# HyoJong-Moon/Distributed-Inference-System-based-Storm

Hardware: AMD Instinct MI355X
Metric: images/sec (whole node) + p50 latency, CIFAR-10 ResNet-20 at 1/2/4/8 GPUs (higher is better)
Workload: dtype bf16

## Files before the change

### csrc/bindings/host_bindings.cpp

```cpp
#include <pybind11/functional.h>
#include <pybind11/numpy.h>
#include <pybind11/pybind11.h>
#include <pybind11/stl.h>

#include <time.h>

#include <atomic>
#include <chrono>
#include <mutex>
#include <thread>

#include "../codec/json_codec.h"
#include "gale/llc_pair.h"
#include "../codec/text_pack.h"
#include "../kafka/broker.h"
#include "../kafka/client.h"
#include "../kafka/compress.h"
#include "../kafka/fetch_framing.h"
#include "../runtime/batch_plan.h"
#include "../runtime/ingest_plan.h"
#include "../runtime/pack_tap.h"
#include "../runtime/resize_plan.h"
#include "../kafka/protocol.h"
#include "../kafka/wire.h"
// ... 380 lines not shown
    const std::string_view s = view(b);
    const codec::Scan sc =
        codec::scan_instances(reinterpret_cast<const uint8_t*>(s.data()), s.size(), H, W, C);
    const int n = sc.status == codec::OK ? sc.images : 0;
    py::array_t<float> out({(py::ssize_t)n, (py::ssize_t)H, (py::ssize_t)W, (py::ssize_t)C});
    int images = 0;
    int st = sc.status;
    if (st == codec::OK)
      st = codec::parse_instances_host(reinterpret_cast<const uint8_t*>(s.data()), s.size(), H, W,
                                       C, out.mutable_data(), max_images, &images);
    return py::make_tuple(st, out);
  }, py::arg("data"), py::arg("H"), py::arg("W"), py::arg("C"), py::arg("max_images") = -1);
  m.def("scan_instances_b64", [](py::bytes b, int H, int W, int C) {
    const std::string_view s = view(b);
    const codec::Scan sc =
        codec::scan_instances_b64(reinterpret_cast<const uint8_t*>(s.data()), s.size(), H, W, C);
    return py::make_tuple(sc.status, sc.arr_off, sc.arr_len, sc.images);
  });
  m.def("parse_instances_b64_host", [](py::bytes b, int H, int W, int C, int max_images) {
    const std::string_view s = view(b);
    const uint8_t* p = reinterpret_cast<const uint8_t*>(s.data());
    const codec::Scan sc = codec::scan_instances_b64(p, s.size(), H, W, C);
    const int n = sc.status == codec::OK ? sc.images : 0;
    py::array_t<float> out({(py::ssize_t)n, (py::ssize_t)H, (py::ssize_t)W, (py::ssize_t)C});
    int images = 0;
    int st = sc.status;
    if (st == codec::OK)
      st = codec::parse_instances_b64_host(p, s.size(), H, W, C, out.mutable_data(), max_images,
                                           &images);
    return py::make_tuple(st, out);
  }, py::arg("data"), py::arg("H"), py::arg("W"), py::arg("C"), py::arg("max_images") = -1);
  m.def("b64_image_offsets", [](py::bytes arr, int H, int W, int C) -> py::object {
    const std::string_view s = view(arr);
    std::vector<uint32_t> offs;
    if (!codec::b64_image_offsets(reinterpret_cast<const uint8_t*>(s.data()), s.size(), H, W, C,
                                  offs))
      return py::none();
    return py::cast(offs);
  });
  m.def("plan_b64_ingest",
        [](std::vector<std::pair<int64_t, int64_t>> batches,
           std::vector<std::tuple<int, int, int64_t, int64_t, int64_t>> recs,
           std::vector<uint32_t> offs, int H, int W, int C, size_t arena_bytes,
           size_t fetch_size, bool check_crcs) {
          std::vector<B64PlanRecord> rs(recs.size());
          for (size_t i = 0; i < recs.size(); ++i) {
            rs[i].status = std::get<0>(recs[i]);
            rs[i].images = std::get<1>(recs[i]);
            rs[i].value_off = std::get<2>(recs[i]);
            rs[i].value_len = std::get<3>(recs[i]);
            rs[i].arr_off = std::get<4>(recs[i]);
          }
          B64IngestPlan p;
          plan_b64_ingest(batches, kafka::kBatchAttrOffset, check_crcs, rs, offs, H, W, C,
                          arena_bytes, fetch_size, p);
          py::list windows, imgs;
          for (const CrcChunk& c : p.chunks) windows.append(py::make_tuple(c.end, c.len));
          for (const B64Image& d : p.imgs) imgs.append(py::make_tuple(d.off, d.slot, d.rec));
          py::dict out;
          out["windows"] = windows;
          out["batch_windows"] = py::cast(p.batch_chunks);
          out["images"] = imgs;
          out["slot0"] = py::cast(p.slot0);
          out["img0"] = py::cast(p.img0);
          out["chunks_per_image"] = p.chunks_per_image;
          out["lo"] = p.lo;
          out["hi"] = p.hi;
          out["o_chunks"] = p.o_chunks;
          out["o_imgs"] = p.o_imgs;
          out["plan_bytes"] = p.plan_bytes;
          out["o_crc"] = p.o_crc;
          out["o_bad"] = p.o_bad;
          out["result_bytes"] = p.result_bytes;
          return out;
        },
        py::arg("batches"), py::arg("recs"), py::arg("offs"), py::arg("H"), py::arg("W"),
        py::arg("C"), py::arg("arena_bytes"), py::arg("fetch_size"),
        py::arg("check_crcs") = true,
        "The host plan of a b64 fetch's device ingest (csrc/runtime/ingest_plan.h)");
  m.def("plan_json_ingest",
        [](std::vector<std::pair<int64_t, int64_t>> batches,
           std::vector<std::tuple<int, int64_t, int64_t, int64_t, int64_t>> recs, int H, int W,
           int C, size_t arena_bytes, size_t fetch_size, size_t dev_cap, int64_t tap_result,
           bool plan_separate, bool check_crcs) {
          std::vector<JsonPlanRecord> rs(recs.size());
          for (size_t i = 0; i < recs.size(); ++i) {
            rs[i].status = std::get<0>(recs[i]);
            rs[i].value_off = std::get<1>(recs[i]);
            rs[i].value_len = std::get<2>(recs[i]);
            rs[i].arr_off = std::get<3>(recs[i]);
            rs[i].arr_len = std::get<4>(recs[i]);
          }
          JsonIngestPlan p;
          plan_json_ingest(batches, kafka::kBatchAttrOffset, check_crcs, rs, H, W, C, arena_bytes,
                           fetch_size, dev_cap, tap_result, plan_separate, p);
          std::string plan(p.o_gsum, '\0');
          if (!p.empty()) fill_json_ingest(p, rs, reinterpret_cast<uint8_t*>(&plan[0]));
          py::list windows;
          for (const CrcChunk& c : p.chunks) windows.append(py::make_tuple(c.end, c.len));
          py::dict out;
          out["windows"] = windows;
          out["batch_windows"] = py::cast(p.batch_chunks);
          out["rec_of"] = py::cast(p.rec_of);
          out["pjs"] = py::cast(p.pjs);
          out["nc"] = p.nc();
          out["nr"] = p.nr();
          out["np"] = p.np();
          out["ntiles"] = p.ntiles;
          out["ngroups"] = p.ngroups;
          out["ptiles"] = p.ptiles;
          out["ng"] = p.ng;
          out["packed"] = p.packed;
          out["lo"] = p.lo;
          out["span"] = p.span;
          out["link"] = p.link;
          out["c_lo"] = p.c_lo;
          out["c_len"] = p.c_len;
          out["tab_off"] = p.tab_off;
          out["used"] = p.used;
          out["cnt_base"] = p.cnt_base;
          out["o_chunks"] = p.o_chunks;
          out["o_groups"] = p.o_groups;
          out["o_recs"] = p.o_recs;
          out["o_precs"] = p.o_precs;
          out["o_ptr"] = p.o_ptr;
          out["o_gsum"] = p.o_gsum;
          out["prefix"] = p.o_gsum;
          out["o_crc"] = p.o_crc;
          out["o_gbad"] = p.o_gbad;
          out["o_pbad"] = p.o_pbad;
          out["io_bytes"] = p.io_bytes;
          out["plan_off"] = p.plan_off;
          out["plan_in_chunk"] = p.plan_in_chunk;
          out["plan"] = py::bytes(plan);
          return out;
        },
        py::arg("batches"), py::arg("recs"), py::arg("H"), py::arg("W"), py::arg("C"),
        py::arg("arena_bytes"), py::arg("fetch_size"), py::arg("dev_cap"),
        py::arg("tap_result") = (int64_t)-1, py::arg("plan_separate") = false,
        py::arg("check_crcs") = true,
        "The host plan of a JSON fetch's device ingest, laid out and filled "
        "(csrc/runtime/ingest_plan.h)");
  m.def("plan_batch",
        [](std::vector<py::dict> recs, int max_batch, int tiles_cap, int64_t per,
           const std::string& form, bool ptr_input, bool b64, uint64_t d_bytes,
           uint64_t input_base) {
          std::vector<BatchPlanRecord> rs(recs.size());
          std::vector<uint32_t> offs;
          for (size_t i = 0; i < recs.size(); ++i) {
            const py::dict& d = recs[i];
            BatchPlanRecord& r = rs[i];
            auto get = [&d](const char* k, auto& v) {
              if (d.contains(k)) v = d[k].cast<std::decay_t<decltype(v)>>();
            };
            get("buf", r.buf);
            get("arr_off", r.arr_off);
            get("arr_len", r.arr_len);
            get("images", r.images);
            get("pinned", r.pinned);
            get("resident", r.resident);
            get("preparsed", r.preparsed);
            get("dev_text", r.dev_text);
            get("dev_counts", r.dev_counts);
            get("dev_image", r.dev_image);
            if (d.contains("b64_offs")) {
              const auto o = d["b64_offs"].cast<std::vector<uint32_t>>();
              r.b64_first = (int32_t)offs.size();
              r.b64_n = (int32_t)o.size();
              offs.insert(offs.end(), o.begin(), o.end());
            }
          }
          const StepForm f = form == "op-by-op"   ? StepForm::OpByOp
                             : form == "captured" ? StepForm::Captured
                             : form == "kernels"  ? StepForm::Kernels
                                                  : throw std::invalid_argument("plan_batch: form");
          BatchPlan p;
          plan_batch(rs, max_batch, per, f, ptr_input, b64, p);
          const MetaLayout L(max_batch, std::max(tiles_cap, p.ntiles));
          const MetaRange used = L.used(p);
          std::string meta(L.total, '\xee');
          fill_batch(p, rs, offs, L, d_bytes, input_base, reinterpret_cast<uint8_t*>(&meta[0]));
          py::list spans, staged;
          for (const BatchPlan::Span& x : p.spans)
            spans.append(py::make_tuple(x.buf, x.lo, x.len, x.dev));
          for (const BatchPlan::Staged& g : p.staged)
            staged.append(py::make_tuple(g.rec, g.host, g.len));
          py::dict out;
          out["spans"] = spans;
          out["staged"] = staged;
          out["parse_idx"] = py::cast(p.parse_idx);
          out["staged_bytes"] = p.staged_bytes;
          out["staged_dev"] = p.staged_dev;
          out["dev_total"] = p.dev_total;
          out["nrec"] = p.nrec;
          out["ntiles"] = p.ntiles;
          out["img"] = p.img;
          out["b64n"] = p.b64n;
          out["npre"] = p.npre;
          out["resident"] = p.resident;
          out["count_pass"] = p.count_pass;
          py::dict lay;
          lay["hdr"] = L.hdr;
          lay["recs"] = L.recs;
          lay["xs"] = L.xs;
          lay["tiles"] = L.tiles;
          lay["b64_table"] = L.b64_table;
          lay["b64_status"] = L.b64_status;
          lay["total"] = L.total;
          out["layout"] = lay;
          out["used"] = py::make_tuple(used.off, used.bytes);
          out["meta"] = py::bytes(meta);
          return out;
        },
        py::arg("recs"), py::arg("max_batch"), py::arg("tiles_cap"), py::arg("per"),
        py::arg("form"), py::arg("ptr_input") = false, py::arg("b64") = false,
        py::arg("d_bytes") = (uint64_t)0, py::arg("input_base") = (uint64_t)0,
        "The host plan of a GPU replica's batch, laid out and filled "
        "(csrc/runtime/batch_plan.h)");
  m.attr("BATCH_ATTR_OFFSET") = (int)kafka::kBatchAttrOffset;
  m.def("split_instances_b64", [](py::bytes arr, int H, int W, int C) -> py::object {
    const std::string_view s = view(arr);
    std::vector<std::pair<uint32_t, uint32_t>> spans;
    if (!codec::split_instances_b64(reinterpret_cast<const uint8_t*>(s.data()), s.size(), H, W,
// ... 891 lines not shown
```

### csrc/bindings/module.cpp

```cpp
#include <pybind11/numpy.h>
#include <pybind11/pybind11.h>
#include <pybind11/stl.h>

#include <optional>
#include <stdexcept>
#include <vector>

#include "../comm/rccl.h"
#include "gale/executor.h"
#include "gale/kernels.h"

namespace py = pybind11;

namespace gale {
void bind_host(py::module_& m);
}

namespace {

using gale::ConvDesc;

template <typename T>
T get_or(const py::dict& d, const char* k, T dflt) {
  return d.contains(k) ? d[k].cast<T>() : dflt;
// ... 279 lines not shown
        [](int images, uintptr_t imgs, uintptr_t bytes, int HS, int WS, int C, uintptr_t out,
           uintptr_t status, uintptr_t stream, uintptr_t d_images, const std::string& format,
           std::optional<std::vector<float>> a, std::optional<std::vector<float>> b, bool nchw) {
          const auto prep = prep_from("b64_packed_instances", a, b, nchw);
          return (int)gale::b64_packed_instances(
              images, static_cast<const gale::B64Image*>(P(imgs)),
              static_cast<const uint8_t*>(P(bytes)), HS, WS, C, static_cast<float*>(P(out)),
              static_cast<int*>(P(status)), S(stream), static_cast<const int*>(P(d_images)),
              prep ? &*prep : nullptr, gale::packed_format_of(format.c_str()));
        },
        py::arg("images"), py::arg("imgs"), py::arg("bytes"), py::arg("HS"), py::arg("WS"),
        py::arg("C"), py::arg("out"), py::arg("status"), py::arg("stream"),
        py::arg("d_images") = 0, py::arg("format") = "bgr24", py::arg("a") = py::none(),
        py::arg("b") = py::none(), py::arg("nchw") = false);
  m.def("b64_yuv_pairs", &gale::b64_yuv_pairs);
  m.def("b64_yuv_lds_bytes", &gale::b64_yuv_lds_bytes);
  m.attr("YUV_LDS_BUDGET") = (int)gale::kYuvLdsBudget;
  m.attr("HIP_ERROR_INVALID_VALUE") = (int)hipErrorInvalidValue;
  m.attr("B64_IMAGE_BYTES") = (int)sizeof(gale::B64Image);
  py::module_ comm = m.def_submodule("comm", "in-process RCCL communicator (ncclCommInitAll)");
  py::class_<gale::CommGroup, std::shared_ptr<gale::CommGroup>>(comm, "CommGroup")
      .def(py::init([](std::vector<int> devices) {
             py::gil_scoped_release nogil;
             return std::make_shared<gale::CommGroup>(devices);
           }),
           py::arg("devices"))
      .def_property_readonly("size", &gale::CommGroup::size)
      .def_property_readonly("devices", &gale::CommGroup::devices)
      .def("broadcast",
           [](gale::CommGroup& g, uintptr_t send_root, std::vector<uintptr_t> recv, size_t bytes,
              int root) {
             std::vector<void*> r;
             for (uintptr_t p : recv) r.push_back(reinterpret_cast<void*>(p));
             py::gil_scoped_release nogil;
             g.broadcast(reinterpret_cast<const void*>(send_root), r, bytes, root);
           },
           py::arg("send_root"), py::arg("recv"), py::arg("bytes"), py::arg("root") = 0)
      .def("all_reduce_sum_f64",
           [](gale::CommGroup& g, std::vector<uintptr_t> bufs, size_t count) {
             std::vector<double*> b;
             for (uintptr_t p : bufs) b.push_back(reinterpret_cast<double*>(p));
             py::gil_scoped_release nogil;
             g.all_reduce_sum_f64(b, count);
           },
           py::arg("bufs"), py::arg("count"));
  m.def("crc32c_chunks",
        [](uintptr_t bytes, uintptr_t chunks, int n, uintptr_t tables, uintptr_t out,
           uintptr_t stream) {
          gale::check_hip(gale::crc32c_chunks(reinterpret_cast<const uint8_t*>(bytes),
                                              reinterpret_cast<const gale::CrcChunk*>(chunks), n,
                                              reinterpret_cast<const uint32_t*>(tables),
                                              reinterpret_cast<uint32_t*>(out),
                                              reinterpret_cast<hipStream_t>(stream)),
                          "crc32c_chunks");
        });
  m.def("ingest_crc_count",
        [](uintptr_t bytes, uintptr_t chunks, int nchunks, uintptr_t tables, uintptr_t crc_out,
           int nrec, int ngroups, uintptr_t recs, uintptr_t groups, uintptr_t counts,
           uintptr_t gsum, uintptr_t stream, uintptr_t gbad, uintptr_t packed, uintptr_t tab,
           uintptr_t text_out) {
          gale::check_hip(
              gale::ingest_crc_count(reinterpret_cast<const uint8_t*>(bytes),
                                     reinterpret_cast<const gale::CrcChunk*>(chunks), nchunks,
                                     reinterpret_cast<const uint32_t*>(tables),
                                     reinterpret_cast<uint32_t*>(crc_out), nrec, ngroups,
                                     reinterpret_cast<gale::JsonRecord*>(recs),
                                     reinterpret_cast<const int2*>(groups),
                                     reinterpret_cast<int*>(counts),
                                     reinterpret_cast<int*>(gsum),
                                     reinterpret_cast<int*>(gbad),
                                     reinterpret_cast<hipStream_t>(stream),
                                     reinterpret_cast<const uint8_t*>(packed),
                                     reinterpret_cast<const uint32_t*>(tab),
                                     reinterpret_cast<uint8_t*>(text_out)),
              "ingest_crc_count");
        },
        py::arg("bytes"), py::arg("chunks"), py::arg("nchunks"), py::arg("tables"),
        py::arg("crc_out"), py::arg("nrec"), py::arg("ngroups"), py::arg("recs"),
        py::arg("groups"), py::arg("counts"), py::arg("gsum"), py::arg("stream"),
        py::arg("gbad") = 0, py::arg("packed") = 0, py::arg("tab") = 0, py::arg("text_out") = 0,
        "groups: int32 (record, first tile) pairs, GROUP_TILES tiles each; counts: per record "
        "tile0 + grp0 -> [tile counts][group sums]; gsum: one int per group");
  m.attr("GROUP_TILES") = gale::kGroupTiles;
  m.def("ingest_crc_b64",
        [](uintptr_t bytes, uintptr_t chunks, int nchunks, uintptr_t tables, uintptr_t crc_out,
           int images, uintptr_t imgs, int H, int W, int C, uintptr_t arena, uintptr_t wg_bad,
           uintptr_t stream, std::optional<std::vector<float>> a,
           std::optional<std::vector<float>> b, bool nchw) {
          const auto prep = prep_from("ingest_crc_b64", a, b, nchw);
          chk(gale::ingest_crc_b64(static_cast<const uint8_t*>(P(bytes)),
                                   static_cast<const gale::CrcChunk*>(P(chunks)), nchunks,
                                   static_cast<const uint32_t*>(P(tables)),
                                   static_cast<uint32_t*>(P(crc_out)), images,
                                   static_cast<const gale::B64Image*>(P(imgs)), H, W, C,
                                   static_cast<float*>(P(arena)), static_cast<int*>(P(wg_bad)),
                                   S(stream), prep ? &*prep : nullptr),
              "ingest_crc_b64");
        },
        py::arg("bytes"), py::arg("chunks"), py::arg("nchunks"), py::arg("tables"),
        py::arg("crc_out"), py::arg("images"), py::arg("imgs"), py::arg("H"), py::arg("W"),
        py::arg("C"), py::arg("arena"), py::arg("wg_bad"), py::arg("stream"),
        py::arg("a") = py::none(), py::arg("b") = py::none(), py::arg("nchw") = false);
  m.attr("B64_CHUNK_CHARS") = gale::kB64ChunkChars;
  m.def("text_unpack", [](uintptr_t packed, uintptr_t tab, int64_t n, uintptr_t out,
                          uintptr_t stream) {
    if (out % 16 || packed % 8) throw std::invalid_argument("text_unpack: misaligned buffers");
    gale::check_hip(gale::text_unpack(reinterpret_cast<const uint8_t*>(packed),
                                      reinterpret_cast<const uint32_t*>(tab), n,
                                      reinterpret_cast<uint8_t*>(out),
                                      reinterpret_cast<hipStream_t>(stream)),
                    "text_unpack");
  });
  m.def("format_floats_java", [](int n, uintptr_t x, uintptr_t out16, uintptr_t stream) {
    gale::check_hip(gale::format_floats_java(n, reinterpret_cast<const float*>(x),
                                             reinterpret_cast<void*>(out16),
                                             reinterpret_cast<hipStream_t>(stream)),
                    "format_floats_java");
  });
  m.def("format_floats_java_dev",
        [](int max_n, uintptr_t d_count, int per, uintptr_t x, uintptr_t out16,
           uintptr_t stream) {
          chk(gale::format_floats_java_dev(max_n, static_cast<const int*>(P(d_count)), per,
                                           static_cast<const float*>(P(x)), P(out16), S(stream)),
              "format_floats_java_dev");
        },
        py::arg("max_n"), py::arg("d_count"), py::arg("per"), py::arg("x"), py::arg("out16"),
        py::arg("stream"));
  m.def("format_floats_java_step",
        [](int max_n, uintptr_t d_count, int per, uintptr_t x, uintptr_t out16, uintptr_t d_nrec,
           uintptr_t status, uintptr_t status_out, uintptr_t stream) {
          chk(gale::format_floats_java_step(max_n, static_cast<const int*>(P(d_count)), per,
                                            static_cast<const float*>(P(x)), P(out16),
                                            static_cast<const int*>(P(d_nrec)),
                                            static_cast<int*>(P(status)),
                                            static_cast<int*>(P(status_out)), S(stream)),
              "format_floats_java_step");
        },
        py::arg("max_n"), py::arg("d_count"), py::arg("per"), py::arg("x"), py::arg("out16"),
        py::arg("d_nrec"), py::arg("status"), py::arg("status_out"), py::arg("stream"));
  m.def("topk_java",
        [](int rows, int classes, int k, uintptr_t x, uintptr_t text16, uintptr_t idx,
           uintptr_t stream) {
          chk(gale::topk_java(rows, classes, k, static_cast<const float*>(P(x)), P(text16),
                              static_cast<int32_t*>(P(idx)), S(stream)),
              "topk_java");
        },
        py::arg("rows"), py::arg("classes"), py::arg("k"), py::arg("x"), py::arg("text16"),
        py::arg("idx"), py::arg("stream"));
  m.def("topk_java_dev",
        [](int max_rows, uintptr_t d_rows, int classes, int k, uintptr_t x, uintptr_t text16,
           uintptr_t idx, uintptr_t stream) {
          chk(gale::topk_java_dev(max_rows, static_cast<const int*>(P(d_rows)), classes, k,
                                  static_cast<const float*>(P(x)), P(text16),
                                  static_cast<int32_t*>(P(idx)), S(stream)),
              "topk_java_dev");
        },
        py::arg("max_rows"), py::arg("d_rows"), py::arg("classes"), py::arg("k"), py::arg("x"),
        py::arg("text16"), py::arg("idx"), py::arg("stream"));
  m.def("topk_java_step",
        [](int max_rows, uintptr_t d_rows, int classes, int k, uintptr_t x, uintptr_t text16,
           uintptr_t idx, uintptr_t d_nrec, uintptr_t status, uintptr_t status_out,
           uintptr_t stream) {
          chk(gale::topk_java_step(max_rows, static_cast<const int*>(P(d_rows)), classes, k,
                                   static_cast<const float*>(P(x)), P(text16),
                                   static_cast<int32_t*>(P(idx)),
                                   static_cast<const int*>(P(d_nrec)),
// ... 203 lines not shown
```

### csrc/include/gale/kernels.h

```cpp
#pragma once
#include <hip/hip_runtime.h>
#include <stdint.h>

#include "../../codec/pixfmt.h"
#include "../../codec/yuv.h"

namespace gale {

struct ConvDesc {
  int H, W, Cin;
  int Ho, Wo, Cout;
  int KH, KW, stride, pad;
  int K;
  int Kpad;
  int Npad;
  int relu;
  int has_res, res_H, res_W, res_C, res_stride;
  int in_f32;
  int out_f32;
  int fp8;
  float in_scale;
  float out_scale;
  float res_scale;
  int stem;
// ... 152 lines not shown
  int nchw = 0;
  float a[4] = {1.f, 1.f, 1.f, 1.f};
  float b[4] = {0.f, 0.f, 0.f, 0.f};
  bool identity() const {
    for (int i = 0; i < 4; ++i)
      if (a[i] != 1.f || b[i] != 0.f) return false;
    return !nchw;
  }
};
hipError_t json_parse_instances(int nrec, int ntiles, JsonRecord* recs, const int* tile_rec,
                                const uint8_t* bytes, int H, int W, int C, int* tile_counts,
                                float* out, hipStream_t stream, bool count_pass = true,
                                const int* d_ntiles = nullptr, int* status = nullptr,
                                int* tile_bad = nullptr, const InputPrep* prep = nullptr);

constexpr int kB64ChunkChars = 4096;
struct B64Image {
  int64_t off;
  int32_t slot;
  int32_t rec;
};
static_assert(sizeof(B64Image) == 16, "B64Image layout (host <-> device tables)");
hipError_t b64_decode_instances(int images, const B64Image* imgs, const uint8_t* bytes, int H,
                                int W, int C, float* out, int* status, hipStream_t stream,
                                const int* d_images = nullptr, const InputPrep* prep = nullptr);

constexpr size_t kYuvLdsBudget = 64 * 1024;
int b64_yuv_pairs(int HS, int WS);
size_t b64_yuv_lds_bytes(int WS, int pairs);
hipError_t b64_yuv_instances(int images, const B64Image* imgs, const uint8_t* bytes, int HS,
                             int WS, int C, float* out, int* status, hipStream_t stream,
                             const int* d_images, const InputPrep* prep, int format,
                             const YuvCoeffs& coeffs, int pairs = 0);

hipError_t b64_packed_instances(int images, const B64Image* imgs, const uint8_t* bytes, int HS,
                                int WS, int C, float* out, int* status, hipStream_t stream,
                                const int* d_images, const InputPrep* prep, int format);

struct ResizePlan {
  int HS = 0, WS = 0, H = 0, W = 0, C = 0;
  const int32_t* y0 = nullptr;
  const int32_t* y1 = nullptr;
  const float* wy = nullptr;
  const int32_t* x0 = nullptr;
  const int32_t* x1 = nullptr;
  const float* wx = nullptr;
};
hipError_t resize_crop(int images, const ResizePlan& plan, const float* src, float* dst,
                       hipStream_t stream);
hipError_t resize_crop_dev(int max_images, const int* d_images, const ResizePlan& plan,
                           const float* src, float* dst, hipStream_t stream);

struct ResizeAaPlan {
  int HS = 0, WS = 0, HR = 0, WR = 0, H = 0, W = 0, C = 0;
  int ty = 0, tx = 0;
  int band = 0, band_rows = 0;
  const int32_t* ys = nullptr;
  const int32_t* yn = nullptr;
  const float* wy = nullptr;
  const int32_t* xs = nullptr;
  const int32_t* xn = nullptr;
  const float* wx = nullptr;
};
hipError_t resize_crop_aa(int images, const ResizeAaPlan& plan, const float* src, float* dst,
                          hipStream_t stream);
hipError_t resize_crop_aa_dev(int max_images, const int* d_images, const ResizeAaPlan& plan,
                              const float* src, float* dst, hipStream_t stream);

constexpr int kCrcChunkBytes = 4096;
struct CrcChunk {
  int64_t end;
  int32_t len;
  int32_t pad_;
};
hipError_t crc32c_chunks(const uint8_t* bytes, const CrcChunk* chunks, int n,
                         const uint32_t* tables, uint32_t* out, hipStream_t stream);

hipError_t ingest_crc_count(const uint8_t* bytes, const CrcChunk* chunks, int nchunks,
                            const uint32_t* tables, uint32_t* crc_out, int nrec, int ngroups,
                            JsonRecord* recs, const int2* groups, int* counts, int* gsum,
                            int* gbad, hipStream_t stream, const uint8_t* packed = nullptr,
                            const uint32_t* tab = nullptr, uint8_t* text_out = nullptr);

hipError_t ingest_crc_b64(const uint8_t* bytes, const CrcChunk* chunks, int nchunks,
                          const uint32_t* tables, uint32_t* crc_out, int images,
                          const B64Image* imgs, int H, int W, int C, float* arena, int* wg_bad,
                          hipStream_t stream, const InputPrep* prep = nullptr);

hipError_t text_unpack(const uint8_t* packed, const uint32_t* tab, int64_t n, uint8_t* out,
                       hipStream_t stream);

constexpr int kFloatTextSlot = 16;
hipError_t format_floats_java(int n, const float* x, void* out16, hipStream_t stream);
hipError_t format_floats_java_dev(int max_n, const int* d_count, int per, const float* x,
                                  void* out16, hipStream_t stream);
hipError_t format_floats_java_step(int max_n, const int* d_count, int per, const float* x,
                                   void* out16, const int* d_nrec, int* status, int* status_out,
                                   hipStream_t stream);

hipError_t topk_java(int rows, int classes, int k, const float* x, void* text16, int32_t* idx,
                     hipStream_t stream);
hipError_t topk_java_dev(int max_rows, const int* d_rows, int classes, int k, const float* x,
                         void* text16, int32_t* idx, hipStream_t stream);
hipError_t topk_java_step(int max_rows, const int* d_rows, int classes, int k, const float* x,
                          void* text16, int32_t* idx, const int* d_nrec, int* status,
                          int* status_out, hipStream_t stream);

}
```

### csrc/kernels/json_parse.hip

```cpp
#include "common.cuh"
#include "crc32c.cuh"
#include "gale/kernels.h"
#include "exact_decimal.cuh"
#include "text_expand.cuh"

namespace gale {
namespace {

constexpr int kTile = kJsonTileBytes;
constexpr int kLaneBytes = kTile / 64;
constexpr int kChunks = kLaneBytes / 16;
static_assert(kChunks >= 1 && kChunks * 16 * 64 == kTile, "tile = 64 lanes x 16-byte chunks");
constexpr int kHalo = 64;
constexpr int kWaves = 4;
constexpr int kText = kTile + 2 * kHalo + 16;
constexpr int kMaxTok = kTile / 2;

__device__ __forceinline__ bool is_ws(unsigned c) {
  return c == ' ' || c == '\n' || c == '\r' || c == '\t';
}
__device__ __forceinline__ bool is_delim(unsigned c) {
  return c == '[' || c == ']' || c == ',' || is_ws(c);
}

__device__ __forceinline__ double pow10_exact(int k) {
  const double a = (k & 1) ? 1e1 : 1.0, b = (k & 2) ? 1e2 : 1.0, c = (k & 4) ? 1e4 : 1.0,
               d = (k & 8) ? 1e8 : 1.0, e = (k & 16) ? 1e16 : 1.0;
  return ((a * b) * (c * d)) * e;
}

constexpr uint32_t kHi03 = 0x08060001u, kHi47 = 0x00102010u;
constexpr uint32_t kLo03 = 0x0808080Au, kLo47 = 0x08081808u, kLo8B = 0x24010908u,
                   kLoCF = 0x00042502u;
constexpr uint32_t kDelimG = 0x23232323u, kNumG = 0x1C1C1C1Cu, kDigitG = 0x08080808u;

__device__ __forceinline__ uint32_t classify4(uint32_t x) {
  const uint32_t hi = __builtin_amdgcn_perm(kHi47, kHi03, (x >> 4) & 0x07070707u);
  const uint32_t l = x & 0x0F0F0F0Fu;
  const uint32_t s = l & 0x07070707u;
  const uint32_t p0 = __builtin_amdgcn_perm(kLo47, kLo03, s);
  const uint32_t p1 = __builtin_amdgcn_perm(kLoCF, kLo8B, s);
  const uint32_t m = ((l >> 3) & 0x01010101u) * 0xFFu;
  const uint32_t lo = (m & p1) | (~m & p0);
  const uint32_t ascii = ~(((x >> 7) & 0x01010101u) * 0xFFu);
  return hi & lo & ascii;
}

__device__ __forceinline__ uint32_t nz4(uint32_t cls, uint32_t g) {
  const uint32_t t = ((cls & g) + 0x7F7F7F7Fu) & 0x80808080u;
  return ((t >> 7) * 0x01020408u) >> 24;
}

struct Masks16 {
  uint32_t delim, num, digit;
};

__device__ __forceinline__ Masks16 classify16(uint32_t w0, uint32_t w1, uint32_t w2,
                                              uint32_t w3) {
  const uint32_t c0 = classify4(w0), c1 = classify4(w1), c2 = classify4(w2), c3 = classify4(w3);
  Masks16 m;
  m.delim = nz4(c0, kDelimG) | nz4(c1, kDelimG) << 4 | nz4(c2, kDelimG) << 8 |
            nz4(c3, kDelimG) << 12;
  m.num = nz4(c0, kNumG) | nz4(c1, kNumG) << 4 | nz4(c2, kNumG) << 8 | nz4(c3, kNumG) << 12;
  m.digit = nz4(c0, kDigitG) | nz4(c1, kDigitG) << 4 | nz4(c2, kDigitG) << 8 |
            nz4(c3, kDigitG) << 12;
  return m;
}

__device__ __forceinline__ uint32_t bits_range(int a, int b) {
  return b > a ? ((1u << b) - 1u) & ~((1u << a) - 1u) : 0u;
}

__device__ __forceinline__ uint32_t valid16(int p, int beg, int end) {
  return bits_range(min(max(beg - p, 0), 16), min(max(end - p, 0), 16));
}

__device__ __forceinline__ uint32_t chunk_masks(const Masks16& m, int p, int beg, int end) {
  const uint32_t vm = valid16(p, beg, end);
  return ((m.delim | ~vm) & 0xFFFFu) | (m.digit & vm) << 16;
}

__device__ __forceinline__ void token_starts(const uint4 (&v)[kChunks], int o, int beg, int end,
                                             bool prev_delim, uint32_t (&st)[kChunks],
                                             uint32_t (&cm)[kChunks], bool* bad) {
  uint32_t carry = prev_delim ? 1u : 0u;
  bool b = false;
#pragma unroll
  for (int i = 0; i < kChunks; ++i) {
    const Masks16 m = classify16(v[i].x, v[i].y, v[i].z, v[i].w);
    cm[i] = chunk_masks(m, o + 16 * i, beg, end);
    const uint32_t dx = cm[i] & 0xFFFFu;
    const uint32_t tokb = ~dx & 0xFFFFu;
    b |= (tokb & ~m.num) != 0;
    st[i] = tokb & ((dx << 1) | carry) & 0xFFFFu;
    carry = dx >> 15;
  }
  *bad = b;
}

__device__ __forceinline__ int wave_sum_i(int v) {
#pragma unroll
  for (int o = 32; o > 0; o >>= 1) v += __shfl_xor(v, o, 64);
  return v;
}

__device__ __forceinline__ void wave_lds_sync() { asm volatile("s_waitcnt lgkmcnt(0)" ::: "memory"); }

struct Text {
  const uint8_t* g;
  const uint8_t* l;
  int lbase, lo, hi;
  __device__ __forceinline__ unsigned at(int q) const {
    return (q >= lo && q < hi) ? (unsigned)l[q - lbase] : (unsigned)g[q];
  }
};


__device__ __forceinline__ void limbs_mul(uint32_t* N, int* nl, uint32_t m) {
  uint64_t carry = 0;
  for (int i = 0; i < *nl; ++i) {
    const uint64_t v = (uint64_t)N[i] * m + carry;
    N[i] = (uint32_t)(v % 1000000000ull);
    carry = v / 1000000000ull;
  }
  while (carry) {
    N[(*nl)++] = (uint32_t)(carry % 1000000000ull);
    carry /= 1000000000ull;
  }
}

__device__ __noinline__ int cmp_token_dyadic(const Text& t, int i0, int end, uint64_t K, int E) {
  uint32_t N[16];
  int nl = 0, s = 0;
  for (uint64_t k = K; k || nl == 0; k /= 1000000000ull) N[nl++] = (uint32_t)(k % 1000000000ull);
  if (E >= 0) {
    for (int k = E; k > 0; k -= 29) limbs_mul(N, &nl, 1u << (k < 29 ? k : 29));
  } else {
    s = -E;
    for (int k = s; k > 0; k -= 13) {
      uint32_t p = 1;
      for (int j = 0; j < (k < 13 ? k : 13); ++j) p *= 5u;
      limbs_mul(N, &nl, p);
    }
  }
  int top = 1;
  for (uint32_t v = N[nl - 1]; v >= 10; v /= 10) ++top;
  const int nd = 9 * (nl - 1) + top;
  int k = i0;
  if (t.at(k) == '-') ++k;
  int int_sig = 0, lead_zeros = 0, first = -1;
  unsigned c = k < end ? t.at(k) : 0u;
  for (; c >= '0' && c <= '9'; c = ++k < end ? t.at(k) : 0u)
    if (first >= 0 || c != '0') {
      if (first < 0) first = k;
      ++int_sig;
    }
  if (c == '.')
    for (c = ++k < end ? t.at(k) : 0u; c >= '0' && c <= '9'; c = ++k < end ? t.at(k) : 0u)
      if (first < 0) {
        if (c == '0') ++lead_zeros;
        else first = k;
      }
  int ex = 0;
  if (c == 'e' || c == 'E') {
    c = ++k < end ? t.at(k) : 0u;
    const bool eneg = c == '-';
    if (c == '+' || c == '-') c = ++k < end ? t.at(k) : 0u;
    for (; c >= '0' && c <= '9'; c = ++k < end ? t.at(k) : 0u)
      if (ex < 100000) ex = ex * 10 + (int)(c - '0');
    if (eneg) ex = -ex;
  }
  if (first < 0) return -1;
  const int Lx = (int_sig > 0 ? int_sig : -lead_zeros) + ex, Lm = nd - s;
  if (Lx != Lm) return Lx > Lm ? 1 : -1;
  int j = nd - 1;
  for (k = first; k < end; ++k) {
    c = t.at(k);
    if (c == '.') continue;
    if (c < '0' || c > '9') break;
    int dm = 0;
    if (j >= 0) {
      uint32_t v = N[j / 9];
      for (int r = j % 9; r > 0; --r) v /= 10;
      dm = (int)(v % 10);
    }
    const int dx = (int)(c - '0');
// ... 301 lines not shown
  const uint64_t pat = k == 0 ? 0x2Cull : k == 1 ? 0x5B2C5Dull
                     : k == 2 ? 0x5B5B2C5D5Dull : 0x5B5B5B2C5D5D5Dull;
  if ((g >> (8 * (8 - plen))) != pat) return false;
  const uint32_t prev = (uint32_t)(g >> (8 * (7 - plen))) & 0xFFu;
  return prev - '0' < 10u;
}

__device__ __forceinline__ int tile_tokens(const JsonRecord& r, int tl, const uint8_t* bytes,
                                           bool* bad) {
  const int lane = threadIdx.x & 63;
  const int64_t abeg = r.off & ~(int64_t)15;
  const uint8_t* rb = bytes + abeg;
  const int beg = (int)(r.off - abeg), end = beg + r.len;
  const int o = tl * kTile + kLaneBytes * lane;
  uint4 v[kChunks];
#pragma unroll
  for (int i = 0; i < kChunks; ++i)
    v[i] = (o + 16 * i < end) ? *reinterpret_cast<const uint4*>(rb + o + 16 * i)
                              : make_uint4(0, 0, 0, 0);
  unsigned prevb = __shfl_up(v[kChunks - 1].w >> 24, 1, 64);
  if (lane == 0 && o - 1 >= beg) prevb = rb[o - 1];
  const bool pd = (o - 1 < beg) || is_delim(prevb);
  uint32_t st[kChunks], cm[kChunks];
  token_starts(v, o, beg, end, pd, st, cm, bad);
  int lc = 0;
#pragma unroll
  for (int i = 0; i < kChunks; ++i) lc += __builtin_popcount(st[i]);
  return wave_sum_i(lc);
}

__device__ __forceinline__ int tile_tokens_packed(const JsonRecord& r, int tl, uint8_t* bytes,
                                                  const PackedText& pt, bool* bad) {
  const int lane = threadIdx.x & 63;
  const int64_t abeg = r.off & ~(int64_t)15;
  uint8_t* rb = bytes + abeg;
  const int beg = (int)(r.off - abeg), end = beg + r.len;
  const int o = tl * kTile + kLaneBytes * lane;
  uint4 v[kChunks];
#pragma unroll
  for (int i = 0; i < kChunks; ++i) {
    if (o + 16 * i < end) {
      v[i] = expand16(pt, abeg + o + 16 * i);
      *reinterpret_cast<uint4*>(rb + o + 16 * i) = v[i];
    } else {
      v[i] = make_uint4(0, 0, 0, 0);
    }
  }
  unsigned prevb = __shfl_up(v[kChunks - 1].w >> 24, 1, 64);
  if (lane == 0 && o - 1 >= beg) prevb = expand16(pt, abeg + o - 16).w >> 24;
  const bool pd = (o - 1 < beg) || is_delim(prevb);
  uint32_t st[kChunks], cm[kChunks];
  token_starts(v, o, beg, end, pd, st, cm, bad);
  int lc = 0;
#pragma unroll
  for (int i = 0; i < kChunks; ++i) lc += __builtin_popcount(st[i]);
  return wave_sum_i(lc);
}

__device__ __forceinline__ int record_tiles(const JsonRecord& r) {
  const int64_t abeg = r.off & ~(int64_t)15;
  return (int)((r.off + r.len - abeg + kTile - 1) / kTile);
}

__device__ __forceinline__ void count_tile(JsonRecord* recs, const int* tile_rec, int t,
                                           const uint8_t* bytes, int* counts, int* status) {
  const int ri = tile_rec[t];
  const JsonRecord r = recs[ri];
  if (r.has_cnt) return;
  bool bad;
  const int cnt = tile_tokens(r, t - r.tile0, bytes, &bad);
  if ((threadIdx.x & 63) == 0) counts[t] = cnt;
  if (bad) atomicMax(status ? &status[ri] : &recs[ri].status, 2);
}

template <bool PACKED>
__device__ __forceinline__ void count_group(JsonRecord* recs, const int2* groups, int g,
                                            uint8_t* bytes, const PackedText& pt, int* counts,
                                            int* gsum, int* gbad, int* lds8) {
  const int wave = threadIdx.x >> 6;
  const int2 gr = groups[g];
  const JsonRecord r = recs[gr.x];
  const int nt = record_tiles(r);
  const int tl = gr.y + wave;
  int cnt = 0;
  bool bad = false;
  if (tl < nt) {
    cnt = PACKED ? tile_tokens_packed(r, tl, bytes, pt, &bad)
                 : tile_tokens(r, tl, bytes, &bad);
    if ((threadIdx.x & 63) == 0) counts[r.tile0 + (int)r.grp0 + tl] = cnt;
    if (bad && !gbad) atomicMax(&recs[gr.x].status, 2);
    bad = __ballot(bad) != 0;
  }
  if ((threadIdx.x & 63) == 0) {
    lds8[wave] = cnt;
    lds8[kGroupTiles + wave] = bad ? 1 : 0;
  }
  __syncthreads();
  if (threadIdx.x == 0) {
    int acc = 0, nbad = 0;
#pragma unroll
    for (int w = 0; w < kGroupTiles; ++w) {
      acc += lds8[w];
      nbad += lds8[kGroupTiles + w];
    }
    counts[r.tile0 + (int)r.grp0 + nt + gr.y / kGroupTiles] = acc;
    gsum[g] = acc;
    if (gbad) gbad[g] = nbad ? 2 : 0;
  }
}

__global__ __launch_bounds__(256) void json_count_kernel(JsonRecord* recs, const int* tile_rec,
                                                         int ntiles, const uint8_t* bytes,
                                                         int* counts, const int* d_ntiles,
                                                         int* status) {
  const int t = blockIdx.x * kWaves + (threadIdx.x >> 6);
  if (d_ntiles) ntiles = min(ntiles, *d_ntiles);
  if (t >= ntiles) return;
  count_tile(recs, tile_rec, t, bytes, counts, status);
}

__device__ __forceinline__ void crc_windows_packed(const PackedText& pt, const CrcChunk* chunks,
                                                   int n, const uint32_t* T, uint32_t* out,
                                                   int block, int nblocks) {
  const int lane = threadIdx.x & 63, wave = threadIdx.x >> 6;
  for (int c = block * crc::kCrcWaves + wave; c < n; c += nblocks * crc::kCrcWaves) {
    const CrcChunk ch = chunks[c];
    const int64_t cs = ch.end - ch.len;
    const int64_t wa = ch.end - (int64_t)64 * (64 - lane);
    const int64_t hi = wa + 64;
    uint32_t crc = 0;
    if (hi > cs) {
      const int64_t b16 = wa & ~(int64_t)15;
      uint32_t w[20];
#pragma unroll
      for (int j = 0; j < 5; ++j) {
        const int64_t p = b16 + 16 * j;
        const uint4 v = (p < hi && p + 16 > cs) ? expand16(pt, p) : make_uint4(0, 0, 0, 0);
        w[4 * j] = v.x;
        w[4 * j + 1] = v.y;
        w[4 * j + 2] = v.z;
        w[4 * j + 3] = v.w;
      }
      const uint32_t sh = (uint32_t)(wa & 3);
      uint32_t x[16];
      switch ((int)((wa & 15) >> 2)) {
#define GALE_ALIGN_WORDS(D)                                                       \
  _Pragma("unroll") for (int t = 0; t < 16; ++t) x[t] =                           \
      __builtin_amdgcn_alignbyte(w[t + (D) + 1], w[t + (D)], sh);
        case 0: GALE_ALIGN_WORDS(0) break;
        case 1: GALE_ALIGN_WORDS(1) break;
        case 2: GALE_ALIGN_WORDS(2) break;
        default: GALE_ALIGN_WORDS(3) break;
#undef GALE_ALIGN_WORDS
      }
#pragma unroll
      for (int t = 0; t < 16; ++t) {
        const int64_t at = wa + 4 * t;
        uint32_t v = x[t];
        if (at + 4 <= cs) v = 0;
        else if (at < cs) v &= 0xffffffffu << (8 * (uint32_t)(cs - at));
        crc = crc::crc_word(T, crc, v);
      }
    }
    crc = crc::gf2_mulmod(crc, T[1024 + lane]);
#pragma unroll
    for (int o = 32; o > 0; o >>= 1) crc ^= __shfl_xor(crc, o, 64);
    if (lane == 0) out[c] = crc;
  }
}

static_assert(kGroupTiles == kWaves, "one tile group per counting workgroup");
template <bool PACKED>
__global__ __launch_bounds__(256) void ingest_crc_count_kernel(
    uint8_t* bytes, PackedText pt, const CrcChunk* chunks, int nchunks, const uint32_t* tables,
    uint32_t* crc_out, int crc_blocks, JsonRecord* recs, const int2* groups, int ngroups,
    int* counts, int* gsum, int* gbad) {
  __shared__ uint32_t T[crc::kTableWords];
  if ((int)blockIdx.x < crc_blocks) {
    crc::crc_stage_tables(tables, T);
    if (PACKED)
      crc_windows_packed(pt, chunks, nchunks, T, crc_out, blockIdx.x, crc_blocks);
    else
      crc::crc_windows(bytes, chunks, nchunks, T, crc_out, blockIdx.x, crc_blocks);
    return;
  }
  const int g = (int)blockIdx.x - crc_blocks;
  if (g >= ngroups) return;
  count_group<PACKED>(recs, groups, g, bytes, pt, counts, gsum, gbad, reinterpret_cast<int*>(T));
}

template <bool PREP>
__device__ __forceinline__ void json_parse_tile(JsonRecord* recs, const int* tile_rec, int ntiles,
                                                const uint8_t* bytes, int H, int W, int C,
                                                const int* counts, float* out,
                                                const int* d_ntiles, int* status, int* tile_bad,
                                                const InputPrep& prep) {
  __shared__ __attribute__((aligned(16))) uint8_t lds_text[kWaves][kText];
  __shared__ uint16_t lds_tok[kWaves][kMaxTok];
  __shared__ uint32_t lds_cm[kWaves][kTile / 16 + 1];
  const int lane = threadIdx.x & 63, wave = threadIdx.x >> 6;
  const int t = blockIdx.x * kWaves + wave;
  if (d_ntiles) ntiles = min(ntiles, *d_ntiles);
  if (t >= ntiles) return;
  uint8_t* text = lds_text[wave];
  uint16_t* tok = lds_tok[wave];
  uint32_t* cmk = lds_cm[wave];
  const int ri = tile_rec[t];
  const JsonRecord r = recs[ri];
  const int64_t abeg = r.off & ~(int64_t)15;
  const uint8_t* rb = bytes + abeg;
  const int beg = (int)(r.off - abeg), end = beg + r.len;
  const int aend = (end + 15) & ~15;
  const int per_image = H * W * C;
  int expected = r.images * per_image;
  if (r.images < 0) {
    const int* rc = reinterpret_cast<const int*>(bytes + r.cnt_off);
    const int nt = record_tiles(r);
    const int ng = (nt + kGroupTiles - 1) / kGroupTiles;
    int s = 0;
    for (int k = lane; k < ng; k += 64) s += rc[nt + k];
    const int tot = wave_sum_i(s);
    expected = (tot % per_image == 0 && tot / per_image <= r.len / (2 * per_image)) ? tot : 0;
  }
  const int tl = t - r.tile0;
  const int t0 = tl * kTile;
  const bool last_tile = t0 + kTile >= end;

  Text tx;
  tx.g = rb;
  tx.l = text;
  tx.lbase = t0 - kHalo;
  tx.lo = max(t0 - kHalo, 0);
  tx.hi = min(t0 + kTile + kHalo, aend);
  for (int q = tx.lo + 16 * lane; q < tx.hi; q += 16 * 64)
    *reinterpret_cast<uint4*>(text + (q - tx.lbase)) = *reinterpret_cast<const uint4*>(rb + q);

  int part = 0;
  if (r.has_cnt) {
    const int* rc = reinterpret_cast<const int*>(bytes + r.cnt_off);
    const int* gs = rc + record_tiles(r);
    const int gi = tl / kGroupTiles;
    for (int k = lane; k < gi; k += 64) part += gs[k];
    if (lane < tl - gi * kGroupTiles) part += rc[gi * kGroupTiles + lane];
  } else {
    for (int k = r.tile0 + lane; k < t; k += 64) part += counts[k];
  }
  const int base = wave_sum_i(part);
  wave_lds_sync();

  const int o = t0 + kLaneBytes * lane;
  uint4 v[kChunks];
#pragma unroll
  for (int i = 0; i < kChunks; ++i)
    v[i] = (o + 16 * i < end) ? *reinterpret_cast<const uint4*>(text + (o + 16 * i - tx.lbase))
                              : make_uint4(0, 0, 0, 0);
  const bool pd = (o - 1 < beg) || is_delim(text[o - 1 - tx.lbase]);
  uint32_t st[kChunks], cm[kChunks];
  bool bad_ignored;
  token_starts(v, o, beg, end, pd, st, cm, &bad_ignored);
#pragma unroll
  for (int i = 0; i < kChunks; ++i) cmk[kChunks * lane + i] = cm[i];
  if (lane == 63) {
    const int p = t0 + kTile;
    const uint4 h = p < end ? *reinterpret_cast<const uint4*>(text + (p - tx.lbase))
                            : make_uint4(0, 0, 0, 0);
    cmk[kTile / 16] = chunk_masks(classify16(h.x, h.y, h.z, h.w), p, beg, end);
  }
  int cnt = 0;
#pragma unroll
  for (int i = 0; i < kChunks; ++i) cnt += __builtin_popcount(st[i]);
  int inc = cnt;
#pragma unroll
  for (int d = 1; d < 64; d <<= 1) {
    const int u = __shfl_up(inc, d, 64);
    if (lane >= d) inc += u;
  }
  const int ntok = __shfl(inc, 63, 64);
  int li = inc - cnt;
#pragma unroll
  for (int i = 0; i < kChunks; ++i) {
    uint32_t s = st[i];
    while (s) {
      const int j = __builtin_ctz(s);
      s &= s - 1;
      tok[li++] = (uint16_t)(o + 16 * i + j - tx.lbase);
    }
  }
  wave_lds_sync();

  const bool nchw = PREP && prep.nchw;
  const int d0 = nchw ? W : C, d1 = nchw ? H : W, d2 = nchw ? C : H;
  Dims dims;
  dims.C = (uint32_t)d0; dims.W = (uint32_t)d1; dims.H = (uint32_t)d2;
  dims.rC = 1.0 / d0; dims.rW = 1.0 / d1; dims.rH = 1.0 / d2;
  float* dst = out + (int64_t)r.slot * per_image;
  int bad = 0;
  for (int j = lane; j < ntok; j += 64) {
    const int x = tok[j];
    const int pos = x + tx.lbase;
    const int idx = base + j;
    float val;
    int len = 0;
    bool ok;
    const int ci = (pos - t0) >> 4;
    if (parse_window(text, x, cmk[ci], cmk[ci + 1], pos & 15, &val)) {
      ok = true;
      len = -1;
    } else {
      ok = false;
      val = parse_number(tx, pos, end, &ok, &len);
    }
    int kn = 0;
    if (PREP) {
      const uint32_t px = udiv_rcp((uint32_t)idx, dims.C, dims.rC);
      const uint32_t i0 = (uint32_t)idx - px * dims.C;
      uint32_t sidx = (uint32_t)idx, ch = i0;
      if (prep.nchw) {
        const uint32_t row = udiv_rcp(px, dims.W, dims.rW);
        const uint32_t i1 = px - row * dims.W;
        const uint32_t img = udiv_rcp(row, dims.H, dims.rH);
        ch = row - img * dims.H;
        kn = i0 ? 0 : i1 ? 1 : ch ? 2 : 3;
        sidx = img * (uint32_t)per_image + (i1 * (uint32_t)W + i0) * (uint32_t)C + ch;
      }
      if (idx < expected) {
        const float a = ch == 0 ? prep.a[0] : ch == 1 ? prep.a[1] : ch == 2 ? prep.a[2] : prep.a[3];
        const float b = ch == 0 ? prep.b[0] : ch == 1 ? prep.b[1] : ch == 2 ? prep.b[2] : prep.b[3];
        dst[sidx] = __builtin_fmaf(val, a, b);
      }
    }
    if (!ok) {
      bad = max(bad, 2);
    } else {
      const int k = idx <= 0 ? 0 : (PREP && prep.nchw) ? kn : wraps((uint32_t)idx, dims);
      const bool fast_gap = idx > 0 && pos - 8 >= tx.lo && pos - (2 * k + 2) >= beg &&
                            gap_window(text, x, k);
      if (!fast_gap && !gap_ok(tx, beg, pos, (uint32_t)idx, k)) {
        bad = 3;
      } else if (idx == expected - 1) {
        if (len < 0) parse_number(tx, pos, end, &ok, &len);
        if (!tail_ok(tx, pos + len, end)) bad = 3;
      }
    }
    if (!PREP && idx < expected) dst[idx] = val;
  }
  if (last_tile && lane == 0 && base + ntok != expected) bad = max(bad, 1);
  if (tile_bad) {
#pragma unroll
    for (int d = 32; d > 0; d >>= 1) bad = max(bad, __shfl_xor(bad, d, 64));
    if (lane == 0) tile_bad[t] = bad;
  } else if (bad) {
    atomicMax(status ? &status[ri] : &recs[ri].status, bad);
  }
}

__global__ __launch_bounds__(256) void json_parse_kernel(JsonRecord* recs, const int* tile_rec,
                                                         int ntiles, const uint8_t* bytes, int H,
                                                         int W, int C, const int* counts,
                                                         float* out, const int* d_ntiles,
                                                         int* status, int* tile_bad) {
  json_parse_tile<false>(recs, tile_rec, ntiles, bytes, H, W, C, counts, out, d_ntiles, status,
                         tile_bad, InputPrep());
}

__global__ __launch_bounds__(256) __attribute__((amdgpu_waves_per_eu(4, 4)))
void json_parse_prep_kernel(JsonRecord* recs, const int* tile_rec, int ntiles,
                            const uint8_t* bytes, int H, int W, int C, const int* counts,
                            float* out, const int* d_ntiles, int* status, int* tile_bad,
                            InputPrep prep) {
  json_parse_tile<true>(recs, tile_rec, ntiles, bytes, H, W, C, counts, out, d_ntiles, status,
                        tile_bad, prep);
}

}



hipError_t ingest_crc_count(const uint8_t* bytes, const CrcChunk* chunks, int nchunks,
                            const uint32_t* tables, uint32_t* crc_out, int nrec, int ngroups,
                            JsonRecord* recs, const int2* groups, int* counts, int* gsum,
                            int* gbad, hipStream_t stream, const uint8_t* packed,
                            const uint32_t* tab, uint8_t* text_out) {
  if (nrec <= 0) ngroups = 0;
  int crc_blocks = (nchunks + crc::kCrcWaves - 1) / crc::kCrcWaves;
  if (crc_blocks > 1024) crc_blocks = 1024;
  if (crc_blocks + ngroups == 0) return hipSuccess;
  if (packed) {
    if (!tab || !text_out || (reinterpret_cast<uintptr_t>(packed) & 7) ||
        (reinterpret_cast<uintptr_t>(text_out) & 15))
      return hipErrorInvalidValue;
    hipLaunchKernelGGL(ingest_crc_count_kernel<true>, dim3(crc_blocks + ngroups), dim3(256), 0,
                       stream, text_out, PackedText{packed, tab}, chunks, nchunks, tables,
                       crc_out, crc_blocks, recs, groups, ngroups, counts, gsum, gbad);
  } else {
    hipLaunchKernelGGL(ingest_crc_count_kernel<false>, dim3(crc_blocks + ngroups), dim3(256), 0,
                       stream, const_cast<uint8_t*>(bytes), PackedText{nullptr, nullptr}, chunks,
                       nchunks, tables, crc_out, crc_blocks, recs, groups, ngroups, counts, gsum,
                       gbad);
  }
  return hipGetLastError();
}

hipError_t json_parse_instances(int nrec, int ntiles, JsonRecord* recs, const int* tile_rec,
                                const uint8_t* bytes, int H, int W, int C, int* tile_counts,
                                float* out, hipStream_t stream, bool count_pass,
                                const int* d_ntiles, int* status, int* tile_bad,
                                const InputPrep* prep) {
  if (nrec <= 0 || ntiles <= 0) return hipSuccess;
  if (H <= 0 || W <= 0 || C <= 0) return hipErrorInvalidValue;
  const bool with_prep = prep && !prep->identity();
  if (with_prep) {
    if ((int64_t)H * W * C >= (1 << 20)) return hipErrorInvalidValue;
    if (C > 4)
      for (int i = 1; i < 4; ++i)
        if (prep->a[i] != prep->a[0] || prep->b[i] != prep->b[0]) return hipErrorInvalidValue;
  }
  if (tile_bad && count_pass) return hipErrorInvalidValue;
  const int blocks = (ntiles + kWaves - 1) / kWaves;
  if (count_pass)
    hipLaunchKernelGGL(json_count_kernel, dim3(blocks), dim3(64 * kWaves), 0, stream, recs,
                       tile_rec, ntiles, bytes, tile_counts, d_ntiles, status);
  if (with_prep)
    hipLaunchKernelGGL(json_parse_prep_kernel, dim3(blocks), dim3(64 * kWaves), 0, stream, recs,
                       tile_rec, ntiles, bytes, H, W, C, tile_counts, out, d_ntiles, status,
                       tile_bad, *prep);
  else
    hipLaunchKernelGGL(json_parse_kernel, dim3(blocks), dim3(64 * kWaves), 0, stream, recs,
                       tile_rec, ntiles, bytes, H, W, C, tile_counts, out, d_ntiles, status,
                       tile_bad);
  return hipGetLastError();
}

}
```

### csrc/runtime/engine.cpp

```cpp
#include "engine.h"
#include "gale/llc_pair.h"
#include "gale/thread_name.h"

#include <hip/hip_runtime.h>
#include <stdio.h>
#include <stdlib.h>
#include <string.h>
#include <sched.h>
#include <sys/prctl.h>

#include <algorithm>
#include <sstream>

#include "../codec/json_codec.h"
#include "../kafka/compress.h"
#include "pack_tap.h"
#include "../kafka/fetch_framing.h"
#include "trace.h"

namespace gale {


class Engine::Batcher {
 public:
// ... 212 lines not shown
bool Engine::fault_hit(double p) {
  if (p <= 0) return false;
  std::lock_guard<std::mutex> lk(rng_mu_);
  return std::uniform_real_distribution<double>(0, 1)(rng_) < p;
}

void Engine::start() {
  if (running_) return;
  if (replicas_.empty()) throw std::logic_error("engine: no replicas");
  for (int i = 0; i < cfg_.sink_parallelism; ++i) {
    kafka::ProducerConfig pc;
    pc.bootstrap = cfg_.bootstrap;
    pc.client_id = cfg_.client_id + "-sink-" + std::to_string(i);
    pc.acks = cfg_.acks;
    pc.linger_ms = cfg_.linger_ms;
    pc.batch_size = cfg_.batch_size;
    pc.buffer_memory = cfg_.producer_buffer_bytes;
    pc.max_request_size = (int)cfg_.producer_request_bytes;
    pc.compression = kafka::codec_from_name(cfg_.compression);
    pc.retries = cfg_.producer_retries;
    pc.retry_backoff_ms = cfg_.retry_backoff_ms;
    pc.delivery_timeout_ms = cfg_.delivery_timeout_ms;
    pc.fail_p = producer_fail_p_;
    pc.fail_seed = cfg_.seed + (uint64_t)i + 1;
    auto prod = std::make_unique<kafka::Producer>(pc);
    std::lock_guard<std::mutex> lk(prod_mu_);
    producers_.push_back(std::move(prod));
  }
  std::vector<int> parts = cfg_.partitions;
  int ns = cfg_.source_parallelism;
  if (!cfg_.group_membership) {
    if (parts.empty()) {
      kafka::Cluster cl(kafka::ClientConfig{cfg_.bootstrap, cfg_.client_id, 30000, 10000});
      const int n = cl.partitions(cfg_.input_topic);
      if (n <= 0) throw kafka::KafkaError(kafka::UNKNOWN_TOPIC_OR_PARTITION,
                                          "input topic " + cfg_.input_topic + " not found");
      for (int p = 0; p < n; ++p) parts.push_back(p);
    }
    ns = std::min<int>(cfg_.source_parallelism, (int)parts.size());
  } else if (cfg_.group_id.empty()) {
    throw std::invalid_argument("engine: group_membership needs a group_id");
  }
  src_ctl_.clear();
  for (int i = 0; i < ns; ++i) src_ctl_.push_back(std::make_unique<SourceCtl>());
  if (!cfg_.group_membership) {
    for (size_t i = 0; i < parts.size(); ++i) src_ctl_[i % (size_t)ns]->parts.push_back(parts[i]);
    for (auto& c : src_ctl_) c->epoch = 1;
  }
  slot_key_.clear();
  slot_dev_.clear();
  for (auto& rs : replicas_) {
    const int key = rs->rep->locality();
    auto it = std::find(slot_key_.begin(), slot_key_.end(), key);
    rs->slot = (int)(it - slot_key_.begin());
    if (it == slot_key_.end()) {
      slot_key_.push_back(key);
      slot_dev_.push_back(rs->rep->device() >= 0 ? rs->rep->device() : key);
    }
  }
  const size_t nslots = slot_key_.size();
  batchers_.clear();
  for (size_t i = 0; i < nslots; ++i)
    batchers_.push_back(std::make_unique<Batcher>(
        (size_t)std::max(1, cfg_.queue_depth / (int)nslots)));
  pools_.assign(nslots, nullptr);
  for (size_t i = 0; i < nslots; ++i) {
    bool gpu = false;
    for (auto& rs : replicas_) gpu |= rs->slot == (int)i && rs->rep->device() >= 0;
    if (!gpu || cfg_.pinned_fetch_bytes <= 0) continue;
    const size_t body = (size_t)cfg_.fetch_max_bytes + (1 << 20);
    const bool pack = cfg_.text_pack && ingest_for((int)i);
    const size_t budget = (size_t)cfg_.pinned_fetch_bytes * (pack ? 2 : 1) / nslots;
    pools_[i] = std::make_shared<PinnedPool>(pack ? codec::pack_layout_bytes(body) + 4096 : body,
                                             budget);
    if (ingest_for((int)i)) {
      const size_t per = (size_t)cfg_.rec_h() * cfg_.rec_w() * cfg_.C;
      const size_t b64_L = 4 * ((per + 2) / 3);
      const size_t slots = !per ? 0 : cfg_.input_b64 ? body / b64_L + 2 : body / (2 * per) + 2;
      const size_t arena = cfg_.ingest_parse ? slots * per * 4 : 0;
      pools_[i]->set_mirror_device(slot_dev_[i], arena);
    }
    pools_[i]->set_wait_ms(200);
  }
  running_ = true;
  stopping_ = false;
  workers_done_ = false;
  sources_done_ = false;
  sources_active_ = ns;
  dec_closed_ = false;
  for (int i = 0; i < cfg_.decode_threads; ++i)
    decoders_.emplace_back([this, i] {
      name_thread("gl-dec", i);
      prctl(PR_SET_TIMERSLACK, 1000UL, 0, 0, 0);
      decode_loop(i);
    });
  for (auto& rs : replicas_)
    workers_.emplace_back([this, rs] {
      name_thread("gl-rep", rs->index);
      pin_thread(rs->rep->device());
      prctl(PR_SET_TIMERSLACK, 1000UL, 0, 0, 0);
      worker_loop(rs.get());
    });
  for (int i = 0; i < ns; ++i)
    sources_.emplace_back([this, i] {
      name_thread("gl-src", i);
      pin_thread(slot_dev_[(size_t)i % slot_dev_.size()]);
      llc::pin_self_next_domain();
      source_loop(i);
    });
  group_stop_ = false;
  if (cfg_.group_membership)
    group_thread_ = std::thread([this] {
      name_thread("gl-group");
      group_loop();
    });
  watchdog_ = std::thread([this] {
    name_thread("gl-watchdog");
    watchdog_loop();
  });
}

void Engine::stop() {
  if (!running_) return;
  stopping_ = true;
  {
    std::lock_guard<std::mutex> lk(dec_mu_);
  }
  dec_space_cv_.notify_all();
  {
    std::unique_lock<std::mutex> lk(done_mu_);
    done_cv_.wait_for(lk, std::chrono::seconds(30), [&] { return sources_active_ == 0; });
  }
  {
    std::lock_guard<std::mutex> lk(dec_mu_);
    dec_closed_ = true;
  }
  dec_cv_.notify_all();
  dec_space_cv_.notify_all();
  for (auto& t : decoders_) t.join();
  decoders_.clear();
  for (auto& b : batchers_) b->close();
  for (size_t i = 0; i < workers_.size(); ++i) {
    if (replicas_[i]->alive || replicas_[i]->restarting) {
      workers_[i].join();
    } else {
      workers_[i].detach();
    }
  }
  workers_done_ = true;
  workers_.clear();
  for (auto& p : producers_) p->flush();
  sources_done_ = true;
  done_cv_.notify_all();
  for (auto& t : sources_) t.join();
  sources_.clear();
  group_stop_ = true;
  if (group_thread_.joinable()) group_thread_.join();
  running_ = false;
  done_cv_.notify_all();
  if (watchdog_.joinable()) watchdog_.join();
  for (auto& p : producers_) p->close();
  {
    std::lock_guard<std::mutex> lk(prod_mu_);
    for (const auto& p : producers_) {
      const kafka::ProducerStats ps = p->stats();
      prod_retried_ += ps.records_retried;
// ... 420 lines not shown
  for (;;) {
    FetchItem it;
    {
      std::unique_lock<std::mutex> lk(dec_mu_);
      dec_cv_.wait(lk, [&] { return !dec_q_.empty() || dec_closed_; });
      if (dec_q_.empty()) return;
      it = std::move(dec_q_.front());
      dec_q_.pop_front();
      dec_space_cv_.notify_one();
    }
    good.clear();
    const int64_t t0 = mono_ns();
    {
      trace::Range tr("gale:decode");
      decode_fetch(it, good, idx);
    }
    ns_decode_ += mono_ns() - t0;
    if (!good.empty()) batchers_[(size_t)it.slot]->push_many(good, stopping_);
  }
}

bool Engine::ingest_fetch(FetchItem& it, std::vector<InRecord>& good, int lane) {
  Ingest* ingest = ingest_for(it.slot);
  if (!ingest || !it.pinned || ingest_failed_) return false;
  kafka::Fetched& f = it.f;
  uint8_t* dev = pools_[(size_t)it.slot]->mirror(f.buf.get());
  if (!dev) return false;
  const int64_t t0 = mono_ns();
  ns_lane_wait_ += t0 - it.t_fetch_ns;
  const size_t n = f.records.size();
  IngestIO io;
  io.status.assign(n, codec::OK);
  io.arr_off.assign(n, 0);
  io.arr_len.assign(n, 0);
  const bool b64 = cfg_.input_b64;
  if (b64 && f.sparse) throw std::logic_error("engine: sparse fetch buffer in b64 mode");
  if (b64) io.images.assign(n, 0);
  std::vector<uint32_t> offs;
  int64_t b64_accepted = 0;
  for (size_t i = 0; i < n; ++i) {
    const kafka::RecordRef& rr = f.records[i];
    if (rr.poison) {
      io.status[i] = codec::CORRUPT;
      continue;
    }
    if (rr.value_len < 0) {
      io.status[i] = codec::BAD_ENVELOPE;
      continue;
    }
    if (b64) {
      const uint8_t* v = f.buf.get() + rr.value_off;
      codec::Scan s = codec::scan_instances_b64_bytes(v, (size_t)rr.value_len, cfg_.rec_bytes());
      if (s.status == codec::OK &&
          (!codec::b64_image_offsets_bytes(v + s.arr_off, (size_t)s.arr_len, cfg_.rec_bytes(),
                                           offs) ||
           (int64_t)offs.size() != s.images))
        s.status = codec::BAD_SHAPE;
      io.status[i] = s.status;
      io.arr_off[i] = s.arr_off;
      io.arr_len[i] = s.arr_len;
      if (s.status != codec::OK) continue;
      io.images[i] = (int32_t)s.images;
      io.b64_offs.insert(io.b64_offs.end(), offs.begin(), offs.end());
      ++b64_accepted;
      continue;
    }
    const codec::Scan s =
        f.sparse ? codec::scan_envelope(f.buf.get() + rr.value_off, (size_t)rr.value_len,
                                        kafka::FramingWalker::kHead, kafka::FramingWalker::kTail)
                 : codec::scan_envelope(f.buf.get() + rr.value_off, (size_t)rr.value_len);
    io.status[i] = s.status;
    io.arr_off[i] = s.arr_off;
    io.arr_len[i] = s.arr_len;
  }
  PinnedPool& pool = *pools_[(size_t)it.slot];
  const size_t arena_bytes = pool.mirror_extra();
  float* arena =
      arena_bytes ? reinterpret_cast<float*>(dev + pool.mirror_extra_offset()) : nullptr;
  try {
    if (b64) {
      const PixelSource::Dims sd = cfg_.pixels.ingest_dims(cfg_.rec_h(), cfg_.rec_w(), cfg_.C);
      ingest->run_b64(lane, f, dev, pool.chunk_bytes(), cfg_.check_crcs && !f.crc_checked, sd.H,
                      sd.W, sd.C, io, arena, arena_bytes);
    } else
      ingest->run(lane, f, dev, pool.chunk_bytes(), cfg_.check_crcs && !f.crc_checked,
                  cfg_.rec_h(), cfg_.rec_w(), cfg_.C, io, arena, arena_bytes);
  } catch (const std::exception& e) {
    if (!ingest_failed_.exchange(true))
      fprintf(stderr, "[gale decode] GPU ingest failed (%s): host decode from now on\n", e.what());
    return false;
  }
  b64_records_ += b64_accepted;
  if (cfg_.pixels.kind() == PixelSource::YUV) yuv_records_ += b64_accepted;
  if (cfg_.pixels.kind() == PixelSource::PACKED) packed_records_ += b64_accepted;
  std::vector<char> corrupt(n, 0);
  for (size_t b = 0; b < f.batches.size(); ++b)
    if (!io.batch_ok[b])
      for (size_t i = 0; i < f.batches[b].nrec; ++i) corrupt[f.batches[b].first_rec + i] = 1;
  kafka::Producer* prod = producer_for(it.source);
  for (size_t i = 0; i < n; ++i) {
    const kafka::RecordRef& rr = f.records[i];
    InRecord r;
    r.buf = f.buf;
    r.pinned = true;
    r.value = rr.value_len >= 0 ? f.buf.get() + rr.value_off : nullptr;
    r.len = rr.value_len;
    r.key = rr.key_len >= 0 ? f.buf.get() + rr.key_off : nullptr;
    r.key_len = rr.key_len;
    r.partition = rr.partition;
    r.offset = rr.offset;
    r.timestamp_ms = rr.timestamp;
    r.t_fetch_ns = it.t_fetch_ns;
    r.source = it.source;
    r.dev_value = dev + rr.value_off;
    r.dev_locality = slot_key_[(size_t)it.slot];
    if (io.cnt_off[i] >= 0) r.dev_counts = dev + io.cnt_off[i];
    r.dev_image = io.img[i];
    r.dev_arena = r.dev_image ? arena : nullptr;
    if (r.dev_image) ++ingest_parsed_;
    ++records_in_;
    if (r.len >= 0) bytes_in_ += r.len;
    r.status = corrupt[i] ? (int)codec::CORRUPT : io.status[i];
    r.arr_off = io.arr_off[i];
    r.arr_len = io.arr_len[i];
    r.images = io.images[i];
    if (r.status == codec::OK && fault_hit(parse_error_p_)) r.status = codec::BAD_ENVELOPE;
    if (r.status == codec::OK && r.images > cfg_.max_batch) {
      images_in_ += r.images;
      if (f.sparse) {
        f.restore();
        ++restored_fetches_;
      }
      if (!split_record(r, good)) emit_error(r, codec::BAD_SHAPE, prod);
    } else if (r.status == codec::OK) {
      images_in_ += r.images;
      good.push_back(std::move(r));
    } else {
      emit_error(r, r.status, prod);
    }
  }
  ingested_records_ += (int64_t)n;
  ingest_ns_ += mono_ns() - t0;
  return true;
}

void Engine::decode_fetch(FetchItem& it, std::vector<InRecord>& good, int lane) {
  if (ingest_fetch(it, good, lane)) return;
  kafka::Fetched& f = it.f;
  if (f.sparse) {
    f.restore();
    ++restored_fetches_;
  }
  std::vector<char> corrupt;
  std::vector<codec::Scan> pre;
  std::vector<char> have_pre;
  const bool nchw = cfg_.prep.nchw != 0;
  const int rec_h = cfg_.rec_h(), rec_w = cfg_.rec_w();
  const int scan_h = nchw ? cfg_.C : rec_h, scan_w = nchw ? rec_h : rec_w,
            scan_c = nchw ? rec_w : cfg_.C;
  const bool b64 = cfg_.input_b64;
  auto scan = [&](const uint8_t* p, size_t n) {
    return b64 ? codec::scan_instances_b64_bytes(p, n, cfg_.rec_bytes())
               : codec::scan_instances(p, n, scan_h, scan_w, scan_c);
  };
  if (cfg_.check_crcs && !f.crc_checked) {
    corrupt.assign(f.records.size(), 0);
    pre.resize(f.records.size());
    have_pre.assign(f.records.size(), 0);
    const uint8_t* base = f.buf.get();
    for (const kafka::BatchSpan& b : f.batches) {
      const uint8_t* p = base + b.off;
      kafka::Reader r(p + kafka::kBatchCrcOffset, 4);
      const uint32_t want = r.u32();
      const uint8_t* pos = p + kafka::kBatchAttrOffset;
      const uint8_t* end = p + b.len;
      uint32_t crc = 0;
      for (size_t i = b.first_rec; i < b.first_rec + b.nrec; ++i) {
        const kafka::RecordRef& rr = f.records[i];
        if (rr.value_len < 0) continue;
        const uint8_t* vend = base + rr.value_off + rr.value_len;
        if (vend > pos && vend <= end) {
          crc = kafka::crc32c(pos, (size_t)(vend - pos), crc);
          pos = vend;
        }
        pre[i] = scan(base + rr.value_off, (size_t)rr.value_len);
        have_pre[i] = 1;
      }
      if (end > pos) crc = kafka::crc32c(pos, (size_t)(end - pos), crc);
      if (crc != want)
        for (size_t i = 0; i < b.nrec; ++i) corrupt[b.first_rec + i] = 1;
    }
  }
  kafka::Producer* prod = producer_for(it.source);
  for (size_t i = 0; i < f.records.size(); ++i) {
    const kafka::RecordRef& rr = f.records[i];
    InRecord r;
    r.buf = f.buf;
    r.pinned = it.pinned;
    r.value = rr.value_len >= 0 ? f.buf.get() + rr.value_off : nullptr;
    r.len = rr.value_len;
// ... 699 lines not shown
      lag_max = std::max(lag_max, o.lag);
    }
    s["lag_records"] = (double)lag;
    s["lag_records_max"] = (double)lag_max;
    s["fetch_lag_records"] = (double)fetch_lag;
  }
  s["batches"] = (double)batches_total_;
  size_t queued = 0;
  for (auto& q : batchers_) queued += q->size();
  s["queue_records"] = (double)queued;
  s["locality_slots"] = (double)batchers_.size();
  s["steals"] = (double)steals_;
  for (int i = 1; i < codec::kStatusCount; ++i)
    s[std::string("err_") + codec::status_name(i)] = (double)err_by_status_[i];
  const double el = (double)(t_last_ns_ - t_first_ns_) * 1e-9;
  s["elapsed_s"] = el > 0 ? el : 0;
  s["images_per_s"] = el > 0 ? (double)images_out_ / el : 0;
  auto q = [&](const char* n, const Histogram& h) {
    s[std::string(n) + "_p50"] = h.quantile(0.5);
    s[std::string(n) + "_p90"] = h.quantile(0.9);
    s[std::string(n) + "_p99"] = h.quantile(0.99);
    s[std::string(n) + "_max"] = (double)h.max();
    s[std::string(n) + "_mean"] = h.mean();
  };
  q("queue_us", h_queue_us_);
  q("device_us", h_device_us_);
  q("e2e_us", h_engine_e2e_us_);
  q("record_e2e_ms", h_record_e2e_ms_);
  q("batch_images", h_batch_images_);
  int alive = 0;
  for (auto& r : replicas_) alive += r->alive ? 1 : 0;
  s["replicas_alive"] = alive;
  s["rebalances"] = (double)rebalances_;
  s["lag_rebalances"] = (double)lag_rebalances_;
  s["lag_rebalances_skipped"] = (double)lag_rebalances_skipped_;
  s["capacity_rps"] = capacity_rps_.load();
  s["generation"] = (double)generation_;
  s["assigned_partitions"] = cfg_.group_membership ? (double)assigned_partitions_
                                                   : (double)partition_offsets().size();
  s["ingested_records"] = (double)ingested_records_;
  s["ingest_parsed_records"] = (double)ingest_parsed_;
  {
    int64_t step = 0, fwd = 0, pre = 0, tab = 0, rsz = 0;
    for (auto& r : replicas_) {
      rsz += r->rep->resized_images();
      step += r->rep->graph_step_batches();
      fwd += r->rep->graph_forward_batches();
      pre += r->rep->preparsed_records();
      tab += r->rep->table_batches();
    }
    s["resized_images"] = (double)rsz;
    s["table_batches"] = (double)tab;
    s["graph_step_batches"] = (double)step;
    s["graph_forward_batches"] = (double)fwd;
    s["preparsed_records"] = (double)pre;
  }
  {
    int64_t text = 0, link = 0;
    for (auto& kv : ingests_) {
      int64_t t = 0, l = 0;
      kv.second->link_bytes(t, l);
      text += t;
      link += l;
    }
    s["ingest_text_bytes"] = (double)text;
    s["ingest_link_bytes"] = (double)link;
  }
  s["thread_s_ingest"] = ingest_ns_ * 1e-9;
  {
    Ingest::Timing t;
    for (auto& kv : ingests_) {
      const Ingest::Timing q = kv.second->timing();
      t.runs += q.runs;
      t.prep_ns += q.prep_ns;
      t.plan_ns += q.plan_ns;
      t.wait_ns += q.wait_ns;
      t.post_ns += q.post_ns;
      t.dev_runs += q.dev_runs;
      t.dev_copy_ns += q.dev_copy_ns;
      t.dev_count_ns += q.dev_count_ns;
      t.dev_parse_ns += q.dev_parse_ns;
      t.dev_wait_ns += q.dev_wait_ns;
      t.plan_in_chunk += q.plan_in_chunk;
    }
    const double n = (double)std::max<int64_t>(1, t.runs);
    s["ingest_fetches"] = (double)t.runs;
    s["ingest_lane_wait_us"] = (double)ns_lane_wait_ / n / 1e3;
    s["ingest_prep_us"] = (double)t.prep_ns / n / 1e3;
    s["ingest_device_wait_us"] = (double)t.wait_ns / n / 1e3;
    s["ingest_post_us"] = (double)t.post_ns / n / 1e3;
    s["ingest_lane_us"] = (double)ingest_ns_ / n / 1e3;
    s["ingest_lane_wait_s"] = (double)ns_lane_wait_ * 1e-9;
    s["ingest_prep_s"] = (double)t.prep_ns * 1e-9;
    s["ingest_plan_s"] = (double)t.plan_ns * 1e-9;
    s["ingest_device_wait_s"] = (double)t.wait_ns * 1e-9;
    s["ingest_post_s"] = (double)t.post_ns * 1e-9;
    s["ingest_plan_in_chunk"] = (double)t.plan_in_chunk;
    s["ingest_dev_runs"] = (double)t.dev_runs;
    s["ingest_dev_copy_s"] = (double)t.dev_copy_ns * 1e-9;
    s["ingest_dev_count_s"] = (double)t.dev_count_ns * 1e-9;
    s["ingest_dev_parse_s"] = (double)t.dev_parse_ns * 1e-9;
    s["ingest_dev_wait_s"] = (double)t.dev_wait_ns * 1e-9;
  }
  s["eff_max_batch"] = (double)eff_batch_;
  s["eff_max_wait_us"] = (double)eff_wait_ns_ / 1000.0;
  s["slo_adjustments"] = (double)slo_adjustments_;
  s["thread_s_poll"] = ns_poll_ * 1e-9;
  s["thread_s_handoff"] = ns_handoff_ * 1e-9;
  s["thread_s_decode"] = ns_decode_ * 1e-9;
  s["thread_s_take"] = ns_take_ * 1e-9;
  s["thread_s_submit"] = ns_submit_ * 1e-9;
  s["thread_s_wait"] = ns_wait_ * 1e-9;
  s["thread_s_finish"] = ns_finish_ * 1e-9;
  return s;
}

std::vector<ReplicaStats> Engine::replica_stats() const {
  std::vector<ReplicaStats> v;
  for (auto& r : replicas_) {
    ReplicaStats s;
    s.name = r->rep->name();
    s.device = r->rep->device();
    s.alive = r->alive;
    s.batches = r->batches;
    s.images = r->images;
    s.records = r->records;
    s.restarts = r->restarts;
    s.slot = r->slot;
    s.resident_records = r->rep->resident_records();
    s.host_records = r->rep->host_records();
    v.push_back(s);
  }
  return v;
}

std::vector<PartitionOffsets> Engine::partition_offsets() const {
  std::vector<PartitionOffsets> v;
  std::lock_guard<std::mutex> lk(const_cast<std::mutex&>(pend_mu_));
  for (const auto& kv : next_fetch_) {
    PartitionOffsets o;
    o.partition = kv.first;
    o.fetched = kv.second;
    auto pit = pending_.find(kv.first);
    o.committed = (pit != pending_.end() && !pit->second.empty()) ? pit->second.first()
                                                                  : kv.second;
    auto hit = high_watermark_.find(kv.first);
    o.high_watermark = hit != high_watermark_.end() ? hit->second : -1;
    if (o.high_watermark >= 0) {
      o.lag = std::max<int64_t>(0, o.high_watermark - o.committed);
      o.fetch_lag = std::max<int64_t>(0, o.high_watermark - o.fetched);
    }
    v.push_back(o);
  }
  return v;
}

void Engine::reset_stats() {
  h_queue_us_.reset();
  h_device_us_.reset();
  h_engine_e2e_us_.reset();
  h_record_e2e_ms_.reset();
  h_batch_images_.reset();
  images_out_ = 0;
  records_out_ = 0;
  bytes_in_ = 0;
  ns_poll_ = ns_decode_ = ns_take_ = ns_submit_ = ns_wait_ = ns_finish_ = ns_handoff_ = 0;
  t_first_ns_ = mono_ns();
  t_last_ns_ = t_first_ns_.load();
}

}
```

### csrc/runtime/engine.h

```cpp
#pragma once
#include <stdint.h>

#include <atomic>
#include <condition_variable>
#include <deque>
#include <map>
#include <memory>
#include <mutex>
#include <random>
#include <set>
#include <string>
#include <utility>
#include <thread>
#include <vector>

#include "../kafka/client.h"
#include "ingest.h"
#include "metrics.h"
#include "pinned_pool.h"
#include "replica.h"

namespace gale {

struct EngineConfig {
// ... 159 lines not shown
  }
  bool empty() const { return npending == 0 && sparse.empty(); }
  int64_t first() const {
    if (npending == 0) return *sparse.begin();
    return sparse.empty() ? base : std::min(base, *sparse.begin());
  }
};

class Engine {
 public:
  explicit Engine(EngineConfig cfg);
  ~Engine();
  Engine(const Engine&) = delete;
  Engine& operator=(const Engine&) = delete;

  void add_replica(std::shared_ptr<Replica> r);
  void set_ingest(std::shared_ptr<Ingest> ing);
  void start();
  void stop();
  bool wait(int64_t timeout_ms);
  bool wait_completed(int64_t n, int64_t timeout_ms);
  std::pair<int64_t, int64_t> last_wait() const {
    std::lock_guard<std::mutex> lk(done_mu_);
    return {last_wait_ns_, last_wait_c_};
  }
  bool running() const { return running_; }
  int64_t completed() const { return completed_.load(); }

  std::map<std::string, double> stats() const;
  std::vector<ReplicaStats> replica_stats() const;
  std::vector<PartitionOffsets> partition_offsets() const;
  void reset_stats();
  void set_ack_log(bool on, size_t capacity = 8u << 20);
  std::vector<AckSample> take_ack_log();
  const EngineConfig& config() const { return cfg_; }

 private:
  struct ReplicaSlot;
  class Batcher;
  struct FetchItem {
    kafka::Fetched f;
    int source = 0;
    int slot = 0;
    int64_t t_fetch_ns = 0;
    bool pinned = false;
  };

  struct SourceCtl {
    std::mutex mu;
    std::condition_variable cv;
    std::vector<int> parts;
    uint64_t epoch = 0, acked = 0;
    int32_t generation = -1;
    std::string member;
  };
  void source_loop(int idx);
  void group_loop();
  bool distribute(const std::vector<int>& parts, int32_t generation, const std::string& member,
                  int timeout_ms);
  bool drain_pending(const std::vector<int>& parts, int timeout_ms);
  void decode_loop(int idx);
  void decode_fetch(FetchItem& it, std::vector<InRecord>& good, int lane);
  bool ingest_fetch(FetchItem& it, std::vector<InRecord>& good, int lane);
  void worker_loop(ReplicaSlot* rs);
  void serve(ReplicaSlot* rs);
  void watchdog_loop();
  void slo_step();
  void finish_batch(ReplicaSlot* rs, Batch& b);
  void emit(InRecord& r, std::string value, bool null_value, kafka::Producer* prod);
  bool split_record(InRecord& r, std::vector<InRecord>& good);
  void fragment_done(const InRecord& frag, std::string rows, int status, kafka::Producer* prod);
  void emit_error(InRecord& r, int status, kafka::Producer* prod);
  void complete_record(const InRecord& r, bool ok);
  void complete_records(const std::vector<InRecord>& rs, bool ok);
  void undelivered(const std::vector<InRecord>& rs);
  void commit(kafka::Consumer& c, const std::vector<int>& parts);
  kafka::Producer* producer_for(int i);
  bool fault_hit(double p);

  EngineConfig cfg_;
  std::vector<std::shared_ptr<ReplicaSlot>> replicas_;
  std::vector<std::unique_ptr<Batcher>> batchers_;
  std::vector<int> slot_key_;
  std::vector<int> slot_dev_;
  std::vector<std::unique_ptr<kafka::Producer>> producers_;
  std::vector<std::thread> sources_, workers_, decoders_;
  std::vector<std::unique_ptr<SourceCtl>> src_ctl_;
  std::thread group_thread_;
  std::atomic<bool> group_stop_{false};
  std::atomic<int64_t> rebalances_{0};
  std::atomic<int> assigned_partitions_{0}, generation_{-1};
  std::vector<std::shared_ptr<PinnedPool>> pools_;
  std::map<int, std::shared_ptr<Ingest>> ingests_;
  Ingest* ingest_for(int slot);
  void pin_thread(int device);
  std::atomic<int64_t> steals_{0};
  std::atomic<bool> ingest_failed_{false};
  std::atomic<int64_t> ingested_records_{0}, ingest_ns_{0};
  std::atomic<int64_t> ingest_parsed_{0};
  std::mutex dec_mu_;
  std::condition_variable dec_cv_, dec_space_cv_;
  std::deque<FetchItem> dec_q_;
  bool dec_closed_ = false;
  std::thread watchdog_;
  std::atomic<bool> running_{false}, stopping_{false}, sources_done_{false},
      workers_done_{false};
  std::atomic<int> sources_active_{0};

  std::mutex pend_mu_;
  std::map<int, OffsetWindow> pending_;
  std::map<int, int64_t> next_fetch_;
  std::map<int, int64_t> high_watermark_;

  mutable std::mutex done_mu_;
  int64_t hit_target_ = 0, hit_ns_ = 0, hit_c_ = 0, last_wait_ns_ = 0, last_wait_c_ = 0;
  void note_completed(int64_t c, int64_t now);
  std::condition_variable done_cv_;
  std::atomic<int64_t> completed_{0};
  std::atomic<int64_t> wait_target_{0};

  int64_t crash_at_batch_ = -1;
  double parse_error_p_ = 0, producer_fail_p_ = 0;
  std::atomic<int64_t> undelivered_{0};
  mutable std::mutex prod_mu_;
  int64_t prod_retried_ = 0, prod_req_failed_ = 0;
  std::atomic<bool> delivery_failed_{false};
  std::atomic<int64_t> batches_total_{0};
  std::mutex rng_mu_;
  std::mt19937_64 rng_;

  std::atomic<int64_t> records_in_{0}, images_in_{0}, records_out_{0}, images_out_{0};
  std::atomic<int64_t> bytes_in_{0}, errors_{0}, produce_failures_{0}, dropped_{0};
  std::atomic<int64_t> requeued_{0}, replica_failures_{0}, replica_restarts_{0}, commits_{0};
  std::atomic<int64_t> err_by_status_[16] = {};
  std::atomic<int64_t> converted_batches_{0}, poison_batches_{0}, poison_records_{0};
  std::atomic<int64_t> poison_unknown_span_{0};
  std::atomic<int64_t> split_records_{0}, split_fragments_{0};
  std::atomic<int64_t> b64_records_{0};
  std::atomic<int64_t> yuv_records_{0};
  std::atomic<int64_t> packed_records_{0};
  std::atomic<int64_t> sparse_fetches_{0}, restored_fetches_{0};
  Histogram h_queue_us_, h_device_us_, h_engine_e2e_us_, h_record_e2e_ms_, h_batch_images_;
  Histogram h_slo_win_us_;
  Histogram h_slo_batch_;
  std::atomic<int> eff_batch_{0};
  std::atomic<int64_t> eff_wait_ns_{0};
  std::atomic<int64_t> slo_adjustments_{0};
  std::atomic<int64_t> ns_poll_{0}, ns_decode_{0}, ns_take_{0}, ns_submit_{0}, ns_wait_{0},
      ns_finish_{0};
  std::atomic<int64_t> ns_handoff_{0};
  std::atomic<int64_t> ns_lane_wait_{0};
  int64_t replica_busy_ns() const;
  std::atomic<double> capacity_rps_{0.0};
  std::atomic<int64_t> lag_rebalances_{0};
  std::atomic<int64_t> lag_rebalances_skipped_{0};
  std::atomic<int64_t> t_first_ns_{0}, t_last_ns_{0};
  std::atomic<bool> ack_log_on_{false};
  std::mutex ack_mu_;
  static constexpr size_t kAckBlock = 1 << 16;
  std::vector<std::unique_ptr<AckSample[]>> ack_blocks_;
  size_t ack_n_ = 0;
  size_t ack_cap_ = 0;
  void ack_push(const AckSample& a);
};

}
// ... 1 lines not shown
```

### csrc/runtime/gpu_ingest.cpp

```cpp
#include "gpu_ingest.h"
#include "metrics.h"

#include <stdlib.h>
#include <string.h>

#include <chrono>
#include <stdexcept>
#include <thread>

#include "../codec/json_codec.h"
#include "gale/executor.h"
#include "replica.h"

namespace gale {

GpuIngest::GpuIngest(int device, int lanes, int poll_us)
    : device_(device), poll_us_(poll_us), shift_chunk_(kCrcChunkBytes) {
  check_hip(hipSetDevice(device_), "ingest: hipSetDevice");
  std::vector<uint32_t> t(kafka::kCrcDeviceTableWords);
  kafka::crc32c_device_tables(t.data());
  check_hip(hipMalloc(reinterpret_cast<void**>(&d_tables_), t.size() * 4), "ingest: tables");
  check_hip(hipMemcpy(d_tables_, t.data(), t.size() * 4, hipMemcpyHostToDevice),
            "ingest: tables H2D");
  for (int i = 0; i < std::max(1, lanes); ++i) {
    auto L = std::make_unique<Lane>();
    check_hip(hipStreamCreateWithFlags(&L->stream, hipStreamNonBlocking), "ingest: stream");
    check_hip(hipEventCreateWithFlags(&L->done, hipEventDisableTiming), "ingest: event");
    lanes_.push_back(std::move(L));
  }
  if (const char* e = getenv("GALE_INGEST_DEV_TIMING")) dev_every_ = std::max(0, atoi(e));
  if (const char* e = getenv("GALE_INGEST_PLAN_SEPARATE")) plan_separate_ = atoi(e) != 0;
  if (dev_every_ > 0)
    for (auto& L : lanes_)
      for (hipEvent_t& ev : L->tev) check_hip(hipEventCreate(&ev), "ingest: timing event");
}

GpuIngest::~GpuIngest() {
  hipSetDevice(device_);
  for (auto& L : lanes_) {
    if (L->stream) hipStreamSynchronize(L->stream);
    if (L->h_io) hipHostFree(L->h_io);
    if (L->d_io) hipFree(L->d_io);
    if (L->d_counts) hipFree(L->d_counts);
    if (L->done) hipEventDestroy(L->done);
    for (hipEvent_t ev : L->tev)
      if (ev) hipEventDestroy(ev);
    if (L->stream) hipStreamDestroy(L->stream);
  }
  if (d_tables_) hipFree(d_tables_);
}

void GpuIngest::grow(Lane& L, size_t io_bytes, size_t tiles) {
  check_hip(hipSetDevice(device_), "ingest: hipSetDevice");
  auto up = [](size_t want, size_t have) {
    return (std::max(want, have * 2) + 4095) & ~(size_t)4095;
  };
  if (io_bytes > L.io_cap) {
    if (L.h_io) hipHostFree(L.h_io);
    if (L.d_io) hipFree(L.d_io);
    L.io_cap = up(io_bytes, L.io_cap);
    check_hip(hipMalloc(reinterpret_cast<void**>(&L.d_io), L.io_cap), "ingest: d_io");
    check_hip(hipHostMalloc(reinterpret_cast<void**>(&L.h_io), L.io_cap, hipHostMallocMapped),
              "ingest: h_io");
    void* dp = nullptr;
    check_hip(hipHostGetDevicePointer(&dp, L.h_io, 0), "ingest: h_io device pointer");
    if (dp != L.h_io) throw std::runtime_error("ingest: mapped plan buffer has another address");
  }
  if (tiles * sizeof(int) > L.counts_cap) {
    if (L.d_counts) hipFree(L.d_counts);
    L.counts_cap = up(tiles * sizeof(int), L.counts_cap);
    check_hip(hipMalloc(reinterpret_cast<void**>(&L.d_counts), L.counts_cap), "ingest: counts");
  }
}

void GpuIngest::wait(Lane& L) {
  if (poll_us_ <= 0) {
    check_hip(hipEventSynchronize(L.done), "ingest: hipEventSynchronize");
    return;
  }
  for (;;) {
    const hipError_t e = hipEventQuery(L.done);
    if (e == hipSuccess) return;
    if (e != hipErrorNotReady) check_hip(e, "ingest: hipEventQuery");
    std::this_thread::sleep_for(std::chrono::microseconds(poll_us_));
  }
}

void GpuIngest::mark(Lane& L, const Stamps& ts, int k) {
  if (ts.timed) check_hip(hipEventRecord(L.tev[k], L.stream), "ingest: timing event");
}

void GpuIngest::begin(Lane& L, Stamps& ts, const kafka::Fetched& f, uint8_t* dev,
                      const Transfer& t) {
  hipStream_t st = L.stream;
  ts.plan = mono_ns();
  ts.timed = dev_every_ > 0 && L.nrun++ % dev_every_ == 0;
  mark(L, ts, 0);
  if (t.tab_bytes) memcpy(t.hpl, t.tab, t.tab_bytes);
  const bool has_plan = t.plan_bytes > 0;
  if (t.in_chunk && has_plan) {
    check_hip(hipMemcpyAsync(dev + t.lo, f.buf.get() + t.lo, t.plan_off + t.plan_bytes - t.lo,
                             hipMemcpyHostToDevice, st),
              "ingest: H2D text + plan");
  } else {
    check_hip(hipMemcpyAsync(dev + t.lo, f.buf.get() + t.lo, t.len, hipMemcpyHostToDevice, st),
              "ingest: H2D text");
    if (has_plan)
      check_hip(hipMemcpyAsync(L.d_io, L.h_io, t.plan_bytes, hipMemcpyHostToDevice, st),
                "ingest: H2D plan");
  }
  plan_in_chunk_ += t.in_chunk && has_plan;
  mark(L, ts, 1);
  text_bytes_ += (int64_t)t.text_bytes;
  link_bytes_ += (int64_t)t.link_bytes;
}

int64_t GpuIngest::end(Lane& L, const Stamps& ts, bool parsed) {
  mark(L, ts, 3);
  check_hip(hipEventRecord(L.done, L.stream), "ingest: event");
  const int64_t t_wait = mono_ns();
  wait(L);
  const int64_t t_post = mono_ns();
  ++runs_;
  prep_ns_ += t_wait - ts.start;
  plan_ns_ += ts.plan - ts.start;
  wait_ns_ += t_post - t_wait;
  if (ts.timed) {
    float ms[3] = {0.f, 0.f, 0.f};
    for (int k = 0; k < (parsed ? 3 : 2); ++k)
      check_hip(hipEventElapsedTime(&ms[k], L.tev[k], L.tev[k + 1]), "ingest: event time");
    ++dev_runs_;
    dev_copy_ns_ += (int64_t)(ms[0] * 1e6);
    dev_count_ns_ += (int64_t)(ms[1] * 1e6);
    dev_parse_ns_ += (int64_t)(ms[2] * 1e6);
    dev_wait_ns_ += t_post - t_wait;
  }
  return t_post;
}

void GpuIngest::join_batch_crcs(const kafka::Fetched& f,
                                const std::vector<std::pair<size_t, size_t>>& batch_chunks,
                                const uint32_t* crc, IngestIO& io) {
  for (size_t b = 0; b < batch_chunks.size(); ++b) {
    const kafka::BatchSpan& bs = f.batches[b];
    uint32_t raw = 0;
    for (size_t k = 0; k < batch_chunks[b].second; ++k) {
      const uint32_t c = crc[batch_chunks[b].first + k];
      raw = k == 0 ? c : shift_chunk_(raw) ^ c;
    }
    const uint64_t len = bs.len - (size_t)kafka::kBatchAttrOffset;
    const uint32_t got = raw ^ kafka::crc32c_shift(0xffffffffu, len) ^ 0xffffffffu;
    kafka::Reader cr(f.buf.get() + bs.off + kafka::kBatchCrcOffset, 4);
    io.batch_ok[b] = got == cr.u32();
  }
}

void GpuIngest::run_b64(int lane, const kafka::Fetched& f, uint8_t* dev, size_t dev_cap,
                        bool check_crcs, int H, int W, int C, IngestIO& io, float* arena,
                        size_t arena_bytes) {
  Lane& L = *lanes_[(size_t)lane % lanes_.size()];
  std::lock_guard<std::mutex> lk(L.mu);
  Stamps ts;
  ts.start = mono_ns();
  const size_t nrec_all = f.records.size();
  io.cnt_off.assign(nrec_all, -1);
  io.batch_ok.assign(f.batches.size(), 1);
  io.img.assign(nrec_all, nullptr);
  std::vector<std::pair<int64_t, int64_t>> batches;
  for (const kafka::BatchSpan& b : f.batches) batches.emplace_back((int64_t)b.off, (int64_t)b.len);
  std::vector<B64PlanRecord> recs(nrec_all);
  for (size_t i = 0; i < nrec_all; ++i) {
    const kafka::RecordRef& rr = f.records[i];
    B64PlanRecord& r = recs[i];
    r.status = io.status[i];
    r.images = io.images[i];
    r.value_off = rr.value_off;
    r.value_len = rr.value_len;
    r.arr_off = io.arr_off[i];
  }
  B64IngestPlan plan;
  plan_b64_ingest(batches, kafka::kBatchAttrOffset, check_crcs, recs, io.b64_offs, H, W, C,
                  arena ? arena_bytes : 0, f.size, plan);
  const size_t nc = plan.chunks.size(), ni = plan.imgs.size();
  if (nc == 0 && plan.ok_records == 0) return;
  grow(L, plan.plan_bytes + plan.result_bytes + 16, 1);
  Transfer t;
  t.lo = plan.c_lo;
  t.len = t.text_bytes = t.link_bytes = plan.c_len;
  t.plan_off = plan.plan_off;
  t.plan_bytes = plan.plan_bytes;
  t.in_chunk = !plan_separate_ && t.plan_off + plan.plan_bytes <= dev_cap;
  t.hpl = t.in_chunk ? f.buf.get() + t.plan_off : L.h_io;
  const uint8_t* dpl = t.in_chunk ? dev + t.plan_off : L.d_io;
  if (nc) memcpy(t.hpl + plan.o_chunks, plan.chunks.data(), nc * sizeof(CrcChunk));
  if (ni) memcpy(t.hpl + plan.o_imgs, plan.imgs.data(), ni * sizeof(B64Image));
  uint8_t* res = L.h_io + plan.plan_bytes;
  int* wg_bad = reinterpret_cast<int*>(res + plan.o_bad);
  begin(L, ts, f, dev, t);
  check_hip(ingest_crc_b64(dev, reinterpret_cast<const CrcChunk*>(dpl + plan.o_chunks), (int)nc,
                           d_tables_, reinterpret_cast<uint32_t*>(res + plan.o_crc), (int)ni,
                           reinterpret_cast<const B64Image*>(dpl + plan.o_imgs), H, W, C, arena,
                           wg_bad, L.stream, &input_prep_),
            "ingest: crc32c + b64 decode");
  mark(L, ts, 2);
  const int64_t t_post = end(L, ts, false);
  join_batch_crcs(f, plan.batch_chunks, reinterpret_cast<const uint32_t*>(res + plan.o_crc), io);
  const int64_t per = (int64_t)H * W * C;
  const int cpi = plan.chunks_per_image;
  for (size_t i = 0; i < nrec_all; ++i) {
    if (plan.img0[i] < 0) continue;
    const int* w = wg_bad + (size_t)plan.img0[i] * cpi;
    int v = 0;
    for (int64_t g = 0; g < (int64_t)io.images[i] * cpi; ++g) v = std::max(v, w[g]);
    if (v == 2) io.status[i] = codec::BAD_NUMBER;
    else io.img[i] = arena + (int64_t)plan.slot0[i] * per;
  }
  post_ns_ += mono_ns() - t_post;
}

void GpuIngest::run(int lane, const kafka::Fetched& f, uint8_t* dev, size_t dev_cap,
                    bool check_crcs, int H, int W, int C, IngestIO& io, float* arena,
                    size_t arena_bytes) {
  Lane& L = *lanes_[(size_t)lane % lanes_.size()];
  std::lock_guard<std::mutex> lk(L.mu);
  Stamps ts;
  ts.start = mono_ns();
  const size_t nrec_all = f.records.size();
  io.images.assign(nrec_all, 0);
  io.cnt_off.assign(nrec_all, -1);
  io.batch_ok.assign(f.batches.size(), 1);
  io.img.assign(nrec_all, nullptr);
  L.batches.clear();
  for (const kafka::BatchSpan& b : f.batches)
    L.batches.emplace_back((int64_t)b.off, (int64_t)b.len);
  L.recs.resize(nrec_all);
  for (size_t i = 0; i < nrec_all; ++i) {
    const kafka::RecordRef& rr = f.records[i];
    JsonPlanRecord& r = L.recs[i];
    r.status = io.status[i];
    r.value_off = rr.value_off;
    r.value_len = rr.value_len;
    r.arr_off = io.arr_off[i];
    r.arr_len = io.arr_len[i];
  }
  const JsonIngestPlan& p = L.plan;
  plan_json_ingest(L.batches, kafka::kBatchAttrOffset, check_crcs, L.recs, H, W, C,
                   arena ? arena_bytes : 0, f.size, dev_cap, f.tap_result, plan_separate_, L.plan);
  if (p.empty()) return;
  const size_t nc = p.nc(), nr = p.nr(), np = p.np();
  grow(L, p.io_bytes + 16, (size_t)p.ntiles + (size_t)p.ngroups + 1);
  uint8_t* hpl = p.plan_in_chunk ? f.buf.get() + p.plan_off : L.h_io;
  uint8_t* dpl = p.plan_in_chunk ? dev + p.plan_off : L.d_io;
  fill_json_ingest(p, L.recs, hpl);
  const JsonRecord* hr = reinterpret_cast<const JsonRecord*>(hpl + p.o_recs);
  const JsonRecord* hp = reinterpret_cast<const JsonRecord*>(hpl + p.o_precs);
  Transfer t;
  t.lo = p.c_lo;
  t.len = p.c_len;
  t.plan_off = p.plan_off;
  t.plan_bytes = p.o_gsum;
  t.in_chunk = p.plan_in_chunk;
  t.hpl = hpl;
  if (p.packed) {
    t.tab = f.buf.get() + p.tab_off;
    t.tab_bytes = p.ng * 2 * sizeof(uint32_t);
  }
  t.text_bytes = p.span;
  t.link_bytes = p.link;
  begin(L, ts, f, dev, t);
  uint32_t* d_crc = reinterpret_cast<uint32_t*>(L.h_io + p.o_crc);
  int* d_gsum = reinterpret_cast<int*>(L.h_io + p.o_gsum);
  int* d_gbad = reinterpret_cast<int*>(L.h_io + p.o_gbad);
  int* d_pbad = reinterpret_cast<int*>(L.h_io + p.o_pbad);
  int* d_cnt = p.cnt_base >= 0 ? reinterpret_cast<int*>(dev + p.cnt_base) : L.d_counts;
  check_hip(ingest_crc_count(dev, reinterpret_cast<const CrcChunk*>(dpl + p.o_chunks), (int)nc,
                             d_tables_, d_crc, (int)nr, p.ngroups,
                             reinterpret_cast<JsonRecord*>(dpl + p.o_recs),
                             reinterpret_cast<const int2*>(dpl + p.o_groups), d_cnt, d_gsum,
                             d_gbad, L.stream, p.packed ? dev + p.c_lo : nullptr,
                             p.packed ? reinterpret_cast<const uint32_t*>(dpl) : nullptr,
                             p.packed ? dev : nullptr),
            "ingest: crc32c + count");
  mark(L, ts, 2);
  if (np > 0)
    check_hip(json_parse_instances((int)np, p.ptiles,
                                   reinterpret_cast<JsonRecord*>(dpl + p.o_precs),
                                   reinterpret_cast<const int*>(dpl + p.o_ptr), dev, H, W, C,
                                   L.d_counts, arena, L.stream, false, nullptr,
                                   nullptr, d_pbad, &input_prep_),
              "ingest: parse");
  const int64_t t_post = end(L, ts, true);
  join_batch_crcs(f, p.batch_chunks, d_crc, io);
  size_t k = 0;
  for (size_t j = 0; j < nr; ++j) {
    const size_t i = (size_t)p.rec_of[j];
    const bool parsed = k < np && (size_t)p.pjs[k] == j;
    const JsonRecord* pr = parsed ? &hp[k++] : nullptr;
    const int64_t g1 = j + 1 < nr ? hr[j + 1].grp0 : p.ngroups;
    int64_t tok = 0;
    int bad = 0;
    for (int64_t g = hr[j].grp0; g < g1; ++g) {
      tok += d_gsum[g];
      bad |= d_gbad[g];
    }
    if (bad != 0) {
      io.status[i] = codec::BAD_NUMBER;
    } else if (tok == 0) {
      io.status[i] = codec::EMPTY;
    } else if (tok % p.per != 0) {
      io.status[i] = codec::BAD_SHAPE;
    } else {
      io.images[i] = (int32_t)(tok / p.per);
      if (p.cnt_base >= 0) io.cnt_off[i] = p.cnt_off(hr[j]);
      if (pr) {
        const int nt = json_tile_count(pr->off, pr->len);
        int v = 0;
        for (int t0 = 0; t0 < nt; ++t0) v = std::max(v, d_pbad[pr->tile0 + t0]);
        const int32_t verdict = device_verdict_status(v);
        if (verdict != codec::OK) io.status[i] = verdict;
        else io.img[i] = arena + (int64_t)pr->slot * p.per;
      }
    }
  }
  post_ns_ += mono_ns() - t_post;
}

}
```

### csrc/runtime/gpu_ingest.h

```cpp
#pragma once
#include <hip/hip_runtime.h>

#include <atomic>
#include <memory>
#include <mutex>
#include <utility>
#include <vector>

#include "gale/kernels.h"
#include "ingest.h"
#include "ingest_plan.h"

namespace gale {

class GpuIngest : public Ingest {
 public:
  GpuIngest(int device, int lanes, int poll_us);
  ~GpuIngest() override;
  int device() const override { return device_; }
  void run(int lane, const kafka::Fetched& f, uint8_t* dev, size_t dev_cap, bool check_crcs,
           int H, int W, int C, IngestIO& io, float* arena = nullptr,
           size_t arena_bytes = 0) override;
  void run_b64(int lane, const kafka::Fetched& f, uint8_t* dev, size_t dev_cap, bool check_crcs,
               int H, int W, int C, IngestIO& io, float* arena = nullptr,
               size_t arena_bytes = 0) override;
  void link_bytes(int64_t& text, int64_t& link) const override {
    text = text_bytes_.load();
    link = link_bytes_.load();
  }
  void set_input_prep(const InputPrep& p) { input_prep_ = p; }
  Timing timing() const override {
    Timing t;
    t.runs = runs_.load();
    t.prep_ns = prep_ns_.load();
    t.plan_ns = plan_ns_.load();
    t.wait_ns = wait_ns_.load();
    t.post_ns = post_ns_.load();
    t.dev_runs = dev_runs_.load();
    t.dev_copy_ns = dev_copy_ns_.load();
    t.dev_count_ns = dev_count_ns_.load();
    t.dev_parse_ns = dev_parse_ns_.load();
    t.dev_wait_ns = dev_wait_ns_.load();
    t.plan_in_chunk = plan_in_chunk_.load();
    return t;
  }

 private:
  struct Lane {
    std::mutex mu;
    hipStream_t stream = nullptr;
    hipEvent_t done = nullptr;
    uint8_t* h_io = nullptr;
    uint8_t* d_io = nullptr;
    size_t io_cap = 0;
    int* d_counts = nullptr;
    size_t counts_cap = 0;
    hipEvent_t tev[4] = {nullptr, nullptr, nullptr, nullptr};
    int64_t nrun = 0;
    std::vector<std::pair<int64_t, int64_t>> batches;
    std::vector<JsonPlanRecord> recs;
    JsonIngestPlan plan;
  };
  struct Transfer {
    size_t lo = 0, len = 0;
    size_t plan_off = 0, plan_bytes = 0;
    bool in_chunk = false;
    uint8_t* hpl = nullptr;
    const uint8_t* tab = nullptr;
    size_t tab_bytes = 0;
    size_t text_bytes = 0, link_bytes = 0;
  };
  struct Stamps {
    int64_t start = 0, plan = 0;
    bool timed = false;
  };
  void grow(Lane& L, size_t io_bytes, size_t tiles);
  void wait(Lane& L);
  void begin(Lane& L, Stamps& ts, const kafka::Fetched& f, uint8_t* dev, const Transfer& t);
  void mark(Lane& L, const Stamps& ts, int k);
  int64_t end(Lane& L, const Stamps& ts, bool parsed);
  void join_batch_crcs(const kafka::Fetched& f,
                       const std::vector<std::pair<size_t, size_t>>& batch_chunks,
                       const uint32_t* crc, IngestIO& io);
  int device_, poll_us_;
  InputPrep input_prep_;
  std::atomic<int64_t> text_bytes_{0}, link_bytes_{0};
  std::atomic<int64_t> runs_{0}, prep_ns_{0}, plan_ns_{0}, wait_ns_{0}, post_ns_{0};
  std::atomic<int64_t> dev_runs_{0}, dev_copy_ns_{0}, dev_count_ns_{0}, dev_parse_ns_{0},
      dev_wait_ns_{0};
  int dev_every_ = 0;
  bool plan_separate_ = false;
  std::atomic<int64_t> plan_in_chunk_{0};
  uint32_t* d_tables_ = nullptr;
  std::vector<std::unique_ptr<Lane>> lanes_;
  kafka::CrcShift shift_chunk_;
};

}
```

### csrc/runtime/gpu_replica.cpp

```cpp
#include <stdio.h>
#include <stdlib.h>
#include <string.h>

#include <algorithm>
#include <chrono>
#include <thread>
#include <vector>
#include <stdexcept>

#include "../codec/json_codec.h"
#include "b64_source.h"
#include "metrics.h"
#include "replica.h"

namespace gale {

namespace {

template <typename T>
T* meta_at(uint8_t* base, size_t off) {
  return reinterpret_cast<T*>(base + off);
}

}
// ... 124 lines not shown
    return d_images ? StepError{resize_crop_aa_dev(images, d_images, r.aa, src, dst, st),
                                "resize_crop_aa_dev"}
                    : StepError{resize_crop_aa(images, r.aa, src, dst, st), "resize_crop_aa"};
  return d_images ? StepError{resize_crop_dev(images, d_images, r.plain, src, dst, st),
                              "resize_crop_dev"}
                  : StepError{resize_crop(images, r.plain, src, dst, st), "resize_crop"};
}

std::string GpuReplica::name() const { return "gpu" + std::to_string(exec_->device()); }

void* GpuReplica::mapped_alloc(size_t bytes, const char* what) {
  void* h = nullptr;
  check_hip(hipHostMalloc(&h, bytes, hipHostMallocMapped), what);
  void* d = nullptr;
  check_hip(hipHostGetDevicePointer(&d, h, 0), what);
  if (d != h) {
    hipHostFree(h);
    throw std::runtime_error(std::string("GpuReplica: mapped ") + what +
                             " buffer has another device address");
  }
  return h;
}

void GpuReplica::ensure_host(Slot& s, size_t bytes) {
  if (bytes <= s.h_cap) return;
  const size_t cap = (std::max(bytes, s.h_cap * 2) + 4095) & ~(size_t)4095;
  if (s.h_bytes) {
    check_hip(hipEventSynchronize(s.done), "hipEventSynchronize");
    hipHostFree(s.h_bytes);
  }
  check_hip(hipHostMalloc(reinterpret_cast<void**>(&s.h_bytes), cap), "hipHostMalloc(bytes)");
  s.h_cap = cap;
}

void GpuReplica::drop_steps(Slot& s) {
  for (hipGraphExec_t& g : s.step) {
    if (g) hipGraphExecDestroy(g);
    g = nullptr;
  }
}

void GpuReplica::ensure_tiles(Slot& s, int ntiles) {
  if (ntiles <= s.meta.tiles_cap) return;
  const MetaLayout m(exec_->max_batch(), std::max(ntiles, s.meta.tiles_cap * 2));
  if (s.h_meta) {
    check_hip(hipEventSynchronize(s.done), "hipEventSynchronize");
    drop_steps(s);
    hipHostFree(s.h_meta);
    hipFree(s.d_meta);
    hipFree(s.d_tiles);
    s.h_meta = s.d_meta = nullptr;
    s.d_tiles = nullptr;
    s.meta = MetaLayout();
  }
  s.h_meta = static_cast<uint8_t*>(mapped_alloc(m.total, "meta"));
  memset(s.h_meta, 0, MetaLayout::kHeaderBytes);
  check_hip(hipMalloc(reinterpret_cast<void**>(&s.d_meta), m.total), "hipMalloc(meta)");
  check_hip(hipMalloc(reinterpret_cast<void**>(&s.d_tiles), sizeof(int) * (size_t)m.tiles_cap),
            "hipMalloc(tiles)");
  s.meta = m;
}

void GpuReplica::ensure_device(Slot& s, size_t bytes) {
  if (bytes <= s.d_cap) return;
  const size_t cap = (std::max(bytes, s.d_cap * 2) + 4095) & ~(size_t)4095;
  if (s.d_bytes) {
    check_hip(hipEventSynchronize(s.done), "hipEventSynchronize");
    drop_steps(s);
    hipFree(s.d_bytes);
  }
  check_hip(hipMalloc(reinterpret_cast<void**>(&s.d_bytes), cap), "hipMalloc(bytes)");
  s.d_cap = cap;
}

void GpuReplica::describe(const Batch& b, Slot& s) {
  s.recs.assign(b.recs.size(), BatchPlanRecord());
  s.b64_offs.clear();
  for (size_t i = 0; i < b.recs.size(); ++i) {
    const InRecord& r = b.recs[i];
    BatchPlanRecord& p = s.recs[i];
    p.arr_len = r.arr_len;
    p.images = r.images;
    p.pinned = r.pinned;
    p.resident = resident(r);
    p.preparsed = preparsed(r);
    if (p.resident) {
      p.dev_text = reinterpret_cast<uint64_t>(r.dev_value + r.arr_off);
      p.dev_counts = reinterpret_cast<uint64_t>(r.dev_counts);
      p.dev_image = reinterpret_cast<uint64_t>(r.dev_image);
    } else {
      p.buf = reinterpret_cast<uint64_t>(r.buf.get());
      p.arr_off = (r.value + r.arr_off) - r.buf.get();
    }
    if (b64_ && !p.preparsed) {
      p.b64_first = (int32_t)s.b64_offs.size();
      p.b64_n = codec::b64_image_offsets_bytes(r.value + r.arr_off, (size_t)r.arr_len,
                                               pixels_.bytes(recH_, recW_, C_), s.b64_scan)
                    ? (int32_t)s.b64_scan.size()
                    : -1;
      s.b64_offs.insert(s.b64_offs.end(), s.b64_scan.begin(), s.b64_scan.end());
    }
  }
}

void GpuReplica::submit(Batch& b) {
  const int slot = next_slot_;
  next_slot_ = (next_slot_ + 1) % (int)slots_.size();
  b.slot = slot;
  Slot& s = slots_[(size_t)slot];
  if (!(ptr_input_ && table_step(b, s, slot))) {
    BatchPlan& p = s.plan;
    describe(b, s);
    plan_batch(s.recs, exec_->max_batch(), (int64_t)H_ * W_ * C_, form_, ptr_input_, b64_, p);
    resident_ += p.resident;
    host_ += (int64_t)b.recs.size() - p.resident;
    preparsed_ += p.npre;
    b.images = p.img;
    ensure_device(s, p.dev_total + 16);
    if (p.staged_bytes) ensure_host(s, p.staged_bytes + 16);
    ensure_tiles(s, p.ntiles);
    stage_text(b, s);
    fill_batch(p, s.recs, s.b64_offs, s.meta, reinterpret_cast<uint64_t>(s.d_bytes),
               reinterpret_cast<uint64_t>(exec_->input(slot)), s.h_meta);
    launch_step(b, s, slot);
    if (d_resize_) resized_ += p.img;
  }
  check_hip(hipEventRecord(s.done, stream_), "hipEventRecord");
  s.t_submit_ns = mono_ns();
}

void GpuReplica::stage_text(const Batch& b, Slot& s) {
  const BatchPlan& p = s.plan;
  for (const BatchPlan::Span& x : p.spans)
    check_hip(hipMemcpyAsync(s.d_bytes + x.dev, reinterpret_cast<const uint8_t*>(x.buf) + x.lo,
                             x.len, hipMemcpyHostToDevice, stream_),
              "H2D span");
  if (!p.staged_bytes) return;
  for (const BatchPlan::Staged& g : p.staged) {
    const InRecord& r = b.recs[(size_t)g.rec];
    memcpy(s.h_bytes + g.host, r.value + r.arr_off, g.len);
  }
  check_hip(hipMemcpyAsync(s.d_bytes + p.staged_dev, s.h_bytes, p.staged_bytes,
                           hipMemcpyHostToDevice, stream_),
            "H2D staged");
}

void GpuReplica::launch_step(Batch& b, Slot& s, int slot) {
  const BatchPlan& p = s.plan;
  const bool captured =
      form_ == StepForm::Captured || (form_ == StepForm::Kernels && !step_direct_);
  hipGraphExec_t g = captured ? step_for(s, slot, p.count_pass) : nullptr;
  if (form_ == StepForm::Kernels) {
    const MetaRange m = s.meta.used(p);
    check_hip(hipMemcpyAsync(s.d_meta + m.off, s.h_meta + m.off, m.bytes, hipMemcpyHostToDevice,
                             stream_),
              "H2D step metadata");
  }
  if (g) {
    check_hip(hipGraphLaunch(g, stream_), "hipGraphLaunch(step)");
  } else {
    const StepError e = emit_step(s, slot, stream_, step_desc(), p.count_pass,
                                  form_ == StepForm::OpByOp || p.nrec > 0);
    check_hip(e.code, e.what);
  }
  if (form_ == StepForm::OpByOp) {
    if (use_graph_ && exec_->graph_pays()) ++fwd_graph_batches_;
  } else {
    b.step_graph = true;
// ... 201 lines not shown
```

### csrc/runtime/ingest.h

```cpp
#pragma once
#include <stdint.h>

#include <vector>

#include "../kafka/client.h"

namespace gale {

struct IngestIO {
  std::vector<int32_t> status;
  std::vector<int64_t> arr_off, arr_len;
  std::vector<int32_t> images;
  std::vector<int64_t> cnt_off;
  std::vector<char> batch_ok;
  std::vector<const float*> img;
  std::vector<uint32_t> b64_offs;
};

class Ingest {
 public:
  virtual ~Ingest() = default;
  virtual int device() const = 0;
  virtual void run(int lane, const kafka::Fetched& f, uint8_t* dev, size_t dev_cap,
                   bool check_crcs, int H, int W, int C, IngestIO& io, float* arena = nullptr,
                   size_t arena_bytes = 0) = 0;
  virtual void run_b64(int lane, const kafka::Fetched& f, uint8_t* dev, size_t dev_cap,
                       bool check_crcs, int H, int W, int C, IngestIO& io,
                       float* arena = nullptr, size_t arena_bytes = 0) {
    (void)lane, (void)f, (void)dev, (void)dev_cap, (void)check_crcs, (void)H, (void)W, (void)C;
    (void)arena, (void)arena_bytes;
    io.cnt_off.assign(f.records.size(), -1);
    io.batch_ok.assign(f.batches.size(), 1);
    io.img.assign(f.records.size(), nullptr);
  }
  virtual void link_bytes(int64_t& text, int64_t& link) const { text = link = 0; }
  struct Timing {
    int64_t runs = 0, prep_ns = 0, wait_ns = 0, post_ns = 0;
    int64_t plan_ns = 0;
    int64_t dev_runs = 0, dev_copy_ns = 0, dev_count_ns = 0, dev_parse_ns = 0, dev_wait_ns = 0;
    int64_t plan_in_chunk = 0;
  };
  virtual Timing timing() const { return Timing(); }
};

}
```

### csrc/runtime/ingest_plan.cpp

```cpp
#include "ingest_plan.h"

#include <string.h>

#include <algorithm>
#include <stdexcept>

#include "../codec/text_pack.h"

namespace gale {

namespace {

size_t align16(size_t n) { return (n + 15) & ~(size_t)15; }
size_t align256(size_t n) { return (n + 255) & ~(size_t)255; }

void plan_batches(const std::vector<std::pair<int64_t, int64_t>>& batches, int64_t attr_off,
                  bool check_crcs, size_t fetch_size, std::vector<CrcChunk>& chunks,
                  std::vector<std::pair<size_t, size_t>>& batch_chunks, size_t& lo, size_t& hi) {
  for (const auto& b : batches) {
    if (b.first < 0 || b.second < 0 || (uint64_t)b.first + (uint64_t)b.second > fetch_size)
      throw std::invalid_argument("ingest plan: batch outside the fetch");
    lo = std::min(lo, (size_t)b.first);
    hi = std::max(hi, (size_t)(b.first + b.second));
    if (!check_crcs) continue;
    const size_t first = chunks.size();
    const size_t n = append_crc_windows(b.first + attr_off, b.first + b.second, chunks);
    batch_chunks.emplace_back(first, n);
  }
}

int64_t image_elements(int H, int W, int C) {
  if (H <= 0 || W <= 0 || C <= 0) throw std::invalid_argument("ingest plan: bad image shape");
  const int64_t per = (int64_t)H * W * C;
  if (per > (1 << 30)) throw std::invalid_argument("ingest plan: image too large");
  return per;
}

}

size_t append_crc_windows(int64_t rs, int64_t re, std::vector<CrcChunk>& chunks) {
  const int64_t len = re - rs;
  if (len <= 0) return 0;
  const int64_t n = (len + kCrcChunkBytes - 1) / kCrcChunkBytes;
  for (int64_t k = 0; k < n; ++k) {
    CrcChunk c;
    c.end = re - (int64_t)kCrcChunkBytes * (n - 1 - k);
    c.len = k == 0 ? (int32_t)(len - (int64_t)kCrcChunkBytes * (n - 1)) : kCrcChunkBytes;
    c.pad_ = 0;
    chunks.push_back(c);
  }
  return (size_t)n;
}

void plan_json_ingest(const std::vector<std::pair<int64_t, int64_t>>& batches, int64_t attr_off,
                      bool check_crcs, const std::vector<JsonPlanRecord>& recs, int H, int W,
                      int C, size_t arena_bytes, size_t fetch_size, size_t dev_cap,
                      int64_t tap_result, bool plan_separate, JsonIngestPlan& out) {
  {
    JsonIngestPlan fresh;
    fresh.chunks.swap(out.chunks);
    fresh.batch_chunks.swap(out.batch_chunks);
    fresh.rec_of.swap(out.rec_of);
    fresh.pjs.swap(out.pjs);
    fresh.chunks.clear();
    fresh.batch_chunks.clear();
    fresh.rec_of.clear();
    fresh.pjs.clear();
    out = std::move(fresh);
  }
  const int64_t per = out.per = image_elements(H, W, C);
  size_t lo = fetch_size, hi = 0;
  plan_batches(batches, attr_off, check_crcs, fetch_size, out.chunks, out.batch_chunks, lo, hi);
  for (size_t i = 0; i < recs.size(); ++i) {
    const JsonPlanRecord& r = recs[i];
    if (r.status != 0) continue;
    if (r.value_off < 0 || r.value_len < 0 || r.arr_off < 0 || r.arr_len < 0 ||
        r.arr_len > 0x7fffffffll ||
        (uint64_t)r.value_off + (uint64_t)r.value_len > fetch_size)
      throw std::invalid_argument("ingest plan: record outside the fetch");
    if ((uint64_t)r.arr_off + (uint64_t)r.arr_len > (uint64_t)r.value_len)
      throw std::invalid_argument("ingest plan: array outside its record");
    out.rec_of.push_back((int)i);
    const int nt = json_tile_count(r.value_off + r.arr_off, (int32_t)r.arr_len);
    out.ntiles += nt;
    out.ngroups += (nt + kGroupTiles - 1) / kGroupTiles;
    lo = std::min(lo, (size_t)r.value_off);
    hi = std::max(hi, (size_t)(r.value_off + r.value_len));
  }
  if (out.empty()) return;
  const size_t nc = out.nc(), nr = out.nr();
  out.packed = tap_result >= 0;
  if (out.packed) {
    lo = 0;
    hi = fetch_size;
  }
  lo &= ~(size_t)15;
  const size_t span = hi - lo;
  out.lo = lo;
  out.span = span;
  out.ng = out.packed ? codec::pack_groups(span) : 0;
  out.link = out.packed ? (size_t)tap_result : span;
  out.c_lo = out.packed ? codec::pack_offset(span) : lo;
  out.c_len = out.link;
  out.tab_off = out.packed ? codec::tab_offset(span) : 0;
  out.used = out.c_lo + out.c_len;
  if (out.used > dev_cap) throw std::invalid_argument("ingest plan: the copy ends past the mirror");
  const size_t ncnt = (size_t)out.ntiles + (size_t)out.ngroups;
  if (out.ntiles > 0) {
    const size_t cb = align256(ncnt * sizeof(int));
    if (dev_cap > cb + 256 && ((dev_cap - cb) & ~(size_t)255) >= align256(out.used + 64))
      out.cnt_base = (int64_t)((dev_cap - cb) & ~(size_t)255);
  }
  if (arena_bytes > 0 && out.cnt_base >= 0) {
    const int64_t S = 2 * per;
    for (size_t j = 0; j < nr; ++j) {
      const JsonPlanRecord& r = recs[(size_t)out.rec_of[j]];
      const int64_t off = r.value_off + r.arr_off;
      const int64_t slot = (off + S - 1) / S, cap = r.arr_len / S;
      if (cap <= 0 || (slot + cap) * per * (int64_t)sizeof(float) > (int64_t)arena_bytes) continue;
      out.pjs.push_back((int)j);
      out.ptiles += json_tile_count(off, (int32_t)r.arr_len);
    }
  }
  const size_t np = out.np(), ngroups = (size_t)out.ngroups, ptiles = (size_t)out.ptiles;
  out.o_chunks = align16(out.ng * 2 * sizeof(uint32_t));
  out.o_groups = out.o_chunks + align16(nc * sizeof(CrcChunk));
  out.o_recs = out.o_groups + align16(ngroups * sizeof(int2));
  out.o_precs = out.o_recs + nr * sizeof(JsonRecord);
  out.o_ptr = out.o_precs + np * sizeof(JsonRecord);
  out.o_gsum = out.o_ptr + align16(ptiles * sizeof(int));
  out.o_crc = out.o_gsum + align16(ngroups * 4);
  out.o_gbad = out.o_crc + align16(nc * 4);
  out.o_pbad = out.o_gbad + align16(ngroups * 4);
  out.io_bytes = out.o_pbad + align16(ptiles * 4);
  out.plan_off = align256(std::max(fetch_size, out.used));
  const size_t plan_lim = out.cnt_base >= 0 ? (size_t)out.cnt_base : dev_cap;
  const bool on_tab = out.packed && out.plan_off < out.tab_off + out.ng * 2 * sizeof(uint32_t) &&
                      out.tab_off < out.plan_off + out.o_gsum;
  out.plan_in_chunk = !plan_separate && !on_tab && out.plan_off + out.o_gsum <= plan_lim;
}

void fill_json_ingest(const JsonIngestPlan& p, const std::vector<JsonPlanRecord>& recs,
                      uint8_t* dst) {
  const size_t nc = p.nc(), nr = p.nr(), np = p.np();
  if (nc) memcpy(dst + p.o_chunks, p.chunks.data(), nc * sizeof(CrcChunk));
  int2* hg = reinterpret_cast<int2*>(dst + p.o_groups);
  JsonRecord* hr = reinterpret_cast<JsonRecord*>(dst + p.o_recs);
  int tile = 0, grp = 0;
  for (size_t j = 0; j < nr; ++j) {
    const JsonPlanRecord& r = recs[(size_t)p.rec_of[j]];
    JsonRecord& jr = hr[j];
    jr.off = r.value_off + r.arr_off;
    jr.len = (int32_t)r.arr_len;
    jr.slot = 0;
    jr.images = 0;
    jr.status = 0;
    jr.tile0 = tile;
    jr.has_cnt = 0;
    jr.cnt_off = 0;
    jr.grp0 = grp;
    const int nt = json_tile_count(jr.off, jr.len);
    for (int t0 = 0; t0 < nt; t0 += kGroupTiles) {
      hg[grp].x = (int)j;
      hg[grp].y = t0;
      ++grp;
    }
    tile += nt;
  }
  JsonRecord* hp = reinterpret_cast<JsonRecord*>(dst + p.o_precs);
  int* hpt = reinterpret_cast<int*>(dst + p.o_ptr);
  const int64_t S = 2 * p.per;
  int pt = 0;
  for (size_t k = 0; k < np; ++k) {
    const JsonRecord& jr = hr[p.pjs[k]];
    JsonRecord& pr = hp[k];
    pr = jr;
    pr.slot = (int32_t)((jr.off + S - 1) / S);
    pr.images = -1;
    pr.status = 0;
    pr.tile0 = pt;
    pr.has_cnt = 1;
    pr.cnt_off = p.cnt_off(jr);
    pr.grp0 = 0;
    const int nt = json_tile_count(pr.off, pr.len);
    for (int t = 0; t < nt; ++t) hpt[pt + t] = (int)k;
    pt += nt;
  }
}

void plan_b64_ingest(const std::vector<std::pair<int64_t, int64_t>>& batches, int64_t attr_off,
                     bool check_crcs, const std::vector<B64PlanRecord>& recs,
                     const std::vector<uint32_t>& offs, int H, int W, int C, size_t arena_bytes,
                     size_t fetch_size, B64IngestPlan& out) {
  out = B64IngestPlan();
  const int64_t per = image_elements(H, W, C);
  const int64_t L = 4 * ((per + 2) / 3);
  out.chunks_per_image = (int)((L + kB64ChunkChars - 1) / kB64ChunkChars);
  size_t lo = fetch_size, hi = 0;
  plan_batches(batches, attr_off, check_crcs, fetch_size, out.chunks, out.batch_chunks, lo, hi);
  out.slot0.assign(recs.size(), -1);
  out.img0.assign(recs.size(), -1);
  size_t next_off = 0;
  int64_t next_slot = 0;
  bool cut = false;
  for (size_t i = 0; i < recs.size(); ++i) {
    const B64PlanRecord& r = recs[i];
    if (r.status != 0) continue;
    if (r.images <= 0 || r.value_off < 0 || r.value_len < 0 || r.arr_off < 0 ||
        r.arr_off > r.value_len || (uint64_t)r.value_off + (uint64_t)r.value_len > fetch_size)
      throw std::invalid_argument("b64 ingest plan: record outside the fetch");
    if (offs.size() - next_off < (size_t)r.images)
      throw std::invalid_argument("b64 ingest plan: fewer string offsets than images");
    ++out.ok_records;
    lo = std::min(lo, (size_t)r.value_off);
    hi = std::max(hi, (size_t)(r.value_off + r.value_len));
    const uint32_t* ro = offs.data() + next_off;
    next_off += (size_t)r.images;
    for (int32_t k = 0; k < r.images; ++k)
      if (r.arr_off + (int64_t)ro[k] + L > r.value_len)
        throw std::invalid_argument("b64 ingest plan: string outside its record");
    if (!cut && ((uint64_t)(next_slot + r.images) * (uint64_t)per * sizeof(float) > arena_bytes ||
                 next_slot + r.images > 0x7fffffffll))
      cut = true;
    if (cut) continue;
    out.slot0[i] = (int32_t)next_slot;
    out.img0[i] = (int32_t)out.imgs.size();
    for (int32_t k = 0; k < r.images; ++k) {
      B64Image d;
      d.off = r.value_off + r.arr_off + (int64_t)ro[k];
      d.slot = (int32_t)(next_slot + k);
      d.rec = (int32_t)i;
      out.imgs.push_back(d);
    }
    next_slot += r.images;
  }
  if (hi < lo) lo = hi = 0;
  out.lo = lo;
  out.hi = hi;
  out.c_lo = lo & ~(size_t)15;
  out.c_len = hi - out.c_lo;
  out.plan_off = align256(fetch_size);
  const size_t nc = out.chunks.size(), ni = out.imgs.size();
  out.o_chunks = 0;
  out.o_imgs = out.o_chunks + align16(nc * sizeof(CrcChunk));
  out.plan_bytes = out.o_imgs + align16(ni * sizeof(B64Image));
  out.o_crc = 0;
  out.o_bad = out.o_crc + align16(nc * sizeof(uint32_t));
  out.result_bytes = out.o_bad + align16(ni * (size_t)out.chunks_per_image * sizeof(int32_t));
}

}
```

### csrc/runtime/ingest_plan.h

```cpp
#pragma once
#include <stddef.h>
#include <stdint.h>

#include <utility>
#include <vector>

#include "gale/kernels.h"

namespace gale {

size_t append_crc_windows(int64_t rs, int64_t re, std::vector<CrcChunk>& chunks);


struct JsonPlanRecord {
  int32_t status = 0;
  int64_t value_off = 0;
  int64_t value_len = 0;
  int64_t arr_off = 0;
  int64_t arr_len = 0;
};

struct JsonIngestPlan {
  std::vector<CrcChunk> chunks;
  std::vector<std::pair<size_t, size_t>> batch_chunks;
  std::vector<int> rec_of;
  std::vector<int> pjs;
  int ntiles = 0, ngroups = 0;
  int ptiles = 0;
  bool packed = false;
  size_t lo = 0, span = 0, link = 0, ng = 0;
  size_t c_lo = 0, c_len = 0;
  size_t tab_off = 0;
  size_t used = 0;
  int64_t cnt_base = -1;
  size_t o_chunks = 0, o_groups = 0, o_recs = 0, o_precs = 0, o_ptr = 0;
  size_t o_gsum = 0;
  size_t o_crc = 0, o_gbad = 0, o_pbad = 0, io_bytes = 0;
  size_t plan_off = 0;
  bool plan_in_chunk = false;
  int64_t per = 0;

  size_t nc() const { return chunks.size(); }
  size_t nr() const { return rec_of.size(); }
  size_t np() const { return pjs.size(); }
  bool empty() const { return chunks.empty() && rec_of.empty(); }
  int64_t cnt_off(const JsonRecord& r) const {
    return cnt_base + ((int64_t)r.tile0 + r.grp0) * (int64_t)sizeof(int);
  }
};

void plan_json_ingest(const std::vector<std::pair<int64_t, int64_t>>& batches, int64_t attr_off,
                      bool check_crcs, const std::vector<JsonPlanRecord>& recs, int H, int W,
                      int C, size_t arena_bytes, size_t fetch_size, size_t dev_cap,
                      int64_t tap_result, bool plan_separate, JsonIngestPlan& out);

void fill_json_ingest(const JsonIngestPlan& plan, const std::vector<JsonPlanRecord>& recs,
                      uint8_t* dst);


struct B64PlanRecord {
  int32_t status = 0;
  int32_t images = 0;
  int64_t value_off = 0;
  int64_t value_len = 0;
  int64_t arr_off = 0;
};

struct B64IngestPlan {
  std::vector<CrcChunk> chunks;
  std::vector<std::pair<size_t, size_t>> batch_chunks;
  std::vector<B64Image> imgs;
  std::vector<int32_t> slot0;
  std::vector<int32_t> img0;
  int chunks_per_image = 1;
  size_t lo = 0, hi = 0;
  size_t c_lo = 0, c_len = 0;
  size_t plan_off = 0;
  size_t ok_records = 0;
  size_t o_chunks = 0, o_imgs = 0, plan_bytes = 0;
  size_t o_crc = 0, o_bad = 0, result_bytes = 0;
};

void plan_b64_ingest(const std::vector<std::pair<int64_t, int64_t>>& batches, int64_t attr_off,
                     bool check_crcs, const std::vector<B64PlanRecord>& recs,
                     const std::vector<uint32_t>& offs, int H, int W, int C, size_t arena_bytes,
                     size_t fetch_size, B64IngestPlan& out);

}
```

### csrc/runtime/replica.h

```cpp
#pragma once
#include <stdint.h>

#include <atomic>
#include <memory>
#include <optional>
#include <string>
#include <vector>

#include "../codec/json_codec.h"
#include "../codec/pixel_source.h"
#include "batch_plan.h"
#include "gale/executor.h"
#include "gale/kernels.h"
#include "resize_plan.h"

namespace gale {

inline int32_t device_verdict_status(int v) {
  return v == 1 || v == 3 ? codec::BAD_SHAPE : v == 2 ? codec::BAD_NUMBER : codec::OK;
}

struct InRecord;
struct SplitRecord;

struct InRecord {
  std::shared_ptr<uint8_t> buf;
  const uint8_t* value = nullptr;
  int32_t len = -1;
  const uint8_t* key = nullptr;
  int32_t key_len = -1;
  int32_t partition = -1;
  int64_t offset = -1;
  int64_t timestamp_ms = -1;
  int64_t t_fetch_ns = 0;
  int64_t t_take_ns = 0, t_done_ns = 0;
  int64_t t_ready_ns = 0;
  int64_t arr_off = 0, arr_len = 0;
  int32_t images = 0;
  int32_t status = 0;
  int32_t source = 0;
  bool pinned = false;
  const uint8_t* dev_value = nullptr;
  int32_t dev_locality = -1;
  const uint8_t* dev_counts = nullptr;
  const float* dev_image = nullptr;
  const float* dev_arena = nullptr;
  std::shared_ptr<SplitRecord> split;
  int32_t split_index = -1;
};

struct Batch {
  std::vector<InRecord> recs;
  int images = 0;
  int slot = 0;
  const float* probs = nullptr;
  const uint8_t* pred_text = nullptr;
  const int32_t* pred_idx = nullptr;
  std::vector<int32_t> dev_status;
  int64_t t_take_ns = 0, t_submit_ns = 0, t_done_ns = 0;
  bool step_graph = false;
};

class Replica {
 public:
  virtual ~Replica() = default;
  virtual std::string name() const = 0;
  virtual int max_images() const = 0;
  virtual int depth() const = 0;
  virtual void submit(Batch& b) = 0;
  virtual void wait(Batch& b) = 0;
  virtual int device() const { return -1; }
  virtual int locality() const { return device(); }
  virtual void recover() {}
  virtual int64_t resident_records() const { return 0; }
  virtual int64_t host_records() const { return 0; }
  virtual int64_t graph_step_batches() const { return 0; }
  virtual int64_t graph_forward_batches() const { return 0; }
  virtual int64_t preparsed_records() const { return 0; }
  virtual int64_t table_batches() const { return 0; }
  virtual int64_t resized_images() const { return 0; }
};

class StubReplica : public Replica {
 public:
  StubReplica(int H, int W, int C, int classes, int max_images, int delay_us, bool compute = true,
              int locality = -1);
  std::string name() const override { return "stub"; }
  int locality() const override { return locality_; }
  int max_images() const override { return max_images_; }
  int depth() const override { return 1; }
  void submit(Batch& b) override;
  void wait(Batch& b) override;
  void set_input_prep(const InputPrep& p) { prep_ = p; }
  void set_input_b64(bool on, const PixelSource& src = PixelSource()) {
    b64_ = on, pixels_ = src;
  }
  void set_input_resize(const InputResize& r);
  int64_t resized_images() const override { return resized_; }

 private:
  InputPrep prep_;
  bool b64_ = false;
  PixelSource pixels_;
  std::optional<InputResize> resize_;
  std::vector<float> src_;
  std::atomic<int64_t> resized_{0};
  int H_, W_, C_, classes_, max_images_, delay_us_;
  bool compute_;
  int locality_ = -1;
  std::vector<float> x_, probs_;
};

class GpuReplica : public Replica {
 public:
  GpuReplica(std::shared_ptr<Executor> exec, int H, int W, int C, int classes, bool use_graph,
             int wait_poll_us = 0, bool gpu_encode = false, int locality = -1,
             bool step_graph = true, bool high_priority = false, bool step_direct = false,
             int top_k = 0);
  ~GpuReplica() override;
  std::string name() const override;
  int max_images() const override { return exec_->max_batch(); }
  int depth() const override { return exec_->slots(); }
  int device() const override { return exec_->device(); }
  int locality() const override { return locality_ >= 0 ? locality_ : exec_->device(); }
  void submit(Batch& b) override;
  void wait(Batch& b) override;
  void recover() override;
  int64_t resident_records() const override { return resident_; }
  int64_t host_records() const override { return host_; }
  int64_t graph_step_batches() const override { return step_batches_; }
  int64_t graph_forward_batches() const override { return fwd_graph_batches_; }
  int64_t preparsed_records() const override { return preparsed_; }
  int64_t table_batches() const override { return table_batches_; }
  bool step_graph() const { return step_graph_; }
  void set_input_prep(const InputPrep& p) { prep_ = p; }
  void set_input_b64(bool on, const PixelSource& src = PixelSource()) {
    b64_ = on, pixels_ = src;
  }
  void set_input_resize(const InputResize& r);
  int64_t resized_images() const override { return resized_; }

 private:
  struct Slot {
    float* d_src = nullptr;
    uint8_t* h_bytes = nullptr;
    uint8_t* d_bytes = nullptr;
    size_t h_cap = 0, d_cap = 0;
    uint8_t* h_meta = nullptr;
    uint8_t* d_meta = nullptr;
    MetaLayout meta;
    hipGraphExec_t step[2] = {nullptr, nullptr};
    int* d_tiles = nullptr;
    float* h_out = nullptr;
    uint8_t* h_text = nullptr;
    int32_t* h_idx = nullptr;
    int* d_status = nullptr;
    int* h_status = nullptr;
    std::vector<BatchPlanRecord> recs;
    std::vector<uint32_t> b64_offs, b64_scan;
    BatchPlan plan;
    hipEvent_t done = nullptr;
    int64_t t_submit_ns = 0;
  };
  struct StepDesc;
  struct StepError;
  void ensure_host(Slot& s, size_t bytes);
  void ensure_device(Slot& s, size_t bytes);
  void ensure_tiles(Slot& s, int ntiles);
  void drop_steps(Slot& s);
  bool resident(const InRecord& r) const {
    return r.dev_value != nullptr && r.dev_locality == my_loc_;
  }
  bool preparsed(const InRecord& r) const { return ptr_input_ && resident(r) && r.dev_image; }
  void describe(const Batch& b, Slot& s);
  bool table_step(Batch& b, Slot& s, int slot);
  void stage_text(const Batch& b, Slot& s);
  void launch_step(Batch& b, Slot& s, int slot);
  hipGraphExec_t step_for(Slot& s, int slot, bool count_pass);
  StepDesc step_desc() const;
  StepError emit_step(Slot& s, int slot, hipStream_t st, const StepDesc& d, bool count_pass,
                      bool parse);
  static StepError launch_resize(const BoundResize& r, int images, const int* d_images,
                                 const float* src, float* dst, hipStream_t st);
  static void* mapped_alloc(size_t bytes, const char* what);
  std::shared_ptr<Executor> exec_;
  InputPrep prep_;
  bool b64_ = false;
  PixelSource pixels_;
  uint8_t* d_resize_ = nullptr;
  BoundResize resize_;
  std::atomic<int64_t> resized_{0};
  int H_, W_, C_, classes_;
  int recH_, recW_;
  bool use_graph_;
  int wait_poll_us_ = 0;
  bool gpu_encode_ = false;
  int top_k_ = 0;
  hipStream_t stream_ = nullptr;
  std::vector<Slot> slots_;
  int next_slot_ = 0;
  int locality_ = -1;
  int my_loc_ = -1;
  std::atomic<int64_t> resident_{0}, host_{0};
  std::atomic<int64_t> step_batches_{0}, fwd_graph_batches_{0};
  bool step_graph_ = false;
  bool step_direct_ = false;
  StepForm form_ = StepForm::OpByOp;
  bool ptr_input_ = false;
  std::atomic<int64_t> preparsed_{0};
  std::atomic<int64_t> table_batches_{0};
  int64_t expect_ns_ = 0;
// ... 4 lines not shown
```

Measured before the change: 2.072 million.

## Fuse CRC, token count and parse for small JSON records into one kernel

Adds a fused ingest path that handles small JSON records (aligned extent within a cap) in a single kernel doing CRC, token counting and number parsing straight into the arena. The host plan now sorts such records into a separate fused list with its own table and result region. The count/parse tile code is factored into shared helpers. This is meant to remove the separate count pass and the second launch for small records, at the cost of more planner complexity and a new dev_text_gone state that affects residency.

```diff
diff --git a/csrc/bindings/host_bindings.cpp b/csrc/bindings/host_bindings.cpp
--- a/csrc/bindings/host_bindings.cpp
+++ b/csrc/bindings/host_bindings.cpp
@@ -486,7 +486,7 @@
         [](std::vector<std::pair<int64_t, int64_t>> batches,
            std::vector<std::tuple<int, int64_t, int64_t, int64_t, int64_t>> recs, int H, int W,
            int C, size_t arena_bytes, size_t fetch_size, size_t dev_cap, int64_t tap_result,
-           bool plan_separate, bool check_crcs) {
+           bool plan_separate, bool check_crcs, int64_t fused_cap) {
           std::vector<JsonPlanRecord> rs(recs.size());
           for (size_t i = 0; i < recs.size(); ++i) {
             rs[i].status = std::get<0>(recs[i]);
@@ -497,7 +497,7 @@
           }
           JsonIngestPlan p;
           plan_json_ingest(batches, kafka::kBatchAttrOffset, check_crcs, rs, H, W, C, arena_bytes,
-                           fetch_size, dev_cap, tap_result, plan_separate, p);
+                           fetch_size, dev_cap, tap_result, plan_separate, p, fused_cap);
           std::string plan(p.o_gsum, '\0');
           if (!p.empty()) fill_json_ingest(p, rs, reinterpret_cast<uint8_t*>(&plan[0]));
           py::list windows;
@@ -507,6 +507,11 @@
           out["batch_windows"] = py::cast(p.batch_chunks);
           out["rec_of"] = py::cast(p.rec_of);
           out["pjs"] = py::cast(p.pjs);
+          out["frec_of"] = py::cast(p.frec_of);
+          out["nf"] = p.nf();
+          out["fused_tiles_max"] = p.fused_tiles_max;
+          out["o_frecs"] = p.o_frecs;
+          out["o_fres"] = p.o_fres;
           out["nc"] = p.nc();
           out["nr"] = p.nr();
           out["np"] = p.np();
@@ -542,7 +547,7 @@
         py::arg("batches"), py::arg("recs"), py::arg("H"), py::arg("W"), py::arg("C"),
         py::arg("arena_bytes"), py::arg("fetch_size"), py::arg("dev_cap"),
         py::arg("tap_result") = (int64_t)-1, py::arg("plan_separate") = false,
-        py::arg("check_crcs") = true,
+        py::arg("check_crcs") = true, py::arg("fused_cap") = (int64_t)0,
         "The host plan of a JSON fetch's device ingest, laid out and filled "
         "(csrc/runtime/ingest_plan.h)");
   m.def("plan_batch",
diff --git a/csrc/bindings/module.cpp b/csrc/bindings/module.cpp
--- a/csrc/bindings/module.cpp
+++ b/csrc/bindings/module.cpp
@@ -385,6 +385,44 @@
         "groups: int32 (record, first tile) pairs, GROUP_TILES tiles each; counts: per record "
         "tile0 + grp0 -> [tile counts][group sums]; gsum: one int per group");
   m.attr("GROUP_TILES") = gale::kGroupTiles;
+  m.def("ingest_crc_fused",
+        [](uintptr_t bytes, uintptr_t chunks, int nchunks, uintptr_t tables, uintptr_t crc_out,
+           int nfused, uintptr_t frecs, int H, int W, int C, uintptr_t arena, uintptr_t fres,
+           int nw, uintptr_t stream, int ngroups, uintptr_t recs, uintptr_t groups,
+           uintptr_t counts, uintptr_t gsum, uintptr_t gbad, uintptr_t packed, uintptr_t tab,
+           uintptr_t text_out, std::optional<std::vector<float>> a,
+           std::optional<std::vector<float>> b, bool nchw) {
+          const auto prep = prep_from("ingest_crc_fused", a, b, nchw);
+          gale::check_hip(
+              gale::ingest_crc_fused(reinterpret_cast<const uint8_t*>(bytes),
+                                     reinterpret_cast<const gale::CrcChunk*>(chunks), nchunks,
+                                     reinterpret_cast<const uint32_t*>(tables),
+                                     reinterpret_cast<uint32_t*>(crc_out), nfused,
+                                     reinterpret_cast<const gale::FusedRecord*>(frecs), H, W, C,
+                                     reinterpret_cast<float*>(arena),
+                                     reinterpret_cast<int*>(fres), nw, ngroups,
+                                     reinterpret_cast<gale::JsonRecord*>(recs),
+                                     reinterpret_cast<const int2*>(groups),
+                                     reinterpret_cast<int*>(counts),
+                                     reinterpret_cast<int*>(gsum), reinterpret_cast<int*>(gbad),
+                                     reinterpret_cast<hipStream_t>(stream),
+                                     reinterpret_cast<const uint8_t*>(packed),
+                                     reinterpret_cast<const uint32_t*>(tab),
+                                     reinterpret_cast<uint8_t*>(text_out),
+                                     prep ? &*prep : nullptr),
+              "ingest_crc_fused");
+        },
+        py::arg("bytes"), py::arg("chunks"), py::arg("nchunks"), py::arg("tables"),
+        py::arg("crc_out"), py::arg("nfused"), py::arg("frecs"), py::arg("H"), py::arg("W"),
+        py::arg("C"), py::arg("arena"), py::arg("fres"), py::arg("nw"), py::arg("stream"),
+        py::arg("ngroups") = 0, py::arg("recs") = 0, py::arg("groups") = 0,
+        py::arg("counts") = 0, py::arg("gsum") = 0, py::arg("gbad") = 0, py::arg("packed") = 0,
+        py::arg("tab") = 0, py::arg("text_out") = 0, py::arg("a") = py::none(),
+        py::arg("b") = py::none(), py::arg("nchw") = false);
+  m.def("json_fused_waves", &gale::json_fused_waves);
+  m.def("json_aligned_extent", &gale::json_aligned_extent);
+  m.attr("FUSED_RECORD_BYTES") = gale::kFusedRecordBytes;
+  m.attr("FUSED_RECORD_BYTES_EACH") = (int)sizeof(gale::FusedRecord);
   m.def("ingest_crc_b64",
         [](uintptr_t bytes, uintptr_t chunks, int nchunks, uintptr_t tables, uintptr_t crc_out,
            int images, uintptr_t imgs, int H, int W, int C, uintptr_t arena, uintptr_t wg_bad,
diff --git a/csrc/include/gale/kernels.h b/csrc/include/gale/kernels.h
--- a/csrc/include/gale/kernels.h
+++ b/csrc/include/gale/kernels.h
@@ -258,6 +258,27 @@
                             int* gbad, hipStream_t stream, const uint8_t* packed = nullptr,
                             const uint32_t* tab = nullptr, uint8_t* text_out = nullptr);
 
+constexpr int kFusedRecordBytes = 40 * 1024;
+constexpr int kFusedTiles = kFusedRecordBytes / kJsonTileBytes;
+struct FusedRecord {
+  int64_t off;
+  int32_t len;
+  int32_t slot;
+};
+static_assert(sizeof(FusedRecord) == 16, "FusedRecord layout (host <-> device tables)");
+constexpr int kFusedResultWords = 3;
+inline int64_t json_aligned_extent(int64_t off, int64_t len) {
+  return ((off & 15) + len + 15) & ~(int64_t)15;
+}
+inline int json_fused_waves(int tiles) { return tiles <= 4 ? 4 : tiles <= 8 ? 8 : 16; }
+hipError_t ingest_crc_fused(const uint8_t* bytes, const CrcChunk* chunks, int nchunks,
+                            const uint32_t* tables, uint32_t* crc_out, int nfused,
+                            const FusedRecord* frecs, int H, int W, int C, float* arena,
+                            int* fres, int nw, int ngroups, JsonRecord* recs, const int2* groups,
+                            int* counts, int* gsum, int* gbad, hipStream_t stream,
+                            const uint8_t* packed = nullptr, const uint32_t* tab = nullptr,
+                            uint8_t* text_out = nullptr, const InputPrep* prep = nullptr);
+
 hipError_t ingest_crc_b64(const uint8_t* bytes, const CrcChunk* chunks, int nchunks,
                           const uint32_t* tables, uint32_t* crc_out, int images,
                           const B64Image* imgs, int H, int W, int C, float* arena, int* wg_bad,
diff --git a/csrc/kernels/json_parse.hip b/csrc/kernels/json_parse.hip
--- a/csrc/kernels/json_parse.hip
+++ b/csrc/kernels/json_parse.hip
@@ -102,6 +102,32 @@
 #pragma unroll
   for (int o = 32; o > 0; o >>= 1) v += __shfl_xor(v, o, 64);
   return v;
+}
+
+__device__ __forceinline__ int compact_token_starts(const uint32_t (&st)[kChunks], int x0,
+                                                    uint16_t* list) {
+  const int lane = threadIdx.x & 63;
+  int cnt = 0;
+#pragma unroll
+  for (int i = 0; i < kChunks; ++i) cnt += __builtin_popcount(st[i]);
+  int inc = cnt;
+#pragma unroll
+  for (int d = 1; d < 64; d <<= 1) {
+    const int u = __shfl_up(inc, d, 64);
+    if (lane >= d) inc += u;
+  }
+  const int ntok = __shfl(inc, 63, 64);
+  int li = inc - cnt;
+#pragma unroll
+  for (int i = 0; i < kChunks; ++i) {
+    uint32_t s = st[i];
+    while (s) {
+      const int j = __builtin_ctz(s);
+      s &= s - 1;
+      list[li++] = (uint16_t)(x0 + 16 * i + j);
+    }
+  }
+  return ntok;
 }
 
 __device__ __forceinline__ void wave_lds_sync() { asm volatile("s_waitcnt lgkmcnt(0)" ::: "memory"); }
@@ -569,16 +595,17 @@
   const JsonRecord r = recs[gr.x];
   const int nt = record_tiles(r);
   const int tl = gr.y + wave;
+  const bool mine = wave < kGroupTiles;
   int cnt = 0;
   bool bad = false;
-  if (tl < nt) {
+  if (mine && tl < nt) {
     cnt = PACKED ? tile_tokens_packed(r, tl, bytes, pt, &bad)
                  : tile_tokens(r, tl, bytes, &bad);
     if ((threadIdx.x & 63) == 0) counts[r.tile0 + (int)r.grp0 + tl] = cnt;
     if (bad && !gbad) atomicMax(&recs[gr.x].status, 2);
     bad = __ballot(bad) != 0;
   }
-  if ((threadIdx.x & 63) == 0) {
+  if (mine && (threadIdx.x & 63) == 0) {
     lds8[wave] = cnt;
     lds8[kGroupTiles + wave] = bad ? 1 : 0;
   }
@@ -674,6 +701,109 @@
   const int g = (int)blockIdx.x - crc_blocks;
   if (g >= ngroups) return;
   count_group<PACKED>(recs, groups, g, bytes, pt, counts, gsum, gbad, reinterpret_cast<int*>(T));
+}
+
+template <bool PREP>
+__device__ __forceinline__ int parse_one_token(const uint8_t* text, int x, uint32_t m0,
+                                               uint32_t m1, const Text& tx, int beg, int end,
+                                               int idx, int expected, const Dims& dims,
+                                               int per_image, int W, int C, float* dst,
+                                               const InputPrep& prep) {
+  const int pos = x + tx.lbase;
+  int bad = 0;
+  float val;
+  int len = 0;
+  bool ok;
+  if (parse_window(text, x, m0, m1, pos & 15, &val)) {
+    ok = true;
+    len = -1;
+  } else {
+    ok = false;
+    val = parse_number(tx, pos, end, &ok, &len);
+  }
+  int kn = 0;
+  if (PREP) {
+    const uint32_t px = udiv_rcp((uint32_t)idx, dims.C, dims.rC);
+    const uint32_t i0 = (uint32_t)idx - px * dims.C;
+    uint32_t sidx = (uint32_t)idx, ch = i0;
+    if (prep.nchw) {
+      const uint32_t row = udiv_rcp(px, dims.W, dims.rW);
+      const uint32_t i1 = px - row * dims.W;
+      const uint32_t img = udiv_rcp(row, dims.H, dims.rH);
+      ch = row - img * dims.H;
+      kn = i0 ? 0 : i1 ? 1 : ch ? 2 : 3;
+      sidx = img * (uint32_t)per_image + (i1 * (uint32_t)W + i0) * (uint32_t)C + ch;
+    }
+    if (idx < expected) {
+      const float a = ch == 0 ? prep.a[0] : ch == 1 ? prep.a[1] : ch == 2 ? prep.a[2] : prep.a[3];
+      const float b = ch == 0 ? prep.b[0] : ch == 1 ? prep.b[1] : ch == 2 ? prep.b[2] : prep.b[3];
+      dst[sidx] = __builtin_fmaf(val, a, b);
+    }
+  }
+  if (!ok) {
+    bad = 2;
+  } else {
+    const int k = idx <= 0 ? 0 : (PREP && prep.nchw) ? kn : wraps((uint32_t)idx, dims);
+    const bool fast_gap = idx > 0 && pos - 8 >= tx.lo && pos - (2 * k + 2) >= beg &&
+                          gap_window(text, x, k);
+    if (!fast_gap && !gap_ok(tx, beg, pos, (uint32_t)idx, k)) {
+      bad = 3;
+    } else if (idx == expected - 1) {
+      if (len < 0) parse_number(tx, pos, end, &ok, &len);
+      if (!tail_ok(tx, pos + len, end)) bad = 3;
+    }
+  }
+  if (!PREP && idx < expected) dst[idx] = val;
+  return bad;
+}
+
+__device__ __forceinline__ Dims nesting_dims(int H, int W, int C, bool nchw) {
+  const int d0 = nchw ? W : C, d1 = nchw ? H : W, d2 = nchw ? C : H;
+  Dims dims;
+  dims.C = (uint32_t)d0; dims.W = (uint32_t)d1; dims.H = (uint32_t)d2;
+  dims.rC = 1.0 / d0; dims.rW = 1.0 / d1; dims.rH = 1.0 / d2;
+  return dims;
+}
+
+template <bool PREP>
+__device__ __forceinline__ int parse_tile_tokens(const uint8_t* text, uint16_t* tok,
+                                                 uint32_t* cmk, const Text& tx, int beg, int end,
+                                                 int t0, int base, int expected, int H, int W,
+                                                 int C, float* dst, const InputPrep& prep,
+                                                 int* ntok_out) {
+  const int lane = threadIdx.x & 63;
+  const int per_image = H * W * C;
+  const int o = t0 + kLaneBytes * lane;
+  uint4 v[kChunks];
+#pragma unroll
+  for (int i = 0; i < kChunks; ++i)
+    v[i] = (o + 16 * i < end) ? *reinterpret_cast<const uint4*>(text + (o + 16 * i - tx.lbase))
+                              : make_uint4(0, 0, 0, 0);
+  const bool pd = (o - 1 < beg) || is_delim(text[o - 1 - tx.lbase]);
+  uint32_t st[kChunks], cm[kChunks];
+  bool bad_ignored;
+  token_starts(v, o, beg, end, pd, st, cm, &bad_ignored);
+#pragma unroll
+  for (int i = 0; i < kChunks; ++i) cmk[kChunks * lane + i] = cm[i];
+  if (lane == 63) {
+    const int p = t0 + kTile;
+    const uint4 h = p < end ? *reinterpret_cast<const uint4*>(text + (p - tx.lbase))
+                            : make_uint4(0, 0, 0, 0);
+    cmk[kTile / 16] = chunk_masks(classify16(h.x, h.y, h.z, h.w), p, beg, end);
+  }
+  const int ntok = compact_token_starts(st, o - tx.lbase, tok);
+  wave_lds_sync();
+
+  const Dims dims = nesting_dims(H, W, C, PREP && prep.nchw);
+  int bad = 0;
+  for (int j = lane; j < ntok; j += 64) {
+    const int x = tok[j];
+    const int ci = (x + tx.lbase - t0) >> 4;
+    bad = max(bad, parse_one_token<PREP>(text, x, cmk[ci], cmk[ci + 1], tx, beg, end, base + j,
+                                         expected, dims, per_image, W, C, dst, prep));
+  }
+  *ntok_out = ntok;
+  return bad;
 }
 
 template <bool PREP>
@@ -735,102 +865,10 @@
   const int base = wave_sum_i(part);
   wave_lds_sync();
 
-  const int o = t0 + kLaneBytes * lane;
-  uint4 v[kChunks];
-#pragma unroll
-  for (int i = 0; i < kChunks; ++i)
-    v[i] = (o + 16 * i < end) ? *reinterpret_cast<const uint4*>(text + (o + 16 * i - tx.lbase))
-                              : make_uint4(0, 0, 0, 0);
-  const bool pd = (o - 1 < beg) || is_delim(text[o - 1 - tx.lbase]);
-  uint32_t st[kChunks], cm[kChunks];
-  bool bad_ignored;
-  token_starts(v, o, beg, end, pd, st, cm, &bad_ignored);
-#pragma unroll
-  for (int i = 0; i < kChunks; ++i) cmk[kChunks * lane + i] = cm[i];
-  if (lane == 63) {
-    const int p = t0 + kTile;
-    const uint4 h = p < end ? *reinterpret_cast<const uint4*>(text + (p - tx.lbase))
-                            : make_uint4(0, 0, 0, 0);
-    cmk[kTile / 16] = chunk_masks(classify16(h.x, h.y, h.z, h.w), p, beg, end);
-  }
-  int cnt = 0;
-#pragma unroll
-  for (int i = 0; i < kChunks; ++i) cnt += __builtin_popcount(st[i]);
-  int inc = cnt;
-#pragma unroll
-  for (int d = 1; d < 64; d <<= 1) {
-    const int u = __shfl_up(inc, d, 64);
-    if (lane >= d) inc += u;
-  }
-  const int ntok = __shfl(inc, 63, 64);
-  int li = inc - cnt;
-#pragma unroll
-  for (int i = 0; i < kChunks; ++i) {
-    uint32_t s = st[i];
-    while (s) {
-      const int j = __builtin_ctz(s);
-      s &= s - 1;
-      tok[li++] = (uint16_t)(o + 16 * i + j - tx.lbase);
-    }
-  }
-  wave_lds_sync();
-
-  const bool nchw = PREP && prep.nchw;
-  const int d0 = nchw ? W : C, d1 = nchw ? H : W, d2 = nchw ? C : H;
-  Dims dims;
-  dims.C = (uint32_t)d0; dims.W = (uint32_t)d1; dims.H = (uint32_t)d2;
-  dims.rC = 1.0 / d0; dims.rW = 1.0 / d1; dims.rH = 1.0 / d2;
   float* dst = out + (int64_t)r.slot * per_image;
-  int bad = 0;
-  for (int j = lane; j < ntok; j += 64) {
-    const int x = tok[j];
-    const int pos = x + tx.lbase;
-    const int idx = base + j;
-    float val;
-    int len = 0;
-    bool ok;
-    const int ci = (pos - t0) >> 4;
-    if (parse_window(text, x, cmk[ci], cmk[ci + 1], pos & 15, &val)) {
-      ok = true;
-      len = -1;
-    } else {
-      ok = false;
-      val = parse_number(tx, pos, end, &ok, &len);
-    }
-    int kn = 0;
-    if (PREP) {
-      const uint32_t px = udiv_rcp((uint32_t)idx, dims.C, dims.rC);
-      const uint32_t i0 = (uint32_t)idx - px * dims.C;
-      uint32_t sidx = (uint32_t)idx, ch = i0;
-      if (prep.nchw) {
-        const uint32_t row = udiv_rcp(px, dims.W, dims.rW);
-        const uint32_t i1 = px - row * dims.W;
-        const uint32_t img = udiv_rcp(row, dims.H, dims.rH);
-        ch = row - img * dims.H;
-        kn = i0 ? 0 : i1 ? 1 : ch ? 2 : 3;
-        sidx = img * (uint32_t)per_image + (i1 * (uint32_t)W + i0) * (uint32_t)C + ch;
-      }
-      if (idx < expected) {
-        const float a = ch == 0 ? prep.a[0] : ch == 1 ? prep.a[1] : ch == 2 ? prep.a[2] : prep.a[3];
-        const float b = ch == 0 ? prep.b[0] : ch == 1 ? prep.b[1] : ch == 2 ? prep.b[2] : prep.b[3];
-        dst[sidx] = __builtin_fmaf(val, a, b);
-      }
-    }
-    if (!ok) {
-      bad = max(bad, 2);
-    } else {
-      const int k = idx <= 0 ? 0 : (PREP && prep.nchw) ? kn : wraps((uint32_t)idx, dims);
-      const bool fast_gap = idx > 0 && pos - 8 >= tx.lo && pos - (2 * k + 2) >= beg &&
-                            gap_window(text, x, k);
-      if (!fast_gap && !gap_ok(tx, beg, pos, (uint32_t)idx, k)) {
-        bad = 3;
-      } else if (idx == expected - 1) {
-        if (len < 0) parse_number(tx, pos, end, &ok, &len);
-        if (!tail_ok(tx, pos + len, end)) bad = 3;
-      }
-    }
-    if (!PREP && idx < expected) dst[idx] = val;
-  }
+  int ntok;
+  int bad = parse_tile_tokens<PREP>(text, tok, cmk, tx, beg, end, t0, base, expected, H, W, C, dst,
+                                    prep, &ntok);
   if (last_tile && lane == 0 && base + ntok != expected) bad = max(bad, 1);
   if (tile_bad) {
 #pragma unroll
@@ -859,9 +897,231 @@
                         tile_bad, prep);
 }
 
-}
-
-
+
+constexpr int kFusedImage = kFusedRecordBytes + 16;
+constexpr int kFusedMasks = (kFusedRecordBytes / 16 + 1 + 3) / 4 * 4;
+constexpr int kFusedWords = 96;
+static_assert(kFusedTiles <= 32, "the prefix search covers 32 tiles");
+static_assert(kFusedRecordBytes < 65536, "token offsets into the record image are 16-bit");
+constexpr int kFusedLds =
+    kFusedImage + kFusedMasks * 4 + kFusedWords * 4 + kFusedTiles * kMaxTok * 2;
+static_assert(kFusedLds >= crc::kTableWords * 4, "the CRC tables fit the same LDS");
+
+template <bool PACKED>
+__device__ __forceinline__ int tile_tokens_lds(int64_t off, int len, int tl, const uint8_t* bytes,
+                                               const PackedText& pt, uint8_t* img, uint32_t* rcm,
+                                               uint16_t* list, bool* bad) {
+  const int lane = threadIdx.x & 63;
+  const int64_t abeg = off & ~(int64_t)15;
+  const uint8_t* rb = bytes + abeg;
+  const int beg = (int)(off - abeg), end = beg + len;
+  const int o = tl * kTile + kLaneBytes * lane;
+  uint4 v[kChunks];
+#pragma unroll
+  for (int i = 0; i < kChunks; ++i) {
+    if (o + 16 * i < end) {
+      v[i] = PACKED ? expand16(pt, abeg + o + 16 * i)
+                    : *reinterpret_cast<const uint4*>(rb + o + 16 * i);
+      *reinterpret_cast<uint4*>(img + o + 16 * i) = v[i];
+    } else {
+      v[i] = make_uint4(0, 0, 0, 0);
+    }
+  }
+  unsigned prevb = __shfl_up(v[kChunks - 1].w >> 24, 1, 64);
+  if (lane == 0 && o - 1 >= beg)
+    prevb = PACKED ? expand16(pt, abeg + o - 16).w >> 24 : (unsigned)rb[o - 1];
+  const bool pd = (o - 1 < beg) || is_delim(prevb);
+  uint32_t st[kChunks], cm[kChunks];
+  token_starts(v, o, beg, end, pd, st, cm, bad);
+#pragma unroll
+  for (int i = 0; i < kChunks; ++i) rcm[(o >> 4) + i] = cm[i];
+  return compact_token_starts(st, o, list);
+}
+
+template <bool PACKED, int NW, bool PREP>
+__device__ __forceinline__ void fused_record(const FusedRecord fr, const uint8_t* bytes,
+                                             const PackedText& pt, int H, int W, int C,
+                                             float* arena, int* res, const InputPrep& prep,
+                                             uint8_t* lds) {
+  const int lane = threadIdx.x & 63, wave = threadIdx.x >> 6;
+  const int64_t abeg = fr.off & ~(int64_t)15;
+  const int beg = (int)(fr.off - abeg), end = beg + fr.len;
+  const int aend = (end + 15) & ~15;
+  if (fr.len <= 0 || aend > kFusedRecordBytes) {
+    if (threadIdx.x == 0) {
+      res[0] = -1;
+      res[1] = 0;
+      res[2] = 0;
+    }
+    return;
+  }
+  const int nt = (end + kTile - 1) / kTile;
+  uint8_t* img = lds;
+  uint32_t* rcm = reinterpret_cast<uint32_t*>(lds + kFusedImage);
+  int* s_inc = reinterpret_cast<int*>(rcm + kFusedMasks);
+  int* s_bad = s_inc + 32;
+  int* s_ver = s_bad + 32;
+  uint16_t* tok = reinterpret_cast<uint16_t*>(s_inc + kFusedWords);
+
+  for (int tl = wave; tl < nt; tl += NW) {
+    bool bad;
+    const int cnt = tile_tokens_lds<PACKED>(fr.off, fr.len, tl, bytes, pt, img, rcm,
+                                            tok + tl * kMaxTok, &bad);
+    const bool wbad = __ballot(bad) != 0;
+    if (lane == 0) {
+      s_inc[tl] = cnt;
+      s_bad[tl] = wbad ? 1 : 0;
+    }
+  }
+  if (threadIdx.x == 0) rcm[nt * (kTile / 16)] = 0xFFFFu;
+  __syncthreads();
+
+  const int per_image = H * W * C;
+  const int mycnt = lane < nt ? s_inc[lane] : 0;
+  const bool anybad = __ballot(lane < nt && s_bad[lane] != 0) != 0;
+  int inc = mycnt;
+#pragma unroll
+  for (int d = 1; d < 64; d <<= 1) {
+    const int u = __shfl_up(inc, d, 64);
+    if (lane >= d) inc += u;
+  }
+  const int tot = __shfl(inc, 63, 64);
+  __syncthreads();
+  if (wave == 0 && lane < 32) s_inc[lane] = inc;
+  __syncthreads();
+  const int expected =
+      (tot % per_image == 0 && tot / per_image <= fr.len / (2 * per_image)) ? tot : 0;
+
+  Text tx;
+  tx.g = img;
+  tx.l = img;
+  tx.lbase = 0;
+  tx.lo = 0;
+  tx.hi = aend;
+  float* dst = arena + (int64_t)fr.slot * per_image;
+  const Dims dims = nesting_dims(H, W, C, PREP && prep.nchw);
+  int verdict = 0;
+  for (int g = (int)threadIdx.x; g < tot; g += 64 * NW) {
+    int t = 0;
+#pragma unroll
+    for (int sft = 16; sft > 0; sft >>= 1)
+      if (g >= s_inc[t + sft - 1]) t += sft;
+    const int x = tok[t * kMaxTok + (g - (t ? s_inc[t - 1] : 0))];
+    const int ci = x >> 4;
+    verdict = max(verdict, parse_one_token<PREP>(img, x, rcm[ci], rcm[ci + 1], tx, beg, end, g,
+                                                 expected, dims, per_image, W, C, dst, prep));
+  }
+  if (threadIdx.x == 0 && tot != expected) verdict = max(verdict, 1);
+
+#pragma unroll
+  for (int d = 32; d > 0; d >>= 1) verdict = max(verdict, __shfl_xor(verdict, d, 64));
+  if (lane == 0) s_ver[wave] = verdict;
+  __syncthreads();
+  if (threadIdx.x == 0) {
+    int v = 0;
+#pragma unroll
+    for (int w = 0; w < NW; ++w) v = max(v, s_ver[w]);
+    res[0] = tot;
+    res[1] = anybad ? 2 : 0;
+    res[2] = v;
+  }
+}
+
+template <bool PACKED, int NW, bool PREP>
+__global__ __launch_bounds__(64 * NW) void ingest_crc_fused_kernel(
+    uint8_t* bytes, PackedText pt, const CrcChunk* chunks, int nchunks, const uint32_t* tables,
+    uint32_t* crc_out, int crc_blocks, const FusedRecord* frecs, int nfused, int H, int W, int C,
+    float* arena, int* fres, JsonRecord* recs, const int2* groups, int ngroups, int* counts,
+    int* gsum, int* gbad, InputPrep prep) {
+  extern __shared__ __attribute__((aligned(16))) uint8_t fused_lds[];
+  if ((int)blockIdx.x < crc_blocks) {
+    uint32_t* T = reinterpret_cast<uint32_t*>(fused_lds);
+    crc::crc_stage_tables(tables, T);
+    if ((int)(threadIdx.x >> 6) >= crc::kCrcWaves) return;
+    if (PACKED)
+      crc_windows_packed(pt, chunks, nchunks, T, crc_out, blockIdx.x, crc_blocks);
+    else
+      crc::crc_windows(bytes, chunks, nchunks, T, crc_out, blockIdx.x, crc_blocks);
+    return;
+  }
+  const int k = (int)blockIdx.x - crc_blocks;
+  if (k < nfused) {
+    fused_record<PACKED, NW, PREP>(frecs[k], bytes, pt, H, W, C, arena,
+                                   fres + kFusedResultWords * k, prep, fused_lds);
+    return;
+  }
+  const int g = k - nfused;
+  if (g >= ngroups) return;
+  count_group<PACKED>(recs, groups, g, bytes, pt, counts, gsum, gbad,
+                      reinterpret_cast<int*>(fused_lds));
+}
+
+template <bool PACKED, int NW>
+hipError_t launch_fused(bool with_prep, int blocks, hipStream_t stream, uint8_t* bytes,
+                        PackedText pt, const CrcChunk* chunks, int nchunks,
+                        const uint32_t* tables, uint32_t* crc_out, int crc_blocks,
+                        const FusedRecord* frecs, int nfused, int H, int W, int C, float* arena,
+                        int* fres, JsonRecord* recs, const int2* groups, int ngroups, int* counts,
+                        int* gsum, int* gbad, const InputPrep& prep) {
+  if (with_prep)
+    hipLaunchKernelGGL((ingest_crc_fused_kernel<PACKED, NW, true>), dim3(blocks), dim3(64 * NW),
+                       kFusedLds, stream, bytes, pt, chunks, nchunks, tables, crc_out,
+                       crc_blocks, frecs, nfused, H, W, C, arena, fres, recs, groups, ngroups,
+                       counts, gsum, gbad, prep);
+  else
+    hipLaunchKernelGGL((ingest_crc_fused_kernel<PACKED, NW, false>), dim3(blocks), dim3(64 * NW),
+                       kFusedLds, stream, bytes, pt, chunks, nchunks, tables, crc_out,
+                       crc_blocks, frecs, nfused, H, W, C, arena, fres, recs, groups, ngroups,
+                       counts, gsum, gbad, prep);
+  return hipGetLastError();
+}
+
+}
+
+hipError_t ingest_crc_fused(const uint8_t* bytes, const CrcChunk* chunks, int nchunks,
+                            const uint32_t* tables, uint32_t* crc_out, int nfused,
+                            const FusedRecord* frecs, int H, int W, int C, float* arena,
+                            int* fres, int nw, int ngroups, JsonRecord* recs, const int2* groups,
+                            int* counts, int* gsum, int* gbad, hipStream_t stream,
+                            const uint8_t* packed, const uint32_t* tab, uint8_t* text_out,
+                            const InputPrep* prep) {
+  if (nfused < 0 || ngroups < 0 || nchunks < 0) return hipErrorInvalidValue;
+  if (nw != 4 && nw != 8 && nw != 16) return hipErrorInvalidValue;
+  if (nfused > 0 && (H <= 0 || W <= 0 || C <= 0 || !arena || !fres || !frecs))
+    return hipErrorInvalidValue;
+  const bool with_prep = prep && !prep->identity();
+  if (with_prep && nfused > 0) {
+    if ((int64_t)H * W * C >= (1 << 20)) return hipErrorInvalidValue;
+    if (C > 4)
+      for (int i = 1; i < 4; ++i)
+        if (prep->a[i] != prep->a[0] || prep->b[i] != prep->b[0]) return hipErrorInvalidValue;
+  }
+  int crc_blocks = (nchunks + crc::kCrcWaves - 1) / crc::kCrcWaves;
+  if (crc_blocks > 1024) crc_blocks = 1024;
+  const int blocks = crc_blocks + nfused + ngroups;
+  if (blocks == 0) return hipSuccess;
+  const bool is_packed = packed != nullptr;
+  if (is_packed && (!tab || (ngroups > 0 && !text_out) ||
+                    (reinterpret_cast<uintptr_t>(packed) & 7) ||
+                    (reinterpret_cast<uintptr_t>(text_out) & 15)))
+    return hipErrorInvalidValue;
+  uint8_t* b = is_packed ? text_out : const_cast<uint8_t*>(bytes);
+  const PackedText pt{packed, tab};
+  const InputPrep pr = prep ? *prep : InputPrep();
+#define GALE_FUSED(P, N)                                                                       \
+  return launch_fused<P, N>(with_prep, blocks, stream, b, pt, chunks, nchunks, tables, crc_out, \
+                            crc_blocks, frecs, nfused, H, W, C, arena, fres, recs, groups,      \
+                            ngroups, counts, gsum, gbad, pr)
+  if (is_packed) {
+    if (nw == 4) GALE_FUSED(true, 4);
+    if (nw == 8) GALE_FUSED(true, 8);
+    GALE_FUSED(true, 16);
+  }
+  if (nw == 4) GALE_FUSED(false, 4);
+  if (nw == 8) GALE_FUSED(false, 8);
+  GALE_FUSED(false, 16);
+#undef GALE_FUSED
+}
 
 hipError_t ingest_crc_count(const uint8_t* bytes, const CrcChunk* chunks, int nchunks,
                             const uint32_t* tables, uint32_t* crc_out, int nrec, int ngroups,
diff --git a/csrc/runtime/engine.cpp b/csrc/runtime/engine.cpp
--- a/csrc/runtime/engine.cpp
+++ b/csrc/runtime/engine.cpp
@@ -318,6 +318,9 @@
     }
     pools_[i]->set_wait_ms(200);
   }
+  slot_images_only_.assign(nslots, 1);
+  for (auto& rs : replicas_)
+    if (!rs->rep->takes_ingest_images()) slot_images_only_[(size_t)rs->slot] = 0;
   running_ = true;
   stopping_ = false;
   workers_done_ = false;
@@ -904,9 +907,11 @@
       const PixelSource::Dims sd = cfg_.pixels.ingest_dims(cfg_.rec_h(), cfg_.rec_w(), cfg_.C);
       ingest->run_b64(lane, f, dev, pool.chunk_bytes(), cfg_.check_crcs && !f.crc_checked, sd.H,
                       sd.W, sd.C, io, arena, arena_bytes);
-    } else
+    } else {
+      io.images_only = slot_images_only_[(size_t)it.slot] != 0;
       ingest->run(lane, f, dev, pool.chunk_bytes(), cfg_.check_crcs && !f.crc_checked,
                   cfg_.rec_h(), cfg_.rec_w(), cfg_.C, io, arena, arena_bytes);
+    }
   } catch (const std::exception& e) {
     if (!ingest_failed_.exchange(true))
       fprintf(stderr, "[gale decode] GPU ingest failed (%s): host decode from now on\n", e.what());
@@ -938,6 +943,7 @@
     r.dev_locality = slot_key_[(size_t)it.slot];
     if (io.cnt_off[i] >= 0) r.dev_counts = dev + io.cnt_off[i];
     r.dev_image = io.img[i];
+    r.dev_text_gone = !io.text_gone.empty() && io.text_gone[i] != 0;
     r.dev_arena = r.dev_image ? arena : nullptr;
     if (r.dev_image) ++ingest_parsed_;
     ++records_in_;
@@ -1803,6 +1809,8 @@
       t.dev_parse_ns += q.dev_parse_ns;
       t.dev_wait_ns += q.dev_wait_ns;
       t.plan_in_chunk += q.plan_in_chunk;
+      t.fused_records += q.fused_records;
+      t.second_launches += q.second_launches;
     }
     const double n = (double)std::max<int64_t>(1, t.runs);
     s["ingest_fetches"] = (double)t.runs;
@@ -1817,6 +1825,8 @@
     s["ingest_device_wait_s"] = (double)t.wait_ns * 1e-9;
     s["ingest_post_s"] = (double)t.post_ns * 1e-9;
     s["ingest_plan_in_chunk"] = (double)t.plan_in_chunk;
+    s["ingest_fused_records"] = (double)t.fused_records;
+    s["ingest_second_launches"] = (double)t.second_launches;
     s["ingest_dev_runs"] = (double)t.dev_runs;
     s["ingest_dev_copy_s"] = (double)t.dev_copy_ns * 1e-9;
     s["ingest_dev_count_s"] = (double)t.dev_count_ns * 1e-9;
diff --git a/csrc/runtime/engine.h b/csrc/runtime/engine.h
--- a/csrc/runtime/engine.h
+++ b/csrc/runtime/engine.h
@@ -265,6 +265,7 @@
   std::vector<std::shared_ptr<ReplicaSlot>> replicas_;
   std::vector<std::unique_ptr<Batcher>> batchers_;
   std::vector<int> slot_key_;
+  std::vector<char> slot_images_only_;
   std::vector<int> slot_dev_;
   std::vector<std::unique_ptr<kafka::Producer>> producers_;
   std::vector<std::thread> sources_, workers_, decoders_;
diff --git a/csrc/runtime/gpu_ingest.cpp b/csrc/runtime/gpu_ingest.cpp
--- a/csrc/runtime/gpu_ingest.cpp
+++ b/csrc/runtime/gpu_ingest.cpp
@@ -30,6 +30,9 @@
   }
   if (const char* e = getenv("GALE_INGEST_DEV_TIMING")) dev_every_ = std::max(0, atoi(e));
   if (const char* e = getenv("GALE_INGEST_PLAN_SEPARATE")) plan_separate_ = atoi(e) != 0;
+  if (const char* e = getenv("GALE_INGEST_FUSED")) fused_ = atoi(e) != 0;
+  if (const char* e = getenv("GALE_INGEST_FUSED_NW")) fused_nw_ = atoi(e);
+  if (fused_nw_ != 4 && fused_nw_ != 8 && fused_nw_ != 16) fused_nw_ = 0;
   if (dev_every_ > 0)
     for (auto& L : lanes_)
       for (hipEvent_t& ev : L->tev) check_hip(hipEventCreate(&ev), "ingest: timing event");
@@ -166,6 +169,7 @@
   io.cnt_off.assign(nrec_all, -1);
   io.batch_ok.assign(f.batches.size(), 1);
   io.img.assign(nrec_all, nullptr);
+  io.text_gone.assign(nrec_all, 0);
   std::vector<std::pair<int64_t, int64_t>> batches;
   for (const kafka::BatchSpan& b : f.batches) batches.emplace_back((int64_t)b.off, (int64_t)b.len);
   std::vector<B64PlanRecord> recs(nrec_all);
@@ -230,6 +234,7 @@
   io.cnt_off.assign(nrec_all, -1);
   io.batch_ok.assign(f.batches.size(), 1);
   io.img.assign(nrec_all, nullptr);
+  io.text_gone.assign(nrec_all, 0);
   L.batches.clear();
   for (const kafka::BatchSpan& b : f.batches)
     L.batches.emplace_back((int64_t)b.off, (int64_t)b.len);
@@ -245,9 +250,10 @@
   }
   const JsonIngestPlan& p = L.plan;
   plan_json_ingest(L.batches, kafka::kBatchAttrOffset, check_crcs, L.recs, H, W, C,
-                   arena ? arena_bytes : 0, f.size, dev_cap, f.tap_result, plan_separate_, L.plan);
+                   arena ? arena_bytes : 0, f.size, dev_cap, f.tap_result, plan_separate_, L.plan,
+                   fused_ && (io.images_only || f.tap_result < 0) ? kFusedRecordBytes : 0);
   if (p.empty()) return;
-  const size_t nc = p.nc(), nr = p.nr(), np = p.np();
+  const size_t nc = p.nc(), nr = p.nr(), np = p.np(), nf = p.nf();
   grow(L, p.io_bytes + 16, (size_t)p.ntiles + (size_t)p.ngroups + 1);
   uint8_t* hpl = p.plan_in_chunk ? f.buf.get() + p.plan_off : L.h_io;
   uint8_t* dpl = p.plan_in_chunk ? dev + p.plan_off : L.d_io;
@@ -272,16 +278,32 @@
   int* d_gsum = reinterpret_cast<int*>(L.h_io + p.o_gsum);
   int* d_gbad = reinterpret_cast<int*>(L.h_io + p.o_gbad);
   int* d_pbad = reinterpret_cast<int*>(L.h_io + p.o_pbad);
+  int* d_fres = reinterpret_cast<int*>(L.h_io + p.o_fres);
   int* d_cnt = p.cnt_base >= 0 ? reinterpret_cast<int*>(dev + p.cnt_base) : L.d_counts;
-  check_hip(ingest_crc_count(dev, reinterpret_cast<const CrcChunk*>(dpl + p.o_chunks), (int)nc,
-                             d_tables_, d_crc, (int)nr, p.ngroups,
-                             reinterpret_cast<JsonRecord*>(dpl + p.o_recs),
-                             reinterpret_cast<const int2*>(dpl + p.o_groups), d_cnt, d_gsum,
-                             d_gbad, L.stream, p.packed ? dev + p.c_lo : nullptr,
-                             p.packed ? reinterpret_cast<const uint32_t*>(dpl) : nullptr,
-                             p.packed ? dev : nullptr),
-            "ingest: crc32c + count");
+  if (nf > 0)
+    check_hip(ingest_crc_fused(dev, reinterpret_cast<const CrcChunk*>(dpl + p.o_chunks), (int)nc,
+                               d_tables_, d_crc, (int)nf,
+                               reinterpret_cast<const FusedRecord*>(dpl + p.o_frecs), H, W, C,
+                               arena, d_fres,
+                               fused_nw_ ? fused_nw_ : json_fused_waves(p.fused_tiles_max),
+                               nr ? p.ngroups : 0, reinterpret_cast<JsonRecord*>(dpl + p.o_recs),
+                               reinterpret_cast<const int2*>(dpl + p.o_groups), d_cnt, d_gsum,
+                               d_gbad, L.stream, p.packed ? dev + p.c_lo : nullptr,
+                               p.packed ? reinterpret_cast<const uint32_t*>(dpl) : nullptr,
+                               p.packed ? dev : nullptr, &input_prep_),
+              "ingest: crc32c + fused count and parse");
+  else
+    check_hip(ingest_crc_count(dev, reinterpret_cast<const CrcChunk*>(dpl + p.o_chunks), (int)nc,
+                               d_tables_, d_crc, (int)nr, p.ngroups,
+                               reinterpret_cast<JsonRecord*>(dpl + p.o_recs),
+                               reinterpret_cast<const int2*>(dpl + p.o_groups), d_cnt, d_gsum,
+                               d_gbad, L.stream, p.packed ? dev + p.c_lo : nullptr,
+                               p.packed ? reinterpret_cast<const uint32_t*>(dpl) : nullptr,
+                               p.packed ? dev : nullptr),
+              "ingest: crc32c + count");
   mark(L, ts, 2);
+  fused_records_ += (int64_t)nf;
+  second_launches_ += np > 0;
   if (np > 0)
     check_hip(json_parse_instances((int)np, p.ptiles,
                                    reinterpret_cast<JsonRecord*>(dpl + p.o_precs),
@@ -289,8 +311,29 @@
                                    L.d_counts, arena, L.stream, false, nullptr,
                                    nullptr, d_pbad, &input_prep_),
               "ingest: parse");
-  const int64_t t_post = end(L, ts, true);
+  const int64_t t_post = end(L, ts, np > 0);
   join_batch_crcs(f, p.batch_chunks, d_crc, io);
+  for (size_t k = 0; k < nf; ++k) {
+    const size_t i = (size_t)p.frec_of[k];
+    const int* w = d_fres + kFusedResultWords * k;
+    const int64_t tok = w[0];
+    if (tok < 0) throw std::logic_error("ingest: a fused record does not fit its workgroup");
+    io.text_gone[i] = p.packed ? 1 : 0;
+    if (w[1] != 0) {
+      io.status[i] = codec::BAD_NUMBER;
+    } else if (tok == 0) {
+      io.status[i] = codec::EMPTY;
+    } else if (tok % p.per != 0) {
+      io.status[i] = codec::BAD_SHAPE;
+    } else {
+      io.images[i] = (int32_t)(tok / p.per);
+      const int32_t verdict = device_verdict_status(w[2]);
+      const int64_t S = 2 * p.per;
+      const int64_t off = L.recs[i].value_off + L.recs[i].arr_off;
+      if (verdict != codec::OK) io.status[i] = verdict;
+      else io.img[i] = arena + (off + S - 1) / S * p.per;
+    }
+  }
   size_t k = 0;
   for (size_t j = 0; j < nr; ++j) {
     const size_t i = (size_t)p.rec_of[j];
diff --git a/csrc/runtime/gpu_ingest.h b/csrc/runtime/gpu_ingest.h
--- a/csrc/runtime/gpu_ingest.h
+++ b/csrc/runtime/gpu_ingest.h
@@ -42,6 +42,8 @@
     t.dev_parse_ns = dev_parse_ns_.load();
     t.dev_wait_ns = dev_wait_ns_.load();
     t.plan_in_chunk = plan_in_chunk_.load();
+    t.fused_records = fused_records_.load();
+    t.second_launches = second_launches_.load();
     return t;
   }
 
@@ -91,6 +93,9 @@
   int dev_every_ = 0;
   bool plan_separate_ = false;
   std::atomic<int64_t> plan_in_chunk_{0};
+  bool fused_ = true;
+  int fused_nw_ = 0;
+  std::atomic<int64_t> fused_records_{0}, second_launches_{0};
   uint32_t* d_tables_ = nullptr;
   std::vector<std::unique_ptr<Lane>> lanes_;
   kafka::CrcShift shift_chunk_;
diff --git a/csrc/runtime/gpu_replica.cpp b/csrc/runtime/gpu_replica.cpp
--- a/csrc/runtime/gpu_replica.cpp
+++ b/csrc/runtime/gpu_replica.cpp
@@ -230,8 +230,8 @@
     p.arr_len = r.arr_len;
     p.images = r.images;
     p.pinned = r.pinned;
-    p.resident = resident(r);
     p.preparsed = preparsed(r);
+    p.resident = resident(r) && (p.preparsed || !r.dev_text_gone);
     if (p.resident) {
       p.dev_text = reinterpret_cast<uint64_t>(r.dev_value + r.arr_off);
       p.dev_counts = reinterpret_cast<uint64_t>(r.dev_counts);
diff --git a/csrc/runtime/ingest.h b/csrc/runtime/ingest.h
--- a/csrc/runtime/ingest.h
+++ b/csrc/runtime/ingest.h
@@ -14,6 +14,8 @@
   std::vector<int64_t> cnt_off;
   std::vector<char> batch_ok;
   std::vector<const float*> img;
+  bool images_only = false;
+  std::vector<char> text_gone;
   std::vector<uint32_t> b64_offs;
 };
 
@@ -32,6 +34,7 @@
     io.cnt_off.assign(f.records.size(), -1);
     io.batch_ok.assign(f.batches.size(), 1);
     io.img.assign(f.records.size(), nullptr);
+    io.text_gone.assign(f.records.size(), 0);
   }
   virtual void link_bytes(int64_t& text, int64_t& link) const { text = link = 0; }
   struct Timing {
@@ -39,6 +42,8 @@
     int64_t plan_ns = 0;
     int64_t dev_runs = 0, dev_copy_ns = 0, dev_count_ns = 0, dev_parse_ns = 0, dev_wait_ns = 0;
     int64_t plan_in_chunk = 0;
+    int64_t fused_records = 0;
+    int64_t second_launches = 0;
   };
   virtual Timing timing() const { return Timing(); }
 };
diff --git a/csrc/runtime/ingest_plan.cpp b/csrc/runtime/ingest_plan.cpp
--- a/csrc/runtime/ingest_plan.cpp
+++ b/csrc/runtime/ingest_plan.cpp
@@ -55,13 +55,16 @@
 void plan_json_ingest(const std::vector<std::pair<int64_t, int64_t>>& batches, int64_t attr_off,
                       bool check_crcs, const std::vector<JsonPlanRecord>& recs, int H, int W,
                       int C, size_t arena_bytes, size_t fetch_size, size_t dev_cap,
-                      int64_t tap_result, bool plan_separate, JsonIngestPlan& out) {
+                      int64_t tap_result, bool plan_separate, JsonIngestPlan& out,
+                      int64_t fused_cap) {
   {
     JsonIngestPlan fresh;
     fresh.chunks.swap(out.chunks);
     fresh.batch_chunks.swap(out.batch_chunks);
     fresh.rec_of.swap(out.rec_of);
     fresh.pjs.swap(out.pjs);
+    fresh.frec_of.swap(out.frec_of);
+    fresh.frec_of.clear();
     fresh.chunks.clear();
     fresh.batch_chunks.clear();
     fresh.rec_of.clear();
@@ -80,12 +83,22 @@
       throw std::invalid_argument("ingest plan: record outside the fetch");
     if ((uint64_t)r.arr_off + (uint64_t)r.arr_len > (uint64_t)r.value_len)
       throw std::invalid_argument("ingest plan: array outside its record");
+    lo = std::min(lo, (size_t)r.value_off);
+    hi = std::max(hi, (size_t)(r.value_off + r.value_len));
+    const int64_t off = r.value_off + r.arr_off;
+    const int nt = json_tile_count(off, (int32_t)r.arr_len);
+    if (fused_cap > 0 && arena_bytes > 0 && r.arr_len > 0 &&
+        json_aligned_extent(off, r.arr_len) <= fused_cap) {
+      const int64_t S = 2 * per, slot = (off + S - 1) / S, cap = r.arr_len / S;
+      if (cap > 0 && (slot + cap) * per * (int64_t)sizeof(float) <= (int64_t)arena_bytes) {
+        out.frec_of.push_back((int)i);
+        out.fused_tiles_max = std::max(out.fused_tiles_max, nt);
+        continue;
+      }
+    }
     out.rec_of.push_back((int)i);
-    const int nt = json_tile_count(r.value_off + r.arr_off, (int32_t)r.arr_len);
     out.ntiles += nt;
     out.ngroups += (nt + kGroupTiles - 1) / kGroupTiles;
-    lo = std::min(lo, (size_t)r.value_off);
-    hi = std::max(hi, (size_t)(r.value_off + r.value_len));
   }
   if (out.empty()) return;
   const size_t nc = out.nc(), nr = out.nr();
@@ -123,16 +136,19 @@
     }
   }
   const size_t np = out.np(), ngroups = (size_t)out.ngroups, ptiles = (size_t)out.ptiles;
+  const size_t nf = out.nf();
   out.o_chunks = align16(out.ng * 2 * sizeof(uint32_t));
   out.o_groups = out.o_chunks + align16(nc * sizeof(CrcChunk));
   out.o_recs = out.o_groups + align16(ngroups * sizeof(int2));
   out.o_precs = out.o_recs + nr * sizeof(JsonRecord);
   out.o_ptr = out.o_precs + np * sizeof(JsonRecord);
-  out.o_gsum = out.o_ptr + align16(ptiles * sizeof(int));
+  out.o_frecs = out.o_ptr + align16(ptiles * sizeof(int));
+  out.o_gsum = out.o_frecs + nf * sizeof(FusedRecord);
   out.o_crc = out.o_gsum + align16(ngroups * 4);
   out.o_gbad = out.o_crc + align16(nc * 4);
   out.o_pbad = out.o_gbad + align16(ngroups * 4);
-  out.io_bytes = out.o_pbad + align16(ptiles * 4);
+  out.o_fres = out.o_pbad + align16(ptiles * 4);
+  out.io_bytes = out.o_fres + align16(nf * kFusedResultWords * 4);
   out.plan_off = align256(std::max(fetch_size, out.used));
   const size_t plan_lim = out.cnt_base >= 0 ? (size_t)out.cnt_base : dev_cap;
   const bool on_tab = out.packed && out.plan_off < out.tab_off + out.ng * 2 * sizeof(uint32_t) &&
@@ -185,6 +201,13 @@
     const int nt = json_tile_count(pr.off, pr.len);
     for (int t = 0; t < nt; ++t) hpt[pt + t] = (int)k;
     pt += nt;
+  }
+  FusedRecord* hf = reinterpret_cast<FusedRecord*>(dst + p.o_frecs);
+  for (size_t k = 0; k < p.nf(); ++k) {
+    const JsonPlanRecord& r = recs[(size_t)p.frec_of[k]];
+    hf[k].off = r.value_off + r.arr_off;
+    hf[k].len = (int32_t)r.arr_len;
+    hf[k].slot = (int32_t)((hf[k].off + S - 1) / S);
   }
 }
 
diff --git a/csrc/runtime/ingest_plan.h b/csrc/runtime/ingest_plan.h
--- a/csrc/runtime/ingest_plan.h
+++ b/csrc/runtime/ingest_plan.h
@@ -25,6 +25,8 @@
   std::vector<std::pair<size_t, size_t>> batch_chunks;
   std::vector<int> rec_of;
   std::vector<int> pjs;
+  std::vector<int> frec_of;
+  int fused_tiles_max = 0;
   int ntiles = 0, ngroups = 0;
   int ptiles = 0;
   bool packed = false;
@@ -36,6 +38,8 @@
   size_t o_chunks = 0, o_groups = 0, o_recs = 0, o_precs = 0, o_ptr = 0;
   size_t o_gsum = 0;
   size_t o_crc = 0, o_gbad = 0, o_pbad = 0, io_bytes = 0;
+  size_t o_frecs = 0;
+  size_t o_fres = 0;
   size_t plan_off = 0;
   bool plan_in_chunk = false;
   int64_t per = 0;
@@ -43,7 +47,8 @@
   size_t nc() const { return chunks.size(); }
   size_t nr() const { return rec_of.size(); }
   size_t np() const { return pjs.size(); }
-  bool empty() const { return chunks.empty() && rec_of.empty(); }
+  size_t nf() const { return frec_of.size(); }
+  bool empty() const { return chunks.empty() && rec_of.empty() && frec_of.empty(); }
   int64_t cnt_off(const JsonRecord& r) const {
     return cnt_base + ((int64_t)r.tile0 + r.grp0) * (int64_t)sizeof(int);
   }
@@ -52,7 +57,8 @@
 void plan_json_ingest(const std::vector<std::pair<int64_t, int64_t>>& batches, int64_t attr_off,
                       bool check_crcs, const std::vector<JsonPlanRecord>& recs, int H, int W,
                       int C, size_t arena_bytes, size_t fetch_size, size_t dev_cap,
-                      int64_t tap_result, bool plan_separate, JsonIngestPlan& out);
+                      int64_t tap_result, bool plan_separate, JsonIngestPlan& out,
+                      int64_t fused_cap = 0);
 
 void fill_json_ingest(const JsonIngestPlan& plan, const std::vector<JsonPlanRecord>& recs,
                       uint8_t* dst);
diff --git a/csrc/runtime/replica.h b/csrc/runtime/replica.h
--- a/csrc/runtime/replica.h
+++ b/csrc/runtime/replica.h
@@ -45,6 +45,7 @@
   const uint8_t* dev_counts = nullptr;
   const float* dev_image = nullptr;
   const float* dev_arena = nullptr;
+  bool dev_text_gone = false;
   std::shared_ptr<SplitRecord> split;
   int32_t split_index = -1;
 };
@@ -73,6 +74,7 @@
   virtual int locality() const { return device(); }
   virtual void recover() {}
   virtual int64_t resident_records() const { return 0; }
+  virtual bool takes_ingest_images() const { return false; }
   virtual int64_t host_records() const { return 0; }
   virtual int64_t graph_step_batches() const { return 0; }
   virtual int64_t graph_forward_batches() const { return 0; }
@@ -127,6 +129,7 @@
   void wait(Batch& b) override;
   void recover() override;
   int64_t resident_records() const override { return resident_; }
+  bool takes_ingest_images() const override { return ptr_input_; }
   int64_t host_records() const override { return host_; }
   int64_t graph_step_batches() const override { return step_batches_; }
   int64_t graph_forward_batches() const override { return fwd_graph_batches_; }
```

Result: slower. 1.743 million (-15.9%).
